# burchim/AVEC

Hardware: AMD Instinct MI355X
Metric: AV utterances/sec fwd+bwd (audio T=400, video 100x88x88) (higher is better)
Workload: dtype bf16

## Files before the change

avec_amd/csrc/api.hip:

```cpp
#include "common.h"
#include "avec_hip.h"
#include "vec.h"
#include "host_tables.h"
#include <stdarg.h>
#include <stdio.h>

static thread_local char g_err[512] = "";

void avec_set_error(const char* fmt, ...) {
  va_list ap; va_start(ap, fmt); vsnprintf(g_err, sizeof(g_err), fmt, ap); va_end(ap);
}
extern "C" const char* avec_last_error() { return g_err; }

static thread_local char g_kname[128] = "";
void avec_note_kernel(const char* fmt, ...) {
  va_list ap; va_start(ap, fmt); vsnprintf(g_kname, sizeof(g_kname), fmt, ap); va_end(ap);
}
extern "C" const char* avec_last_kernel() { return g_kname; }
extern "C" int avec_version() { return AVEC_ABI_VERSION; }
extern "C" int avec_struct_size(int which) {
  switch (which) {
    case 0: return (int)sizeof(avec_rows_t); case 1: return (int)sizeof(avec_epilogue_t); case 2: return (int)sizeof(avec_attn_t); case 3: return (int)sizeof(avec_tn_item_t);
    case 4: return (int)sizeof(avec_tn_batched_t); case 5: return (int)sizeof(avec_ln_item_t); case 6: return (int)sizeof(avec_fp8_item_t); case 7: return (int)sizeof(avec_wgrad3x3_item_t);
    case 8: return (int)sizeof(avec_ngram_t);
    default: return -1;
  }
}

static WsRegistry g_ws;
static LdsOptin g_lds;

extern "C" int avec_set_reduce_workspace(void* base, long long bytes) {
  int dev = 0; hipError_t e = hipGetDevice(&dev);
  AVEC_CHECK_ARG(e == hipSuccess && dev >= 0 && dev < WsRegistry::MAX_DEV, "set_reduce_workspace: no current device");
  AVEC_CHECK_ARG((base == nullptr && bytes == 0) || (base != nullptr && bytes >= (1 << 16) && ((size_t)base & 255) == 0),
                 "set_reduce_workspace: need a 256-byte aligned buffer of at least 64 KB (or NULL, 0 to unregister)");
  g_ws.set_default(dev, base, (size_t)bytes);
  return 0;
}
extern "C" int avec_set_reduce_workspace_stream(void* base, long long bytes, hipStream_t stream) {
  int dev = 0; hipError_t e = hipGetDevice(&dev);
  AVEC_CHECK_ARG(e == hipSuccess && dev >= 0 && dev < WsRegistry::MAX_DEV && base != nullptr && bytes >= (1 << 16) && ((size_t)base & 255) == 0, "set_reduce_workspace_stream: bad arguments");
  AVEC_CHECK_ARG(g_ws.set_stream(dev, stream, base, (size_t)bytes), "set_reduce_workspace_stream: at most %d stream-bound workspaces", WsRegistry::MAX_STREAMS);
  return 0;
}
ColWs avec_reduce_ws(size_t partial_floats, hipStream_t st) {
  int dev = 0; if (hipGetDevice(&dev) != hipSuccess) return ColWs{nullptr};
  return ColWs{(float*)g_ws.find(dev, st, partial_floats * sizeof(float))};
}

int avec_lds_optin_quiet(const void* kernel, size_t bytes) {
  if (bytes <= LdsOptin::FREE_BYTES) return 0;
  int dev = 0; if (hipGetDevice(&dev) != hipSuccess || dev < 0) return (int)hipErrorNoDevice;
  return g_lds.request(dev, kernel, bytes, [](const void* k, size_t n) {
    const hipError_t e = hipFuncSetAttribute(k, hipFuncAttributeMaxDynamicSharedMemorySize, (int)n);
    if (e != hipSuccess) (void)hipGetLastError();
    return (int)e;
  });
}
int avec_lds_optin(const void* kernel, size_t bytes) {
  const int r = avec_lds_optin_quiet(kernel, bytes);
  if (r == LdsOptin::TOO_LARGE) avec_set_error("%zu bytes of LDS requested (> 160 KiB)", bytes);
  else if (r) avec_set_error("cannot reserve %zu bytes of LDS: %s", bytes, hipGetErrorString((hipError_t)r));
  return r;
}
```

avec_amd/csrc/convmod.hip:

```cpp
#include "vec.h"
#include "avec_hip.h"

static constexpr int KMAX = 16;

template <typename T>
__device__ __forceinline__ void glu4(const T* u, long long row, int C, int col, float g[4]) {
  float a[4], b[4]; ld4<T>(u + row * 2 * C + col, a); ld4<T>(u + row * 2 * C + C + col, b);
  for (int e = 0; e < 4; ++e) g[e] = a[e] * sigmoidf_(b[e]);
}

static constexpr int DW_TT = 32;
template <typename T>
__device__ __forceinline__ void stage_glu(float* gs, const T* u, long long b, int Tn, int C, int col, int t_base, int nrows) {
  const int tx = threadIdx.x & 31, ty = threadIdx.x >> 5;
  for (int r0 = ty; r0 < nrows; r0 += 48) {
    float a[6][4], bq[6][4];
#pragma unroll
    for (int q = 0; q < 6; ++q) {
      const int r = r0 + 8 * q, t = t_base + r;
      const bool ok = r < nrows && col < C && t >= 0 && t < Tn;
      const long long row = ok ? b * Tn + t : b * Tn;
      const int cc = col < C ? col : 0;
      ld4<T>(u + row * 2 * C + cc, a[q]); ld4<T>(u + row * 2 * C + C + cc, bq[q]);
      if (!ok) { a[q][0] = a[q][1] = a[q][2] = a[q][3] = 0.f; }
// ... 144 lines not shown
      float g4[4], s1[4], s2[4];
      ld4<float>(bnb.ss + cc, bSc); ld4<float>(bnb.ss + C + cc, bSh); ld4<float>(bnb.ss + 2 * C + cc, bMu); ld4<float>(bnb.ss + 3 * C + cc, bRs);
      ld4<float>(bnb.gamma + cc, g4); ld4<float>(bnb.dstats + cc, s1); ld4<float>(bnb.dstats + C + cc, s2);
#pragma unroll
      for (int e = 0; e < 4; ++e) { bA[e] = g4[e] * bRs[e]; bM1[e] = s1[e] * bnb.inv_n; bM2[e] = s2[e] * bnb.inv_n; }
      if (blockIdx.y == 0 && ty == 0 && col < C && bnb.dgamma) {
#pragma unroll
        for (int e = 0; e < 4; ++e) { atomicAdd(bnb.dgamma + col + e, s2[e]); atomicAdd(bnb.dbeta + col + e, s1[e]); }
      }
    }
    for (int r0 = ty; r0 < nrows; r0 += 48) {
      float d[6][4];
#pragma unroll
      for (int q = 0; q < 6; ++q) {
        const int r = r0 + 8 * q, f = f0 + r; const bool ok = r < nrows && col < C && f >= 0 && f < Tn;
        ld4<T>(dc + ((long long)b * Tn + (ok ? f : 0)) * C + cc, d[q]);
        if (bnb.c) {
          float cv[4]; ld4<T>((const T*)bnb.c + ((long long)b * Tn + (ok ? f : 0)) * C + cc, cv);
#pragma unroll
          for (int e = 0; e < 4; ++e) { const float dd = d[q][e] * dswishf_(cv[e] * bSc[e] + bSh[e]); d[q][e] = bA[e] * (dd - bM1[e] - (cv[e] - bMu[e]) * bRs[e] * bM2[e]); }
        }
        if (!ok) d[q][0] = d[q][1] = d[q][2] = d[q][3] = 0.f;
      }
#pragma unroll
      for (int q = 0; q < 6; ++q) { const int r = r0 + 8 * q; if (r < nrows) *(float4*)(ds + r * 128 + tx * 4) = make_float4(d[q][0], d[q][1], d[q][2], d[q][3]); }
    }
  }
  __syncthreads();
  float part[KMAX + 1][4];
#pragma unroll
  for (int k = 0; k <= KMAX; ++k) for (int e = 0; e < 4; ++e) part[k][e] = 0.f;
  if (col < C) {
    float ww[KMAX][4];
#pragma unroll
    for (int k = 0; k < KMAX; ++k) { if (k < K) ld4<float>(w + (long long)k * C + col, ww[k]); else ww[k][0] = ww[k][1] = ww[k][2] = ww[k][3] = 0.f; }
    const int own = K - 1 - padl;
#pragma unroll
    for (int q = 0; q < DW_TT / 8; ++q) {
      const int r = ty + 8 * q;
      if (r >= nto) break;
      const long long row = (long long)b * Tn + t0 + r;
      float a[4], bq[4]; ld4<T>(u + row * 2 * C + col, a); ld4<T>(u + row * 2 * C + C + col, bq);
      const float4 dq = *(const float4*)(ds + (own + r) * 128 + tx * 4);
      part[KMAX][0] += dq.x; part[KMAX][1] += dq.y; part[KMAX][2] += dq.z; part[KMAX][3] += dq.w;
      float dg[4] = {0.f, 0.f, 0.f, 0.f};
#pragma unroll
      for (int k = 0; k < KMAX; ++k) {
        if (k < K) {
          const float4 g = *(const float4*)(gs + (r + k) * 128 + tx * 4);
          part[k][0] += dq.x * g.x; part[k][1] += dq.y * g.y; part[k][2] += dq.z * g.z; part[k][3] += dq.w * g.w;
          const float4 dd = *(const float4*)(ds + (r + K - 1 - k) * 128 + tx * 4);
          dg[0] += ww[k][0] * dd.x; dg[1] += ww[k][1] * dd.y; dg[2] += ww[k][2] * dd.z; dg[3] += ww[k][3] * dd.w;
        }
      }
      float o1[4], o2[4];
#pragma unroll
      for (int e = 0; e < 4; ++e) { const float sg = sigmoidf_(bq[e]); o1[e] = dg[e] * sg; o2[e] = dg[e] * a[e] * sg * (1.f - sg); }
      st4<T>(du + row * 2 * C + col, o1); st4<T>(du + row * 2 * C + C + col, o2);
    }
  }
  __syncthreads();
  const int lane = threadIdx.x & 63, wv = threadIdx.x >> 6;
#pragma unroll
  for (int k = 0; k <= KMAX; ++k)
#pragma unroll
    for (int e = 0; e < 4; ++e) part[k][e] += __shfl_xor(part[k][e], 32, 64);
  if (lane < 32) {
#pragma unroll
    for (int k = 0; k <= KMAX; ++k) *(float4*)(gs + ((wv * (KMAX + 1) + k) * 32 + tx) * 4) = make_float4(part[k][0], part[k][1], part[k][2], part[k][3]);
  }
  __syncthreads();
  float* mine = ws.partial ? ws_slot(ws, blockIdx.x, blockIdx.y, gridDim.y, (KMAX + 1) * 128) : nullptr;
  for (int i = threadIdx.x; i < (KMAX + 1) * 128; i += 256) {
    const int k = i >> 7, c = i & 127;
    const float v = gs[(0 * (KMAX + 1) + k) * 128 + c] + gs[(1 * (KMAX + 1) + k) * 128 + c] + gs[(2 * (KMAX + 1) + k) * 128 + c] + gs[(3 * (KMAX + 1) + k) * 128 + c];
    if (mine) mine[i] = v;
    else {
      const int cc = blockIdx.x * 128 + c;
      float* d = k == KMAX ? dbias : (k < K ? dw + (long long)k * C : nullptr);
      if (d && cc < C) atomicAdd(d + cc, v);
    }
  }
}

extern "C" int avec_glu_dwconv_fwd(int dtype, const void* u, const float* w, const float* bias, void* out, float* stats,
                                   int B, int T_, int C, int K, int stride, int pad_left, hipStream_t st) {
  AVEC_CHECK_ARG(u && w && out && B > 0 && T_ > 0 && C > 0 && C % 4 == 0 && K > 0 && K <= KMAX && stride > 0 && pad_left >= 0 && pad_left < K, "glu_dwconv_fwd: bad arguments (C=%d K=%d pad_left=%d)", C, K, pad_left);
  const int To = (T_ - 1) / stride + 1;
  const int nchunks = (To + DW_TT - 1) / DW_TT;
  dim3 grid((unsigned)((C / 4 + 31) / 32), (unsigned)(B * nchunks)); const ColPlan plan = ColPlan::grid<2>(grid, C, st, stats != nullptr);
  const size_t lds = (size_t)((DW_TT - 1) * stride + K) * 128 * sizeof(float);
  AVEC_CHECK_ARG(lds <= 64 * 1024, "glu_dwconv_fwd: stride %d too large", stride);
  DISPATCH_T(dtype, hipLaunchKernelGGL(glu_dwconv_fwd_kernel<T>, grid, dim3(256), lds, st, (const T*)u, w, bias, (T*)out, stats, B, T_, C, K, stride, To, pad_left, nchunks, plan.ws));
  AVEC_LAUNCH_CHECK();
  return plan.finish({stats, stats + C}, C, st);
}
__global__ __launch_bounds__(256) void bn_finalize_ws_kernel(const float* __restrict__ partial, int nslots, float count, const float* gamma, const float* beta, float* rmean, float* rvar,
                                                             long long* nbt, float momentum, float eps, float* ss, int C) {
  __shared__ float red[2][16][17];
  const int cl = threadIdx.x & 15, rl = threadIdx.x >> 4;
  const int c = blockIdx.x * 16 + cl;
  const bool lead = rl == 0 && c < C;
  float gm = 0.f, bt = 0.f, rm = 0.f, rv = 0.f;
  if (lead) { gm = gamma[c]; bt = beta[c]; if (rmean) { rm = rmean[c]; rv = rvar[c]; } }
  float s1 = 0.f, s2 = 0.f;
  if (c < C) {
    const float* p = partial + (size_t)(c >> 7) * nslots * 256 + (c & 127);
    for (int r = rl; r < nslots; r += 16) { s1 += p[(size_t)r * 256]; s2 += p[(size_t)r * 256 + 128]; }
  }
  red[0][rl][cl] = s1; red[1][rl][cl] = s2;
  __syncthreads();
  if (!lead) return;
  s1 = 0.f; s2 = 0.f;
#pragma unroll
  for (int k = 0; k < 16; ++k) { s1 += red[0][k][cl]; s2 += red[1][k][cl]; }
  const float n = count;
  const float mean = s1 / n, var = fmaxf(s2 / n - mean * mean, 0.f);
  if (rmean && isfinite(mean) && isfinite(var)) {
    rmean[c] = (1.f - momentum) * rm + momentum * mean;
    rvar[c] = (1.f - momentum) * rv + momentum * var * (n / fmaxf(n - 1.f, 1.f));
    if (c == 0 && nbt) *nbt += 1;
  }
  const float rs = rsqrtf(var + eps);
  ss[c] = gm * rs; ss[C + c] = bt - mean * gm * rs; ss[2 * C + c] = mean; ss[3 * C + c] = rs;
}

extern "C" int avec_glu_dwconv_fwd_bn(int dtype, const void* u, const float* w, const float* bias, void* out, float* stats, int B, int T_, int C, int K, int stride, int pad_left,
                                      const float* gamma, const float* beta, float* running_mean, float* running_var, long long* num_batches_tracked, float momentum, float eps,
                                      float* ss, hipStream_t st) {
  AVEC_CHECK_ARG(u && w && out && stats && gamma && beta && ss && B > 0 && T_ > 0 && C > 0 && C % 4 == 0 && K > 0 && K <= KMAX && stride > 0 && pad_left >= 0 && pad_left < K,
                 "glu_dwconv_fwd_bn: bad arguments (C=%d K=%d pad_left=%d)", C, K, pad_left);
  const int To = (T_ - 1) / stride + 1;
  const int nchunks = (To + DW_TT - 1) / DW_TT;
  dim3 grid((unsigned)((C / 4 + 31) / 32), (unsigned)(B * nchunks)); const ColPlan plan = ColPlan::grid<2>(grid, C, st);
  const size_t lds = (size_t)((DW_TT - 1) * stride + K) * 128 * sizeof(float);
  AVEC_CHECK_ARG(lds <= 64 * 1024, "glu_dwconv_fwd_bn: stride %d too large", stride);
  DISPATCH_T(dtype, hipLaunchKernelGGL(glu_dwconv_fwd_kernel<T>, grid, dim3(256), lds, st, (const T*)u, w, bias, (T*)out, stats, B, T_, C, K, stride, To, pad_left, nchunks, plan.ws));
  AVEC_LAUNCH_CHECK();
  const float count = (float)((long long)B * To);
  if (plan.ws.partial) {
    hipLaunchKernelGGL(bn_finalize_ws_kernel, dim3((C + 15) / 16), dim3(256), 0, st, (const float*)plan.ws.partial, (int)plan.nslots, count, gamma, beta, running_mean, running_var,
                       num_batches_tracked, momentum, eps, ss, C);
    AVEC_LAUNCH_CHECK();
    return 0;
  }
  return avec_bn_finalize(stats, 1, nullptr, count, gamma, beta, running_mean, running_var, num_batches_tracked, momentum, eps, ss, C, 1, st);
}
static int dw_finish(const ColPlan& plan, float* dw, float* dbias, int C, int K, hipStream_t st) {
  float* dst[KMAX + 1];
  for (int k = 0; k < KMAX; ++k) dst[k] = (k < K) ? dw + (long long)k * C : nullptr;
  dst[KMAX] = dbias;
  return plan.finish(dst, C, st);
}
extern "C" int avec_dwconv_glu_bwd_bn(int dtype, const void* da, const void* c, const float* ss, const float* gamma, const float* dstats, float count, const void* u, const float* w,
                                      void* du, float* dw, float* dbias, float* dgamma, float* dbeta, int B, int T_, int C, int K, int pad_left, hipStream_t st) {
  AVEC_CHECK_ARG(da && c && ss && gamma && dstats && count > 0.f && u && w && du && dw && B > 0 && T_ > 0 && C > 0 && C % 4 == 0 && K > 0 && K <= KMAX && pad_left >= 0 && pad_left < K,
                 "dwconv_glu_bwd_bn: bad arguments");
  AVEC_CHECK_ARG((dgamma == nullptr) == (dbeta == nullptr), "dwconv_glu_bwd_bn: dgamma and dbeta come together (both or neither)");
  const int nchunks = (T_ + DW_TT - 1) / DW_TT;
  dim3 grid((unsigned)((C / 4 + 31) / 32), (unsigned)(B * nchunks)); const ColPlan plan = ColPlan::grid<KMAX + 1>(grid, C, st);
  size_t l2 = (size_t)2 * (DW_TT - 1 + K) * 128 * sizeof(float);
  if (l2 < (size_t)4 * (KMAX + 1) * 128 * sizeof(float)) l2 = (size_t)4 * (KMAX + 1) * 128 * sizeof(float);
  AVEC_CHECK_ARG(l2 <= 64 * 1024, "dwconv_glu_bwd_bn: kernel size %d too large", K);
  DwBnb bnb{c, ss, gamma, dstats, 1.f / count, dgamma, dbeta};
  DISPATCH_T(dtype, hipLaunchKernelGGL(dwconv_glu_bwd_fused_kernel<T>, grid, dim3(256), l2, st, (const T*)da, (const T*)u, w, (T*)du, dw, dbias, B, T_, C, K, pad_left, nchunks, plan.ws, bnb));
  AVEC_LAUNCH_CHECK();
  return dw_finish(plan, dw, dbias, C, K, st);
}
extern "C" int avec_dwconv_glu_bwd(int dtype, const void* dc, const void* u, const float* w, void* du, float* dw, float* dbias,
                                   int B, int T_, int C, int K, int stride, int pad_left, hipStream_t st) {
  AVEC_CHECK_ARG(dc && u && w && du && dw && B > 0 && T_ > 0 && C > 0 && C % 4 == 0 && K > 0 && K <= KMAX && stride > 0 && pad_left >= 0 && pad_left < K, "dwconv_glu_bwd: bad arguments");
  const int To = (T_ - 1) / stride + 1;
  long long n4 = (long long)B * T_ * (C / 4); long long nb = (n4 + 255) / 256; if (nb > 4096) nb = 4096;
  const int nchunks = (To + DW_TT - 1) / DW_TT;
  dim3 grid((unsigned)((C / 4 + 31) / 32), (unsigned)(B * nchunks)); const ColPlan plan = ColPlan::grid<KMAX + 1>(grid, C, st);
  size_t lds = (size_t)((DW_TT - 1) * stride + K) * 128 * sizeof(float);
  if (lds < (size_t)4 * (KMAX + 1) * 128 * sizeof(float)) lds = (size_t)4 * (KMAX + 1) * 128 * sizeof(float);
  AVEC_CHECK_ARG(lds <= 64 * 1024, "dwconv_glu_bwd: stride %d too large", stride);
  if (stride == 1) {
    size_t l2 = (size_t)2 * (DW_TT - 1 + K) * 128 * sizeof(float); if (l2 < lds) l2 = lds;
    DISPATCH_T(dtype, hipLaunchKernelGGL(dwconv_glu_bwd_fused_kernel<T>, grid, dim3(256), l2, st, (const T*)dc, (const T*)u, w, (T*)du, dw, dbias, B, T_, C, K, pad_left, nchunks, plan.ws));
  } else
  DISPATCH_T(dtype, hipLaunchKernelGGL(dwconv_glu_bwd_input_kernel<T>, dim3((unsigned)nb), dim3(256), 0, st, (const T*)dc, (const T*)u, w, (T*)du, B, T_, C, K, stride, To, pad_left);
             hipLaunchKernelGGL(dwconv_bwd_weight_kernel<T>, grid, dim3(256), lds, st, (const T*)dc, (const T*)u, dw, dbias, B, T_, C, K, stride, To, pad_left, nchunks, plan.ws));
  AVEC_LAUNCH_CHECK();
  return dw_finish(plan, dw, dbias, C, K, st);
}

template <typename T>
__device__ __forceinline__ void glu_dwconv_stream_body(const T* __restrict__ u, const float* __restrict__ w, const float* __restrict__ bias, const float* __restrict__ ss,
                                                       T* __restrict__ out, T* state, long long p0, int n, int Tq, int C, int K, int stride, int To) {
  extern __shared__ __attribute__((aligned(16))) float gs[];
  const int tx = threadIdx.x & 31, ty = threadIdx.x >> 5; const int col = (blockIdx.x * 32 + tx) * 4; const int b = blockIdx.y;
  const int Hn = K - 1;
  const bool live = col < C; const int cc = live ? col : 0;
  float ww[KMAX][4], bb[4] = {0.f, 0.f, 0.f, 0.f}, sc[4], sh[4];
#pragma unroll
  for (int k = 0; k < KMAX; ++k) { if (k < K) ld4<float>(w + (long long)k * C + cc, ww[k]); else ww[k][0] = ww[k][1] = ww[k][2] = ww[k][3] = 0.f; }
  if (bias) ld4<float>(bias + cc, bb);
  ld4<float>(ss + cc, sc); ld4<float>(ss + C + cc, sh);
  T* const sb = state + (long long)b * Hn * 2 * C;
  const T* const ub = u + (long long)b * Tq * 2 * C;
  for (int r = ty; r < Hn + Tq; r += 8) {
    const bool ctx = r < Hn; const bool ok = live && (!ctx || p0 - Hn + r >= 0);
    const T* row = ctx ? sb + (long long)r * 2 * C : ub + (long long)(r - Hn) * 2 * C;
    float a[4], g[4]; ld4<T>(row + cc, a); ld4<T>(row + C + cc, g);
    *(float4*)(gs + r * 128 + tx * 4) = ok ? make_float4(a[0] * sigmoidf_(g[0]), a[1] * sigmoidf_(g[1]), a[2] * sigmoidf_(g[2]), a[3] * sigmoidf_(g[3])) : make_float4(0.f, 0.f, 0.f, 0.f);
  }
  float na[2][4], nb[2][4];
#pragma unroll
  for (int q = 0; q < 2; ++q) {
    const int r = ty + 8 * q;
    if (r < Hn && n > 0) {
      const int src = r + n; const T* row = src < Hn ? sb + (long long)src * 2 * C : ub + (long long)(src - Hn) * 2 * C;
      ld4<T>(row + cc, na[q]); ld4<T>(row + C + cc, nb[q]);
    }
  }
  __syncthreads();
  if (!live) return;
#pragma unroll
  for (int q = 0; q < 2; ++q) {
    const int r = ty + 8 * q;
    if (r < Hn && n > 0) { st4<T>(sb + (long long)r * 2 * C + col, na[q]); st4<T>(sb + (long long)r * 2 * C + C + col, nb[q]); }
  }
  for (int o = ty; o < To; o += 8) {
    float acc[4] = {bb[0], bb[1], bb[2], bb[3]};
#pragma unroll
    for (int k = 0; k < KMAX; ++k) {
      if (k < K) {
        const float4 g = *(const float4*)(gs + (o * stride + k) * 128 + tx * 4);
        acc[0] += ww[k][0] * g.x; acc[1] += ww[k][1] * g.y; acc[2] += ww[k][2] * g.z; acc[3] += ww[k][3] * g.w;
      }
    }
#pragma unroll
    for (int e = 0; e < 4; ++e) acc[e] = swishf_(acc[e] * sc[e] + sh[e]);
    st4<T>(out + ((long long)b * To + o) * C + col, acc);
  }
}
template <typename T>
__global__ __launch_bounds__(256) void glu_dwconv_stream_kernel(const T* __restrict__ u, const float* __restrict__ w, const float* __restrict__ bias, const float* __restrict__ ss,
                                                                T* __restrict__ out, T* state, const long long* __restrict__ pos, const unsigned char* __restrict__ reset,
                                                                const long long* __restrict__ clen, int div, int Tq, int C, int K, int stride, int To) {
  const int b = blockIdx.y;
  long long p0 = (reset && reset[b]) ? 0 : pos[b] / div; if (p0 < 0) p0 = 0;
  int n = Tq;
  if (clen) { long long c = (clen[b] + div - 1) / div; n = c < 0 ? 0 : (c > Tq ? Tq : (int)c); }
  glu_dwconv_stream_body<T>(u, w, bias, ss, out, state, p0, n, Tq, C, K, stride, To);
}
template <typename T>
__global__ __launch_bounds__(256) void glu_dwconv_stream_la_kernel(const T* __restrict__ u, const float* __restrict__ w, const float* __restrict__ bias, const float* __restrict__ ss,
                                                                   T* __restrict__ out, T* state, const long long* __restrict__ pos, const unsigned char* __restrict__ reset,
                                                                   const long long* __restrict__ ncommit, int div, int Wq, int C, int K, int stride, int To) {
  const int b = blockIdx.y;
  long long p0 = (reset && reset[b]) ? 0 : pos[b] / div; if (p0 < 0) p0 = 0;
  const long long c = ncommit[b] / div;
  glu_dwconv_stream_body<T>(u, w, bias, ss, out, state, p0, c < 0 ? 0 : (c > Wq ? Wq : (int)c), Wq, C, K, stride, To);
}

extern "C" long long avec_glu_dwconv_stream_state_bytes(int dtype, int B, int C, int K) {
  if (B <= 0 || C <= 0 || K <= 0) return 0;
  return (long long)B * (K - 1) * 2 * C * (dtype == AVEC_BF16 ? 2 : 4);
}
extern "C" int avec_glu_dwconv_stream(int dtype, const void* u, const float* w, const float* bias, const float* ss, void* out, void* state, long long state_bytes,
                                      const long long* pos, const unsigned char* reset, const long long* chunk_len, int div, int B, int Tq, int C, int K, int stride, hipStream_t st) {
  AVEC_CHECK_ARG(u && w && ss && out && pos, "glu_dwconv_stream: null pointer (u, w, ss, out and pos are required)");
  AVEC_CHECK_ARG(B > 0 && Tq > 0 && div > 0 && stride > 0 && Tq % stride == 0, "glu_dwconv_stream: bad dims B=%d Tq=%d div=%d stride=%d (Tq must be a multiple of the stride)", B, Tq, div, stride);
  AVEC_CHECK_ARG(C > 0 && C % 4 == 0, "glu_dwconv_stream: C=%d must be a positive multiple of 4 (4-channel vector accesses)", C);
  AVEC_CHECK_ARG(K > 0 && K <= KMAX, "glu_dwconv_stream: kernel size K=%d outside 1..%d", K, KMAX);
  AVEC_CHECK_ARG(K == 1 || state, "glu_dwconv_stream: null state (K=%d needs %d context rows per slot)", K, K - 1);
  AVEC_CHECK_ARG(state_bytes >= avec_glu_dwconv_stream_state_bytes(dtype, B, C, K), "glu_dwconv_stream: state of %lld bytes, %lld needed (avec_glu_dwconv_stream_state_bytes)",
                 state_bytes, avec_glu_dwconv_stream_state_bytes(dtype, B, C, K));
  AVEC_CHECK_ARG(avec_aligned16(u) && avec_aligned16(w) && avec_aligned16(bias) && avec_aligned16(ss) && avec_aligned16(out) && avec_aligned16(state),
                 "glu_dwconv_stream: u, w, bias, ss, out and state must be 16-byte aligned");
  AVEC_CHECK_ARG((((uintptr_t)pos) & 7) == 0 && (((uintptr_t)chunk_len) & 7) == 0, "glu_dwconv_stream: pos and chunk_len must be 8-byte aligned (int64)");
  const size_t lds = (size_t)(K - 1 + Tq) * 128 * sizeof(float);
  AVEC_CHECK_ARG(lds <= 48 * 1024, "glu_dwconv_stream: chunk of %d frames too long (K - 1 + Tq <= 96)", Tq);
  dim3 grid((unsigned)((C / 4 + 31) / 32), (unsigned)B);
  DISPATCH_T(dtype, hipLaunchKernelGGL(glu_dwconv_stream_kernel<T>, grid, dim3(256), lds, st, (const T*)u, w, bias, ss, (T*)out, (T*)state, pos, reset, chunk_len, div, Tq, C, K, stride, Tq / stride));
  AVEC_LAUNCH_CHECK();
  return 0;
}
extern "C" int avec_glu_dwconv_stream_la(int dtype, const void* u, const float* w, const float* bias, const float* ss, void* out, void* state, long long state_bytes,
                                         const long long* pos, const unsigned char* reset, const long long* ncommit, int div, int B, int Wq, int C, int K, int stride, hipStream_t st) {
  AVEC_CHECK_ARG(u && w && ss && out && pos && ncommit, "glu_dwconv_stream_la: null pointer (u, w, ss, out, pos and ncommit are required)");
  AVEC_CHECK_ARG(B > 0 && Wq > 0 && div > 0 && stride > 0 && Wq % stride == 0, "glu_dwconv_stream_la: bad dims B=%d Wq=%d div=%d stride=%d (Wq must be a multiple of the stride)", B, Wq, div, stride);
  AVEC_CHECK_ARG(C > 0 && C % 4 == 0, "glu_dwconv_stream_la: C=%d must be a positive multiple of 4 (4-channel vector accesses)", C);
  AVEC_CHECK_ARG(K > 0 && K <= KMAX, "glu_dwconv_stream_la: kernel size K=%d outside 1..%d", K, KMAX);
  AVEC_CHECK_ARG(K == 1 || state, "glu_dwconv_stream_la: null state (K=%d needs %d context rows per slot)", K, K - 1);
  AVEC_CHECK_ARG(state_bytes >= avec_glu_dwconv_stream_state_bytes(dtype, B, C, K), "glu_dwconv_stream_la: state of %lld bytes, %lld needed (avec_glu_dwconv_stream_state_bytes)",
                 state_bytes, avec_glu_dwconv_stream_state_bytes(dtype, B, C, K));
  AVEC_CHECK_ARG(avec_aligned16(u) && avec_aligned16(w) && avec_aligned16(bias) && avec_aligned16(ss) && avec_aligned16(out) && avec_aligned16(state),
                 "glu_dwconv_stream_la: u, w, bias, ss, out and state must be 16-byte aligned");
  AVEC_CHECK_ARG((((uintptr_t)pos) & 7) == 0 && (((uintptr_t)ncommit) & 7) == 0, "glu_dwconv_stream_la: pos and ncommit must be 8-byte aligned (int64)");
  const size_t lds = (size_t)(K - 1 + Wq) * 128 * sizeof(float);
  AVEC_CHECK_ARG(lds <= 48 * 1024, "glu_dwconv_stream_la: window of %d frames too long (K - 1 + Wq <= 96)", Wq);
  dim3 grid((unsigned)((C / 4 + 31) / 32), (unsigned)B);
  DISPATCH_T(dtype, hipLaunchKernelGGL(glu_dwconv_stream_la_kernel<T>, grid, dim3(256), lds, st, (const T*)u, w, bias, ss, (T*)out, (T*)state, pos, reset, ncommit, div, Wq, C, K, stride, Wq / stride));
  AVEC_LAUNCH_CHECK();
  return 0;
}
__global__ void stream_advance_kernel(long long* pos, unsigned char* reset, const long long* clen, long long full, int B) {
  const int b = blockIdx.x * blockDim.x + threadIdx.x;
  if (b >= B) return;
  long long c = clen ? clen[b] : full; c = c < 0 ? 0 : (c > full ? full : c);
  pos[b] = ((reset && reset[b]) ? 0 : pos[b]) + c;
  if (reset) reset[b] = 0;
}
extern "C" int avec_stream_advance(long long* pos, unsigned char* reset, const long long* chunk_len, long long full, int B, hipStream_t st) {
  AVEC_CHECK_ARG(pos && B > 0 && full > 0 && (((uintptr_t)pos) & 7) == 0 && (((uintptr_t)chunk_len) & 7) == 0, "stream_advance: bad arguments (B=%d full=%lld)", B, full);
  hipLaunchKernelGGL(stream_advance_kernel, dim3((B + 63) / 64), dim3(64), 0, st, pos, reset, chunk_len, full, B);
  AVEC_LAUNCH_CHECK();
  return 0;
}

__global__ __launch_bounds__(256) void stream_window_kernel(const float* __restrict__ x_new, const float* __restrict__ tail, float* __restrict__ X, const long long* __restrict__ pend,
                                                            const long long* __restrict__ n_new, const unsigned char* __restrict__ last, const unsigned char* __restrict__ reset,
                                                            const unsigned char* __restrict__ ended, long long* __restrict__ nvalid, long long* __restrict__ ncommit,
                                                            long long* __restrict__ emit, int Tc, int LAe, int D, int S) {
  const int r = blockIdx.x, b = blockIdx.y;
  const bool rs = reset && reset[b];
  long long pe = rs ? 0 : pend[b]; pe = pe < 0 ? 0 : (pe > LAe ? LAe : pe);
  long long nn = n_new ? n_new[b] : Tc; nn = nn < 0 ? 0 : (nn > Tc ? Tc : nn);
  if (!rs && ended[b]) { pe = 0; nn = 0; }
  const long long n = pe + nn;
  const float* src = r < pe ? tail + ((long long)b * LAe + r) * D : (r < n ? x_new + ((long long)b * Tc + (r - pe)) * D : nullptr);
  float* dst = X + ((long long)b * (Tc + LAe) + r) * D;
  for (int c = threadIdx.x; c < D; c += 256) dst[c] = src ? src[c] : 0.f;
  if (r == 0 && threadIdx.x == 0) {
    const bool ends = last && last[b];
    long long c = n - LAe; c = c < 0 ? 0 : c - c % S;
    nvalid[b] = n; ncommit[b] = ends ? 0 : c; emit[b] = ends ? n : c;
  }
}
extern "C" int avec_stream_window(const float* x_new, const float* tail, float* X, const long long* pend, const long long* n_new, const unsigned char* last, const unsigned char* reset,
                                  const unsigned char* ended, long long* nvalid, long long* ncommit, long long* emit, int B, int Tc, int LAe, int D, int S, hipStream_t st) {
  AVEC_CHECK_ARG(x_new && X && pend && ended && nvalid && ncommit && emit && (tail || LAe == 0),
                 "stream_window: null pointer (x_new, tail, X, pend, ended, nvalid, ncommit and emit are required)");
  AVEC_CHECK_ARG(B > 0 && Tc > 0 && LAe >= 0 && D > 0 && S > 0 && Tc % S == 0 && LAe % S == 0, "stream_window: bad dims B=%d Tc=%d LAe=%d D=%d S=%d (Tc and LAe must be multiples of S)", B, Tc, LAe, D, S);
  AVEC_CHECK_ARG(!(((uintptr_t)x_new | (uintptr_t)tail | (uintptr_t)X) & 3) && !(((uintptr_t)pend | (uintptr_t)n_new | (uintptr_t)nvalid | (uintptr_t)ncommit | (uintptr_t)emit) & 7),
// ... 38 lines not shown
```

avec_amd/csrc/norm.hip:

```cpp
#include "common.h"
#include "avec_hip.h"

#include "vec.h"
#include <type_traits>

__global__ __launch_bounds__(256) void col_finalize_kernel(ColFin f) {
  __shared__ float red[16][17];
  const int cw = threadIdx.x & 15, sl = threadIdx.x >> 4;
  const int ncols = f.NV * f.W;
  const int o = blockIdx.x * 16 + cw;
  const unsigned cb = blockIdx.y;
  const int s0 = blockIdx.z * 128;
  float s = 0.f;
  if (o < ncols) {
    const float* p = f.partial + ((size_t)cb * f.nslots) * ncols + o;
#pragma unroll
    for (int k = 0; k < 8; ++k) {
      const int si = s0 + sl + 16 * k; const int sc = si < f.nslots ? si : f.nslots - 1;
      const float v = p[(size_t)sc * ncols];
      s += si < f.nslots ? v : 0.f;
    }
  }
  red[sl][cw] = s;
  __syncthreads();
  if (sl == 0 && o < ncols) {
    float t = 0.f;
#pragma unroll
    for (int k = 0; k < 16; ++k) t += red[k][cw];
    const int n = o / f.W, w = o - n * f.W; const int col = (int)cb * f.W + w;
    float* d = nullptr;
#pragma unroll
    for (int i = 0; i < FIN_MAXNV; ++i) if (i == n) d = f.dst[i];
    if (d && col < f.C) atomicAdd(d + (long long)col * f.dstride, t);
  }
}
int col_finalize(const ColWs& ws, unsigned colblocks, unsigned nslots, int NV, int W, float* const* dst, int C, hipStream_t st, int dstride) {
  AVEC_CHECK_ARG(NV >= 1 && NV <= FIN_MAXNV, "col_finalize: %d reduced quantities (at most %d)", NV, FIN_MAXNV);
  ColFin f; f.partial = ws.partial; f.NV = NV; f.W = W; f.C = C; f.nslots = (int)nslots; f.dstride = dstride;
  for (int i = 0; i < FIN_MAXNV; ++i) f.dst[i] = i < NV ? dst[i] : nullptr;
  dim3 grid((unsigned)((NV * W + 15) / 16), colblocks, (nslots + 127) / 128);
  hipLaunchKernelGGL(col_finalize_kernel, grid, dim3(256), 0, st, f);
  AVEC_LAUNCH_CHECK(); return 0;
}

template <typename TO>
__global__ __launch_bounds__(256) void ln_fwd_kernel(const float* __restrict__ x, const float* __restrict__ g, const float* __restrict__ b,
                                                     TO* __restrict__ y, float* __restrict__ mean, float* __restrict__ rstd, long long M, int D, float eps) {
  const int lane = threadIdx.x & 63; const long long row = (long long)blockIdx.x * 4 + (threadIdx.x >> 6);
  if (row >= M) return;
  const float* xr = x + row * D;
  float s = 0.f;
  for (int c = lane * 4; c < D; c += 256) { float v[4]; ld4<float>(xr + c, v); s += v[0] + v[1] + v[2] + v[3]; }
  const float mu = wave_sum(s) / D;
  float q = 0.f;
  for (int c = lane * 4; c < D; c += 256) { float v[4]; ld4<float>(xr + c, v); for (int e = 0; e < 4; ++e) { float d = v[e] - mu; q += d * d; } }
  const float rs = rsqrtf(wave_sum(q) / D + eps);
  if (lane == 0) { mean[row] = mu; rstd[row] = rs; }
  for (int c = lane * 4; c < D; c += 256) {
    float v[4], gg[4], bb[4], o[4]; ld4<float>(xr + c, v); ld4<float>(g + c, gg); ld4<float>(b + c, bb);
    for (int e = 0; e < 4; ++e) o[e] = (v[e] - mu) * rs * gg[e] + bb[e];
    st4<TO>(y + row * D + c, o);
  }
}

template <typename TG, int NG>
__global__ __launch_bounds__(256) void ln_bwd_kernel(const TG* __restrict__ dy, const float* __restrict__ x, const float* __restrict__ mean,
                                                     const float* __restrict__ rstd, const float* __restrict__ g, float* dx, const float* dres,
                                                     float* __restrict__ dg, float* __restrict__ db, long long M, int D, ColWs ws) {
  const int lane = threadIdx.x & 63; const int wave_id = blockIdx.x * 4 + (threadIdx.x >> 6); const int nwaves = gridDim.x * 4;
  float pg[NG][4], pb[NG][4], gg[NG][4];
#pragma unroll
  for (int i = 0; i < NG; ++i) {
    const int c = lane * 4 + i * 256;
#pragma unroll
    for (int e = 0; e < 4; ++e) { pg[i][e] = 0.f; pb[i][e] = 0.f; gg[i][e] = 0.f; }
    if (c < D) ld4<float>(g + c, gg[i]);
  }
  struct RowData { float d[NG][4], v[NG][4], o[NG][4], mu, rs; };
  auto fetch = [&](long long row, RowData& r) {
    r.mu = mean[row]; r.rs = rstd[row];
#pragma unroll
    for (int i = 0; i < NG; ++i) {
      const int c = lane * 4 + i * 256;
      if (c < D) {
        ld4<TG>(dy + row * D + c, r.d[i]); ld4<float>(x + row * D + c, r.v[i]);
        if (dres) ld4<float>(dres + row * D + c, r.o[i]); else { r.o[i][0] = r.o[i][1] = r.o[i][2] = r.o[i][3] = 0.f; }
      } else {
#pragma unroll
        for (int e = 0; e < 4; ++e) { r.d[i][e] = 0.f; r.v[i][e] = r.mu; r.o[i][e] = 0.f; }
      }
    }
  };
  RowData cur, nxt;
  long long row = wave_id;
  if (row < M) fetch(row, cur);
  for (; row < M; row += nwaves) {
    const bool more = row + nwaves < M;
    if (more) fetch(row + nwaves, nxt);
    float s1 = 0.f, s2 = 0.f;
#pragma unroll
    for (int i = 0; i < NG; ++i)
#pragma unroll
      for (int e = 0; e < 4; ++e) {
        const float xh = (cur.v[i][e] - cur.mu) * cur.rs, t = cur.d[i][e] * gg[i][e];
        cur.v[i][e] = xh; s1 += t; s2 += t * xh; pg[i][e] += cur.d[i][e] * xh; pb[i][e] += cur.d[i][e];
      }
    s1 = wave_sum(s1) / D; s2 = wave_sum(s2) / D;
#pragma unroll
    for (int i = 0; i < NG; ++i) {
      const int c = lane * 4 + i * 256; if (c >= D) break;
#pragma unroll
      for (int e = 0; e < 4; ++e) cur.o[i][e] += cur.rs * (cur.d[i][e] * gg[i][e] - s1 - cur.v[i][e] * s2);
      st4<float>(dx + row * D + c, cur.o[i]);
    }
    if (more) cur = nxt;
  }
  extern __shared__ float lnred[];
  for (int c = threadIdx.x; c < 2 * D; c += 256) lnred[c] = 0.f;
  __syncthreads();
#pragma unroll
  for (int i = 0; i < NG; ++i) {
    int c = lane * 4 + i * 256; if (c >= D) break;
    for (int e = 0; e < 4; ++e) { atomicAdd(lnred + c + e, pg[i][e]); atomicAdd(lnred + D + c + e, pb[i][e]); }
  }
  __syncthreads();
  if (!ws.partial) { for (int c = threadIdx.x; c < D; c += 256) { atomicAdd(dg + c, lnred[c]); atomicAdd(db + c, lnred[D + c]); } return; }
  float* mine = ws_slot(ws, 0, blockIdx.x, gridDim.x, 2 * D);
  for (int c = threadIdx.x; c < 2 * D; c += 256) mine[c] = lnred[c];
}

extern "C" int avec_layernorm_fwd(int dtype, const float* x, const float* gamma, const float* beta, void* y, int y_f32,
                                  float* mean, float* rstd, long long M, int D, float eps, hipStream_t st) {
  AVEC_CHECK_ARG(x && gamma && beta && y && mean && rstd, "layernorm_fwd: null pointer");
  AVEC_CHECK_ARG(M > 0 && D > 0 && D % 4 == 0, "layernorm_fwd: D=%d must be a positive multiple of 4", D);
  dim3 grid((unsigned)((M + 3) / 4));
  if (y_f32 || dtype == AVEC_F32) hipLaunchKernelGGL(ln_fwd_kernel<float>, grid, dim3(256), 0, st, x, gamma, beta, (float*)y, mean, rstd, M, D, eps);
  else hipLaunchKernelGGL(ln_fwd_kernel<bf16>, grid, dim3(256), 0, st, x, gamma, beta, (bf16*)y, mean, rstd, M, D, eps);
  AVEC_LAUNCH_CHECK(); return 0;
}

struct LnPrep { void* out; float alpha, p; const unsigned long long* rng; unsigned stream; int f32; };
template <typename TG, int NG>
__global__ __launch_bounds__(256) void ln_bwd_rows_kernel(const TG* __restrict__ dy, const float* __restrict__ x, const float* __restrict__ mean,
                                                          const float* __restrict__ rstd, const float* __restrict__ g, float* __restrict__ dx,
                                                          const float* __restrict__ dres, long long M, int D, LnPrep pr) {
  const int lane = threadIdx.x & 63; const long long row = (long long)blockIdx.x * 4 + (threadIdx.x >> 6);
  if (row >= M) return;
  const float mu = mean[row], rs = rstd[row];
  DropKey dk; dk.k0 = 0u; dk.thr = 0u; dk.scale = 1.f;
  if (pr.out) dk = drop_key(pr.rng, pr.stream, pr.p);
  float d[NG][4], v[NG][4], o[NG][4], gg[NG][4];
#pragma unroll
  for (int i = 0; i < NG; ++i) {
    const int c = lane * 4 + i * 256;
    if (c < D) {
      ld4<TG>(dy + row * D + c, d[i]); ld4<float>(x + row * D + c, v[i]); ld4<float>(g + c, gg[i]);
      if (dres) ld4<float>(dres + row * D + c, o[i]); else { o[i][0] = o[i][1] = o[i][2] = o[i][3] = 0.f; }
    } else {
#pragma unroll
      for (int e = 0; e < 4; ++e) { d[i][e] = 0.f; v[i][e] = mu; o[i][e] = 0.f; gg[i][e] = 0.f; }
    }
  }
  float s1 = 0.f, s2 = 0.f;
#pragma unroll
  for (int i = 0; i < NG; ++i)
#pragma unroll
    for (int e = 0; e < 4; ++e) { const float xh = (v[i][e] - mu) * rs, t = d[i][e] * gg[i][e]; v[i][e] = xh; s1 += t; s2 += t * xh; }
  s1 = wave_sum(s1) / D; s2 = wave_sum(s2) / D;
#pragma unroll
  for (int i = 0; i < NG; ++i) {
    const int c = lane * 4 + i * 256; if (c >= D) break;
#pragma unroll
    for (int e = 0; e < 4; ++e) o[i][e] += rs * (d[i][e] * gg[i][e] - s1 - v[i][e] * s2);
    st4<float>(dx + row * D + c, o[i]);
    if (pr.out) {
      float q[4];
      float ds[4]; drop4(dk, (unsigned long long)row * D + c, ds);
#pragma unroll
      for (int e = 0; e < 4; ++e) q[e] = o[i][e] * (pr.alpha * ds[e]);
      if (pr.f32) st4<float>((float*)pr.out + row * D + c, q); else st4<bf16>((bf16*)pr.out + row * D + c, q);
    }
  }
}

template <typename TO>
__global__ __launch_bounds__(256) void ln_fwd2_kernel(const float* __restrict__ x, const float* __restrict__ g1, const float* __restrict__ b1, float eps1,
                                                      float* __restrict__ y1, float* __restrict__ mean1, float* __restrict__ rstd1,
                                                      const float* __restrict__ g2, const float* __restrict__ b2, float eps2,
                                                      TO* __restrict__ h2, float* __restrict__ mean2, float* __restrict__ rstd2, long long M, int D) {
  const int lane = threadIdx.x & 63; const long long row = (long long)blockIdx.x * 4 + (threadIdx.x >> 6);
  if (row >= M) return;
  float v[2][4];
#pragma unroll
  for (int i = 0; i < 2; ++i) { const int c = lane * 4 + i * 256; if (c < D) ld4<float>(x + row * D + c, v[i]); else v[i][0] = v[i][1] = v[i][2] = v[i][3] = 0.f; }
  auto norm = [&](const float* g, const float* b, float eps, float* mean, float* rstd) {
    float sm = 0.f;
#pragma unroll
    for (int i = 0; i < 2; ++i) sm += v[i][0] + v[i][1] + v[i][2] + v[i][3];
    const float mu = wave_sum(sm) / D;
    float q = 0.f;
#pragma unroll
    for (int i = 0; i < 2; ++i) { const int c = lane * 4 + i * 256; if (c < D) for (int e = 0; e < 4; ++e) { const float d = v[i][e] - mu; q += d * d; } }
    const float rs = rsqrtf(wave_sum(q) / D + eps);
    if (lane == 0) { mean[row] = mu; rstd[row] = rs; }
#pragma unroll
    for (int i = 0; i < 2; ++i) {
      const int c = lane * 4 + i * 256; if (c >= D) break;
      float gg[4], bb[4]; ld4<float>(g + c, gg); ld4<float>(b + c, bb);
      for (int e = 0; e < 4; ++e) v[i][e] = (v[i][e] - mu) * rs * gg[e] + bb[e];
    }
  };
  norm(g1, b1, eps1, mean1, rstd1);
#pragma unroll
  for (int i = 0; i < 2; ++i) { const int c = lane * 4 + i * 256; if (c < D) st4<float>(y1 + row * D + c, v[i]); }
  norm(g2, b2, eps2, mean2, rstd2);
#pragma unroll
  for (int i = 0; i < 2; ++i) { const int c = lane * 4 + i * 256; if (c < D) st4<TO>(h2 + row * D + c, v[i]); }
}
extern "C" int avec_layernorm_fwd2(int dtype, const float* x, const float* gamma1, const float* beta1, float eps1, float* y1, float* mean1, float* rstd1,
                                   const float* gamma2, const float* beta2, float eps2, void* h2, float* mean2, float* rstd2, long long M, int D, hipStream_t st) {
  AVEC_CHECK_ARG(x && gamma1 && beta1 && y1 && mean1 && rstd1 && gamma2 && beta2 && h2 && mean2 && rstd2, "layernorm_fwd2: null pointer");
  AVEC_CHECK_ARG(M > 0 && D > 0 && D % 4 == 0 && D <= 512, "layernorm_fwd2: D=%d must be a multiple of 4 in [4, 512]", D);
  dim3 grid((unsigned)((M + 3) / 4));
  if (dtype == AVEC_F32) hipLaunchKernelGGL(ln_fwd2_kernel<float>, grid, dim3(256), 0, st, x, gamma1, beta1, eps1, y1, mean1, rstd1, gamma2, beta2, eps2, (float*)h2, mean2, rstd2, M, D);
  else hipLaunchKernelGGL(ln_fwd2_kernel<bf16>, grid, dim3(256), 0, st, x, gamma1, beta1, eps1, y1, mean1, rstd1, gamma2, beta2, eps2, (bf16*)h2, mean2, rstd2, M, D);
  AVEC_LAUNCH_CHECK(); return 0;
}
template <typename TG>
__global__ __launch_bounds__(256) void ln_bwd_rows2_kernel(const TG* __restrict__ dy2, const float* __restrict__ x2, const float* __restrict__ mean2, const float* __restrict__ rstd2,
                                                           const float* __restrict__ g2, const float* __restrict__ dres2, float* __restrict__ dx2,
                                                           const float* __restrict__ x1, const float* __restrict__ mean1, const float* __restrict__ rstd1,
                                                           const float* __restrict__ g1, float* __restrict__ dx1, long long M, int D, LnPrep pr) {
  const int lane = threadIdx.x & 63; const long long row = (long long)blockIdx.x * 4 + (threadIdx.x >> 6);
  if (row >= M) return;
  float d[2][4], v[2][4], o[2][4], gg[2][4], w1[2][4], gg1[2][4];
  const float mu2 = mean2[row], rs2 = rstd2[row], mu1 = mean1[row], rs1 = rstd1[row];
  DropKey dk; dk.k0 = 0u; dk.thr = 0u; dk.scale = 1.f;
  if (pr.out) dk = drop_key(pr.rng, pr.stream, pr.p);
#pragma unroll
  for (int i = 0; i < 2; ++i) {
    const int c = lane * 4 + i * 256;
    if (c < D) {
      ld4<TG>(dy2 + row * D + c, d[i]); ld4<float>(x2 + row * D + c, v[i]); ld4<float>(g2 + c, gg[i]); ld4<float>(x1 + row * D + c, w1[i]); ld4<float>(g1 + c, gg1[i]);
      if (dres2) ld4<float>(dres2 + row * D + c, o[i]); else { o[i][0] = o[i][1] = o[i][2] = o[i][3] = 0.f; }
    } else {
#pragma unroll
      for (int e = 0; e < 4; ++e) { d[i][e] = 0.f; v[i][e] = mu2; o[i][e] = 0.f; gg[i][e] = 0.f; w1[i][e] = mu1; gg1[i][e] = 0.f; }
    }
  }
  float s1 = 0.f, s2 = 0.f;
#pragma unroll
  for (int i = 0; i < 2; ++i)
#pragma unroll
    for (int e = 0; e < 4; ++e) { const float xh = (v[i][e] - mu2) * rs2, t = d[i][e] * gg[i][e]; v[i][e] = xh; s1 += t; s2 += t * xh; }
  s1 = wave_sum(s1) / D; s2 = wave_sum(s2) / D;
#pragma unroll
  for (int i = 0; i < 2; ++i) {
    const int c = lane * 4 + i * 256;
#pragma unroll
    for (int e = 0; e < 4; ++e) o[i][e] += rs2 * (d[i][e] * gg[i][e] - s1 - v[i][e] * s2);
    if (c < D) st4<float>(dx2 + row * D + c, o[i]); else { o[i][0] = o[i][1] = o[i][2] = o[i][3] = 0.f; }
  }
  float t1 = 0.f, t2 = 0.f;
#pragma unroll
  for (int i = 0; i < 2; ++i)
#pragma unroll
    for (int e = 0; e < 4; ++e) { const float xh = (w1[i][e] - mu1) * rs1, t = o[i][e] * gg1[i][e]; w1[i][e] = xh; t1 += t; t2 += t * xh; }
  t1 = wave_sum(t1) / D; t2 = wave_sum(t2) / D;
#pragma unroll
  for (int i = 0; i < 2; ++i) {
    const int c = lane * 4 + i * 256; if (c >= D) break;
    float r[4];
#pragma unroll
    for (int e = 0; e < 4; ++e) r[e] = rs1 * (o[i][e] * gg1[i][e] - t1 - w1[i][e] * t2);
    st4<float>(dx1 + row * D + c, r);
    if (pr.out) {
      float q[4], ds[4]; drop4(dk, (unsigned long long)row * D + c, ds);
#pragma unroll
      for (int e = 0; e < 4; ++e) q[e] = r[e] * (pr.alpha * ds[e]);
      if (pr.f32) st4<float>((float*)pr.out + row * D + c, q); else st4<bf16>((bf16*)pr.out + row * D + c, q);
    }
  }
}
extern "C" int avec_layernorm_bwd2(int dtype, const void* dy2, const float* x2, const float* mean2, const float* rstd2, const float* gamma2, const float* dres2, float* dx2,
                                   const float* x1, const float* mean1, const float* rstd1, const float* gamma1, float* dx1,
                                   void* prep, float prep_alpha, float prep_drop_p, const unsigned long long* rng, unsigned rng_stream, long long M, int D, hipStream_t st) {
  AVEC_CHECK_ARG(dy2 && x2 && mean2 && rstd2 && gamma2 && dx2 && x1 && mean1 && rstd1 && gamma1 && dx1, "layernorm_bwd2: null pointer");
  AVEC_CHECK_ARG(M > 0 && D > 0 && D % 4 == 0 && D <= 512 && (!prep || prep_drop_p <= 0.f || rng), "layernorm_bwd2: D=%d must be a multiple of 4 in [4, 512]; dropout needs rng", D);
  LnPrep pr; pr.out = prep; pr.alpha = prep_alpha; pr.p = prep ? prep_drop_p : 0.f; pr.rng = rng; pr.stream = rng_stream; pr.f32 = dtype == AVEC_F32;
  dim3 grid((unsigned)((M + 3) / 4));
  if (dtype == AVEC_F32) hipLaunchKernelGGL(ln_bwd_rows2_kernel<float>, grid, dim3(256), 0, st, (const float*)dy2, x2, mean2, rstd2, gamma2, dres2, dx2, x1, mean1, rstd1, gamma1, dx1, M, D, pr);
  else hipLaunchKernelGGL(ln_bwd_rows2_kernel<bf16>, grid, dim3(256), 0, st, (const bf16*)dy2, x2, mean2, rstd2, gamma2, dres2, dx2, x1, mean1, rstd1, gamma1, dx1, M, D, pr);
  AVEC_LAUNCH_CHECK(); return 0;
}

struct LnItem { const void* dy; const float* x; const float* mean; const float* rstd; float* dg; float* db; int M, D, dy_f32, first; };
struct LnGroup { LnItem it[AVEC_LN_GROUP_MAX]; int n; };
static constexpr int LNG_ROWS = 128;
__global__ __launch_bounds__(256) void ln_param_grads_grouped_kernel(LnGroup grp) {
  __shared__ float red[2][256][4];
  const int w = blockIdx.x;
  int lo = 0, hi = grp.n - 1;
  while (lo < hi) { const int mid = (lo + hi + 1) >> 1; if (grp.it[mid].first <= w) lo = mid; else hi = mid - 1; }
  const LnItem& t = grp.it[lo];
  const int D = t.D, L = D >> 2, R = 256 / L;
  const int r = threadIdx.x / L, l = threadIdx.x - r * L;
  const int m0 = (w - t.first) * LNG_ROWS; int m1 = m0 + LNG_ROWS; if (m1 > t.M) m1 = t.M;
  float pg[4] = {0.f, 0.f, 0.f, 0.f}, pb[4] = {0.f, 0.f, 0.f, 0.f};
  if (r < R) {
    constexpr int U = 8;
    for (int m = m0 + r; m < m1; m += R * U) {
      float d[U][4], v[U][4], mu[U], rs[U];
#pragma unroll
      for (int u = 0; u < U; ++u) {
        const int mm = m + u * R; const bool ok = mm < m1; const long long mi = ok ? mm : m;
        if (t.dy_f32) ld4<float>((const float*)t.dy + mi * D + l * 4, d[u]); else ld4<bf16>((const bf16*)t.dy + mi * D + l * 4, d[u]);
        ld4<float>(t.x + mi * D + l * 4, v[u]); mu[u] = t.mean[mi]; rs[u] = ok ? t.rstd[mi] : 0.f;
        if (!ok) d[u][0] = d[u][1] = d[u][2] = d[u][3] = 0.f;
      }
#pragma unroll
      for (int u = 0; u < U; ++u)
#pragma unroll
        for (int e = 0; e < 4; ++e) { pg[e] += d[u][e] * (v[u][e] - mu[u]) * rs[u]; pb[e] += d[u][e]; }
    }
  }
#pragma unroll
  for (int e = 0; e < 4; ++e) { red[0][threadIdx.x][e] = pg[e]; red[1][threadIdx.x][e] = pb[e]; }
  __syncthreads();
  for (int o = threadIdx.x; o < 2 * D; o += 256) {
    const int which = o >= D, c = o - which * D; float s = 0.f;
    for (int rr = 0; rr < R; ++rr) s += red[which][rr * L + (c >> 2)][c & 3];
    atomicAdd((which ? t.db : t.dg) + c, s);
  }
}
extern "C" int avec_layernorm_param_grads_grouped(int dtype, const avec_ln_item_t* items, int n, hipStream_t st) {
  AVEC_CHECK_ARG(items && n > 0 && n <= AVEC_LN_GROUP_MAX, "layernorm_param_grads_grouped: need 1..%d items (got %d)", AVEC_LN_GROUP_MAX, n);
  LnGroup grp; grp.n = n; int first = 0;
  for (int k = 0; k < n; ++k) {
    const avec_ln_item_t& s = items[k];
    AVEC_CHECK_ARG(s.dy && s.x && s.mean && s.rstd && s.dgamma && s.dbeta && s.M > 0 && s.M < (1ll << 31) && s.D >= 4 && s.D % 4 == 0 && s.D <= 1024,
                   "layernorm_param_grads_grouped: item %d: null pointer or D=%d not a multiple of 4 in [4, 1024]", k, s.D);
    LnItem& t = grp.it[k];
    t.dy = s.dy; t.x = s.x; t.mean = s.mean; t.rstd = s.rstd; t.dg = s.dgamma; t.db = s.dbeta; t.M = (int)s.M; t.D = s.D;
    t.dy_f32 = (s.dy_f32 || dtype == AVEC_F32) ? 1 : 0; t.first = first;
    first += (int)((s.M + LNG_ROWS - 1) / LNG_ROWS);
  }
  hipLaunchKernelGGL(ln_param_grads_grouped_kernel, dim3((unsigned)first), dim3(256), 0, st, grp);
  AVEC_LAUNCH_CHECK(); return 0;
}

static int layernorm_bwd_impl(int dtype, const void* dy, int dy_f32, const float* x, const float* mean, const float* rstd, const float* gamma,
                              float* dx, const float* dres, float* dgamma, float* dbeta, long long M, int D, const LnPrep& pr, hipStream_t st) {
  AVEC_CHECK_ARG(dy && x && mean && rstd && gamma && dx && (!dgamma == !dbeta), "layernorm_bwd: null pointer");
  AVEC_CHECK_ARG(M > 0 && D > 0 && D % 4 == 0 && D <= 1536, "layernorm_bwd: D=%d must be a multiple of 4 and <= 1536", D);
  AVEC_CHECK_ARG(!pr.out || (!dgamma && (pr.p <= 0.f || pr.rng)), "layernorm_bwd_prep: the second output comes with the dx-only kernel (dgamma == NULL); dropout needs rng");
  if (!dgamma) {
    const dim3 grid((unsigned)((M + 3) / 4)); const bool f32in = dy_f32 || dtype == AVEC_F32;
#define AVEC_LN_ROWS(TG, NG) hipLaunchKernelGGL((ln_bwd_rows_kernel<TG, NG>), grid, dim3(256), 0, st, (const TG*)dy, x, mean, rstd, gamma, dx, dres, M, D, pr)
    if (D <= 512) { if (f32in) AVEC_LN_ROWS(float, 2); else AVEC_LN_ROWS(bf16, 2); }
    else { if (f32in) AVEC_LN_ROWS(float, 6); else AVEC_LN_ROWS(bf16, 6); }
#undef AVEC_LN_ROWS
    AVEC_LAUNCH_CHECK(); return 0;
  }
  long long nb = (M + 15) / 16; if (nb > 256) nb = 256; if (nb < 1) nb = 1;
  const ColPlan plan = ColPlan::flat<2>((unsigned)nb, D, st).cap_without_ws(128);
  const size_t lds = (size_t)2 * D * sizeof(float);
#define AVEC_LN_BWD(TG, NG) hipLaunchKernelGGL((ln_bwd_kernel<TG, NG>), dim3(plan.nslots), dim3(256), lds, st, (const TG*)dy, x, mean, rstd, gamma, dx, dres, dgamma, dbeta, M, D, plan.ws)
  const bool f32in = dy_f32 || dtype == AVEC_F32;
  if (D <= 512) { if (f32in) AVEC_LN_BWD(float, 2); else AVEC_LN_BWD(bf16, 2); }
  else { if (f32in) AVEC_LN_BWD(float, 6); else AVEC_LN_BWD(bf16, 6); }
#undef AVEC_LN_BWD
  AVEC_LAUNCH_CHECK();
  return plan.finish({dgamma, dbeta}, D, st);
}
extern "C" int avec_layernorm_bwd(int dtype, const void* dy, int dy_f32, const float* x, const float* mean, const float* rstd, const float* gamma,
                                  float* dx, const float* dres, float* dgamma, float* dbeta, long long M, int D, hipStream_t st) {
  LnPrep pr; pr.out = nullptr; pr.alpha = 1.f; pr.p = 0.f; pr.rng = nullptr; pr.stream = 0; pr.f32 = 0;
  return layernorm_bwd_impl(dtype, dy, dy_f32, x, mean, rstd, gamma, dx, dres, dgamma, dbeta, M, D, pr, st);
}
extern "C" int avec_layernorm_bwd_prep(int dtype, const void* dy, int dy_f32, const float* x, const float* mean, const float* rstd, const float* gamma,
                                       float* dx, const float* dres, void* prep, float prep_alpha, float prep_drop_p, const unsigned long long* rng, unsigned rng_stream,
                                       long long M, int D, hipStream_t st) {
  AVEC_CHECK_ARG(prep, "layernorm_bwd_prep: null prep buffer");
  LnPrep pr; pr.out = prep; pr.alpha = prep_alpha; pr.p = prep_drop_p; pr.rng = rng; pr.stream = rng_stream; pr.f32 = dtype == AVEC_F32;
  return layernorm_bwd_impl(dtype, dy, dy_f32, x, mean, rstd, gamma, dx, dres, nullptr, nullptr, M, D, pr, st);
}

template <typename T>
__global__ __launch_bounds__(256) void grad_prep_kernel(const float* __restrict__ dout, long long ldd, T* __restrict__ dacc, float alpha, float p,
                                                        const unsigned long long* rng, unsigned stream, float* dbias, long long M, int N, ColWs ws) {
  const int tx = threadIdx.x & 31, ty = threadIdx.x >> 5;
  const int col = (blockIdx.x * 32 + tx) * 4;
  float part[1][4] = {{0.f, 0.f, 0.f, 0.f}};
  const DropKey dk = drop_key(rng, stream, p);
  if (col < N) {
    for (long long row = (long long)blockIdx.y * 8 + ty; row < M; row += (long long)gridDim.y * 8) {
      float v[4]; ld4<float>(dout + row * ldd + col, v);
      float ds[4]; drop4(dk, (unsigned long long)row * N + col, ds);
      for (int e = 0; e < 4; ++e) { v[e] *= alpha * ds[e]; part[0][e] += v[e]; }
      st4<T>(dacc + row * N + col, v);
    }
  }
  float* const dst[1] = {dbias};
  if (dbias) colreduce_atomic<1>(part, dst, col, N, ws);
}

template <typename T>
__global__ __launch_bounds__(256) void grad_prep_flat_kernel(const float* __restrict__ dout, long long ldd, T* __restrict__ dacc, float alpha, float p,
                                                             const unsigned long long* rng, unsigned stream, long long M, int N) {
  const int N4 = N >> 2; const long long n4 = M * N4;
  const DropKey dk = drop_key(rng, stream, p);
  for (long long i = (long long)blockIdx.x * 256 + threadIdx.x; i < n4; i += (long long)gridDim.x * 256) {
    const long long row = n4 < (1ll << 31) ? (long long)((unsigned)i / (unsigned)N4) : i / N4; const int col = (int)(i - row * N4) * 4;
    float v[4]; ld4<float>(dout + row * ldd + col, v);
    float ds[4]; drop4(dk, (unsigned long long)row * N + col, ds);
    for (int e = 0; e < 4; ++e) v[e] *= alpha * ds[e];
    st4<T>(dacc + row * N + col, v);
  }
}
extern "C" int avec_grad_prep(int dtype, const float* dout, long long ld, void* dacc, float alpha, float drop_p, const unsigned long long* rng,
                              unsigned rng_stream, float* dbias, long long M, int N, hipStream_t st) {
  AVEC_CHECK_ARG(dout && dacc && M > 0 && N > 0 && N % 4 == 0 && ld % 4 == 0, "grad_prep: bad arguments (N=%d ld=%lld)", N, ld);
  AVEC_CHECK_ARG(!(drop_p > 0.f) || rng, "grad_prep: dropout without rng");
  if (!dbias) {
    long long nb = (M * (N / 4) + 255) / 256; if (nb > 8192) nb = 8192;
    DISPATCH_T(dtype, hipLaunchKernelGGL(grad_prep_flat_kernel<T>, dim3((unsigned)nb), dim3(256), 0, st, dout, ld, (T*)dacc, alpha, drop_p, rng, rng_stream, M, N));
    AVEC_LAUNCH_CHECK(); return 0;
  }
  dim3 grid = col_grid(M, N); const ColPlan plan = ColPlan::grid<1>(grid, N, st);
  DISPATCH_T(dtype, hipLaunchKernelGGL(grad_prep_kernel<T>, grid, dim3(256), 0, st, dout, ld, (T*)dacc, alpha, drop_p, rng, rng_stream, dbias, M, N, plan.ws));
  AVEC_LAUNCH_CHECK();
  return plan.finish({dbias}, N, st);
}

template <typename T>
__global__ __launch_bounds__(256) void colsum_kernel(const T* __restrict__ x, long long ld, float* out, long long M, int N, ColWs ws) {
  const int tx = threadIdx.x & 31, ty = threadIdx.x >> 5; const int col = (blockIdx.x * 32 + tx) * 4;
  float part[1][4] = {{0.f, 0.f, 0.f, 0.f}};
  if (col < N) for (long long row = (long long)blockIdx.y * 8 + ty; row < M; row += (long long)gridDim.y * 8) {
    float v[4]; ld4<T>(x + row * ld + col, v); for (int e = 0; e < 4; ++e) part[0][e] += v[e];
  }
  float* const dst[1] = {out};
  colreduce_atomic<1>(part, dst, col, N, ws);
}
extern "C" int avec_colsum(int dtype, const void* x, long long ld, float* out, long long M, int N, hipStream_t st) { return colsum_launch(dtype, x, ld, out, M, N, true, st); }
int colsum_launch(int dtype, const void* x, long long ld, float* out, long long M, int N, bool use_ws, hipStream_t st) {
  AVEC_CHECK_ARG(x && out && M > 0 && N > 0 && N % 4 == 0 && ld % 4 == 0, "colsum: bad arguments");
  dim3 grid = col_grid(M, N); if (!use_ws && grid.y > 16) grid.y = 16; const ColPlan plan = ColPlan::grid<1>(grid, N, st, use_ws);
  DISPATCH_T(dtype, hipLaunchKernelGGL(colsum_kernel<T>, grid, dim3(256), 0, st, (const T*)x, ld, out, M, N, plan.ws));
  AVEC_LAUNCH_CHECK();
  return plan.finish({out}, N, st);
}

template <typename T>
__global__ __launch_bounds__(256) void bn_stats_kernel(const T* __restrict__ y, float* stats, long long M, int C, ColWs ws) {
  const int tx = threadIdx.x & 31, ty = threadIdx.x >> 5; const int col = (blockIdx.x * 32 + tx) * 4;
  float part[2][4] = {{0.f, 0.f, 0.f, 0.f}, {0.f, 0.f, 0.f, 0.f}};
  if (col < C) for (long long row = (long long)blockIdx.y * 8 + ty; row < M; row += (long long)gridDim.y * 8) {
    float v[4]; ld4<T>(y + row * C + col, v); for (int e = 0; e < 4; ++e) { part[0][e] += v[e]; part[1][e] += v[e] * v[e]; }
  }
  float* const dst[2] = {stats, stats + C};
  colreduce_atomic<2>(part, dst, col, C, ws);
}
extern "C" int avec_bn_stats(int dtype, const void* y, float* stats, long long M, int C, hipStream_t st) {
  AVEC_CHECK_ARG(y && stats && M > 0 && C > 0 && C % 4 == 0, "bn_stats: bad arguments");
  dim3 grid = col_grid(M, C); const ColPlan plan = ColPlan::grid<2>(grid, C, st);
  DISPATCH_T(dtype, hipLaunchKernelGGL(bn_stats_kernel<T>, grid, dim3(256), 0, st, (const T*)y, stats, M, C, plan.ws));
  AVEC_LAUNCH_CHECK();
  return plan.finish({stats, stats + C}, C, st);
}

__global__ __launch_bounds__(256) void bn_finalize_kernel(const float* stats, int nrep, const float* count_ptr, float count, const float* gamma, const float* beta, float* rmean, float* rvar,
                                                          long long* nbt, float momentum, float eps, float* ss, int C, int training) {
  __shared__ float red[2][16][17];
  const int cl = threadIdx.x & 15, rl = threadIdx.x >> 4;
  const int c = blockIdx.x * 16 + cl;
  const bool lead = rl == 0 && c < C;
  float gm = 0.f, bt = 0.f, rm = 0.f, rv = 0.f, n = count;
  if (lead) { gm = gamma[c]; bt = beta[c]; if (rmean) { rm = rmean[c]; rv = rvar[c]; } if (training && count_ptr) n = *count_ptr; }
  float s1 = 0.f, s2 = 0.f;
  if (training && c < C) for (int r = rl; r < nrep; r += 16) { s1 += stats[(long long)r * 2 * C + c]; s2 += stats[(long long)r * 2 * C + C + c]; }
  red[0][rl][cl] = s1; red[1][rl][cl] = s2;
  __syncthreads();
  if (!lead) return;
  float mean, var;
  if (training) {
    s1 = 0.f; s2 = 0.f;
#pragma unroll
    for (int k = 0; k < 16; ++k) { s1 += red[0][k][cl]; s2 += red[1][k][cl]; }
    mean = s1 / n; var = fmaxf(s2 / n - mean * mean, 0.f);
    if (rmean && isfinite(mean) && isfinite(var)) {
      rmean[c] = (1.f - momentum) * rm + momentum * mean;
      rvar[c] = (1.f - momentum) * rv + momentum * var * (n / fmaxf(n - 1.f, 1.f));
      if (c == 0 && nbt) *nbt += 1;
    }
  } else { mean = rm; var = rv; }
  const float rs = rsqrtf(var + eps);
  ss[c] = gm * rs; ss[C + c] = bt - mean * gm * rs; ss[2 * C + c] = mean; ss[3 * C + c] = rs;
}
__global__ __launch_bounds__(256) void bn_collapse_kernel(const float* __restrict__ stats, int nrep, float count, float* __restrict__ out, int C2) {
  const int c = blockIdx.x * 256 + threadIdx.x;
  if (c < C2) { float s = 0.f; for (int r = 0; r < nrep; ++r) s += stats[(long long)r * C2 + c]; out[c] = s; }
  if (c == 0) out[C2] = count;
}
__global__ __launch_bounds__(256) void bn_affine_grads_kernel(const float* __restrict__ dstats, float* dgamma, float* dbeta, int C) {
  const int c = blockIdx.x * 256 + threadIdx.x;
  if (c < C) { dgamma[c] += dstats[C + c]; dbeta[c] += dstats[c]; }
}
extern "C" int avec_bn_collapse(const float* stats, int n_replicas, float count, float* out, int C, hipStream_t st) {
  AVEC_CHECK_ARG(stats && out && n_replicas > 0 && C > 0, "bn_collapse: bad arguments");
  hipLaunchKernelGGL(bn_collapse_kernel, dim3((2 * C + 255) / 256), dim3(256), 0, st, stats, n_replicas, count, out, 2 * C);
  AVEC_LAUNCH_CHECK(); return 0;
}
extern "C" int avec_bn_affine_grads(const float* dstats, float* dgamma, float* dbeta, int C, hipStream_t st) {
  AVEC_CHECK_ARG(dstats && dgamma && dbeta && C > 0, "bn_affine_grads: bad arguments");
  hipLaunchKernelGGL(bn_affine_grads_kernel, dim3((C + 255) / 256), dim3(256), 0, st, dstats, dgamma, dbeta, C);
  AVEC_LAUNCH_CHECK(); return 0;
}
extern "C" int avec_bn_finalize(const float* stats, int n_replicas, const float* count_ptr, float count, const float* gamma, const float* beta, float* running_mean,
                                float* running_var, long long* num_batches_tracked, float momentum, float eps, float* ss, int C, int training, hipStream_t st) {
  AVEC_CHECK_ARG(gamma && beta && ss && C > 0 && (training ? (stats != nullptr) : (running_mean && running_var)), "bn_finalize: bad arguments");
  hipLaunchKernelGGL(bn_finalize_kernel, dim3((C + 15) / 16), dim3(256), 0, st, stats, n_replicas > 0 ? n_replicas : 1, count_ptr, count, gamma, beta, running_mean, running_var,
                     num_batches_tracked, momentum, eps, ss, C, training);
  AVEC_LAUNCH_CHECK(); return 0;
}

__global__ void stamp_kernel(unsigned long long* out, int i) { if (threadIdx.x == 0) out[i] = wall_clock64(); }
extern "C" int avec_stamp(unsigned long long* out, int slot, hipStream_t st) {
  AVEC_CHECK_ARG(out && slot >= 0, "stamp: bad arguments");
  hipLaunchKernelGGL(stamp_kernel, dim3(1), dim3(64), 0, st, out, slot);
  AVEC_LAUNCH_CHECK(); return 0;
}

__global__ __launch_bounds__(256) void bn_bwd_finalize_kernel(const float* __restrict__ stats, int nrep, const float* __restrict__ ss, float* __restrict__ dstats, int C) {
  const int c = blockIdx.x * 256 + threadIdx.x;
  if (c >= C) return;
  float s1 = 0.f, sy = 0.f;
  for (int r = 0; r < nrep; ++r) { s1 += stats[(long long)r * 2 * C + c]; sy += stats[(long long)r * 2 * C + C + c]; }
  dstats[c] = s1; dstats[C + c] = ss[3 * C + c] * (sy - ss[2 * C + c] * s1);
// ... 666 lines not shown
```

avec_amd/lib.py:

```python
import ctypes
import os
import re

_HERE = os.path.dirname(os.path.abspath(__file__))
HEADER = os.path.join(os.path.dirname(_HERE), "include", "avec_hip.h")
LIB_PATH = os.environ.get("AVEC_LIB_PATH") or os.path.join(_HERE, "libavec_hip.so")

F32, BF16 = 0, 1
ROWS_PLAIN, ROWS_CONV_FWD, ROWS_CONV_BWD, ROWS_STEM3D = 0, 1, 2, 3
ACT_NONE, ACT_SWISH, ACT_RELU, ACT_GELU = 0, 1, 2, 3


class Rows(ctypes.Structure):
    _fields_ = [("ld", ctypes.c_longlong), ("rows_out", ctypes.c_int), ("rows_in", ctypes.c_int), ("step", ctypes.c_int),
                ("H", ctypes.c_int), ("W", ctypes.c_int), ("C", ctypes.c_int), ("KH", ctypes.c_int), ("KW", ctypes.c_int),
                ("stride", ctypes.c_int), ("pad", ctypes.c_int), ("OH", ctypes.c_int), ("OW", ctypes.c_int), ("T3", ctypes.c_int)]


class Epilogue(ctypes.Structure):
    _fields_ = [("out", ctypes.c_void_p), ("ldo", ctypes.c_longlong), ("out_f32", ctypes.c_int),
                ("out_pre", ctypes.c_void_p), ("ldpre", ctypes.c_longlong),
                ("bias", ctypes.c_void_p), ("act", ctypes.c_int),
                ("drop_p", ctypes.c_float), ("rng", ctypes.c_void_p), ("rng_stream", ctypes.c_uint),
                ("res", ctypes.c_void_p), ("ldres", ctypes.c_longlong), ("alpha", ctypes.c_float), ("res_act", ctypes.c_int),
                ("dact_z", ctypes.c_void_p), ("ldz", ctypes.c_longlong), ("dact", ctypes.c_int),
                ("colsum", ctypes.c_void_p), ("stats", ctypes.c_void_p),
                ("bnb_y", ctypes.c_void_p), ("ldby", ctypes.c_longlong), ("bnb_ss", ctypes.c_void_p), ("bnb_mask", ctypes.c_int),
                ("res_cls0", ctypes.c_int), ("res_mask", ctypes.c_void_p)]


class Attn(ctypes.Structure):
    _fields_ = [("q", ctypes.c_void_p), ("k", ctypes.c_void_p), ("v", ctypes.c_void_p), ("ld", ctypes.c_longlong),
                ("e", ctypes.c_void_p), ("lde", ctypes.c_longlong),
                ("lens", ctypes.c_void_p), ("len_div", ctypes.c_int), ("q_full", ctypes.c_int),
                ("mask", ctypes.c_void_p), ("mask_bstride", ctypes.c_longlong),
                ("o", ctypes.c_void_p), ("ldo", ctypes.c_longlong), ("lse", ctypes.c_void_p),
                ("dout", ctypes.c_void_p),
                ("dq", ctypes.c_void_p), ("dk", ctypes.c_void_p), ("dv", ctypes.c_void_p), ("lddq", ctypes.c_longlong), ("ldd", ctypes.c_longlong),
                ("de", ctypes.c_void_p), ("ldde", ctypes.c_longlong), ("pbuf", ctypes.c_void_p), ("dsbuf", ctypes.c_void_p), ("ldt", ctypes.c_longlong), ("dsrel", ctypes.c_void_p), ("ldr", ctypes.c_longlong),
                ("B", ctypes.c_int), ("H", ctypes.c_int), ("T", ctypes.c_int), ("d", ctypes.c_int), ("scale", ctypes.c_float), ("Tk", ctypes.c_int)]


class TnItem(ctypes.Structure):
    _fields_ = [("P", ctypes.c_void_p), ("Q", ctypes.c_void_p), ("O", ctypes.c_void_p), ("p_colsum", ctypes.c_void_p),
                ("ldp", ctypes.c_longlong), ("ldq", ctypes.c_longlong), ("ldo", ctypes.c_longlong), ("M", ctypes.c_longlong),
                ("I", ctypes.c_int), ("J", ctypes.c_int), ("q_rows_out", ctypes.c_int), ("q_rows_in", ctypes.c_int), ("q_step", ctypes.c_int),
                ("reserved", ctypes.c_int)]


class TnBatched(ctypes.Structure):
    _fields_ = [("P", ctypes.c_void_p), ("ldp", ctypes.c_longlong), ("Q", ctypes.c_void_p), ("ldq", ctypes.c_longlong),
                ("O", ctypes.c_void_p), ("O_act", ctypes.c_void_p), ("ldo", ctypes.c_longlong),
                ("M", ctypes.c_longlong), ("I", ctypes.c_int), ("J", ctypes.c_int), ("nb_outer", ctypes.c_int), ("nb_inner", ctypes.c_int),
                ("strides6", ctypes.POINTER(ctypes.c_longlong))]


class LnItem(ctypes.Structure):
    _fields_ = [("dy", ctypes.c_void_p), ("x", ctypes.c_void_p), ("mean", ctypes.c_void_p), ("rstd", ctypes.c_void_p), ("dgamma", ctypes.c_void_p),
                ("dbeta", ctypes.c_void_p), ("M", ctypes.c_longlong), ("D", ctypes.c_int), ("dy_f32", ctypes.c_int)]


class Fp8Item(ctypes.Structure):
    _fields_ = [("src", ctypes.c_void_p), ("dst", ctypes.c_void_p), ("n", ctypes.c_longlong), ("slot", ctypes.c_int), ("K", ctypes.c_int), ("Kp", ctypes.c_int),
                ("reserved", ctypes.c_int)]


class WgradItem(ctypes.Structure):
    _fields_ = [("x", ctypes.c_void_p), ("dy", ctypes.c_void_p), ("dw", ctypes.c_void_p), ("images", ctypes.c_longlong), ("C", ctypes.c_int), ("H", ctypes.c_int),
                ("W", ctypes.c_int), ("reserved", ctypes.c_int)]


class NGram(ctypes.Structure):
    _fields_ = [("order", ctypes.c_int), ("V", ctypes.c_int), ("unigram", ctypes.c_void_p), ("ctx_cap", ctypes.c_longlong), ("ctx_key", ctypes.c_void_p),
                ("ctx_bo", ctypes.c_void_p), ("ctx_off", ctypes.c_void_p), ("ctx_cnt", ctypes.c_void_p), ("cont_tok", ctypes.c_void_p), ("cont_lp", ctypes.c_void_p)]


TN_GROUP_MAX, LN_GROUP_MAX, WGRAD_GROUP_MAX = 32, 40, 16
ABI_STRUCTS = (Rows, Epilogue, Attn, TnItem, TnBatched, LnItem, Fp8Item, WgradItem, NGram)


def _ctype(decl):
    decl = decl.strip()
    if "*" in decl or decl.startswith("hipStream_t"):
        return ctypes.c_void_p
    base = re.sub(r"\b[A-Za-z_][A-Za-z_0-9]*$", "", decl).strip() or decl
    base = base.replace("const", "").strip()
    return {"int": ctypes.c_int, "long long": ctypes.c_longlong, "float": ctypes.c_float, "unsigned": ctypes.c_uint,
            "void": None}[base]


def declared_functions(header=HEADER):
    txt = open(header).read()
    txt = re.sub(r"/\*.*?\*/", " ", txt, flags=re.S)
    out = {}
    for m in re.finditer(r"(?:^|\n)\s*(const char\*|long long|int)\s+(avec_[a-z0-9_]+)\s*\(([^;{]*?)\)\s*;", txt):
        ret, name, args = m.group(1), m.group(2), m.group(3)
        args = " ".join(args.split())
        argtypes = [] if args in ("", "void") else [_ctype(a) for a in args.split(",")]
        restype = {"int": ctypes.c_int, "long long": ctypes.c_longlong, "const char*": ctypes.c_char_p}[ret]
        out[name] = (restype, argtypes)
    return out


class _Lib:
    def __init__(self):
        self._dll = None

    def load(self):
        if self._dll is None:
            if not os.path.exists(LIB_PATH):
                raise RuntimeError("libavec_hip.so not found at %s -- build it with `python -m avec_amd.build` "
                                   "(there is no non-HIP fallback)" % LIB_PATH)
            dll = ctypes.CDLL(LIB_PATH)
            for name, (restype, argtypes) in declared_functions().items():
                fn = getattr(dll, name)
                fn.restype = restype
                fn.argtypes = argtypes
            want = int(re.search(r"#define AVEC_ABI_VERSION (\d+)", open(HEADER).read()).group(1))
            if dll.avec_version() != want:
                raise RuntimeError("libavec_hip.so ABI version %d, include/avec_hip.h declares %d: rebuild (python -m avec_amd.build)" % (dll.avec_version(), want))
            for which, st in enumerate(ABI_STRUCTS):
                if dll.avec_struct_size(which) != ctypes.sizeof(st):
                    raise RuntimeError("libavec_hip.so: sizeof(%s) is %d in the library, %d in avec_amd/lib.py" % (st.__name__, dll.avec_struct_size(which), ctypes.sizeof(st)))
            self._dll = dll
        return self._dll

    def __getattr__(self, name):
        fn = getattr(self.load(), "avec_" + name)

        def call(*args):
            rc = fn(*args)
            if rc != 0:
                raise RuntimeError("avec_%s failed (%d): %s" % (name, rc, self._dll.avec_last_error().decode()))
        call.__name__ = name
        self.__dict__[name] = call
        return call

    def raw(self, name):
        return getattr(self.load(), name)


lib = _Lib()
```

avec_amd/ops.py:

```python
import collections
import ctypes
import os

import torch

from . import fp8
from . import runtime as rt
from .lib import (ACT_GELU, ACT_NONE, ACT_RELU, ACT_SWISH, BF16, LN_GROUP_MAX, ROWS_CONV_BWD, ROWS_CONV_FWD, ROWS_PLAIN, ROWS_STEM3D, TN_GROUP_MAX, WGRAD_GROUP_MAX, Attn, Epilogue, LnItem, Rows, TnBatched, TnItem,
                  WgradItem, lib)

_byref = ctypes.byref


class KernelTimer:
    NAMES = {(0, ROWS_CONV_FWD): "gemm_nt<conv_fwd>", (0, ROWS_CONV_BWD): "gemm_nt<conv_bwd_data>", (0, ROWS_STEM3D): "gemm_nt<stem3d>",
             (0, ROWS_PLAIN): "gemm_nt<plain>", (1, ROWS_CONV_FWD): "gemm_tn<conv_wgrad>", (1, ROWS_STEM3D): "gemm_tn<stem3d_wgrad>",
             (1, ROWS_PLAIN): "gemm_tn<plain>", (2, 0): "conv3x3_slab<fwd>", (2, 1): "conv3x3_slab<bwd_data>", (2, 2): "conv3x3_slab<wgrad>"}

    def __init__(self):
        self.enabled = False
        self.records = []

    def reset(self, enabled):
        self.enabled, self.records = enabled, []

    def start(self):
        if not self.enabled:
            return None
        e = torch.cuda.Event(enable_timing=True)
        e.record()
        return e

    def stop(self, e0, key, flops, abytes=0.0):
        if e0 is None:
            return
        e1 = torch.cuda.Event(enable_timing=True)
        e1.record()
        name = lib.raw("avec_last_kernel")()
        self.records.append((key, flops, e0, e1, name.decode() if name else "", float(abytes)))

    def bracket_overhead_us(self, n=200):
        evs = []
        for _ in range(n):
            a, b = torch.cuda.Event(enable_timing=True), torch.cuda.Event(enable_timing=True)
            a.record(); b.record()
            evs.append((a, b))
        torch.cuda.synchronize()
        d = sorted(a.elapsed_time(b) * 1e3 for a, b in evs)
        return d[len(d) // 2]

    def summary(self, peak_tflops, steps=1):
        if not self.records:
            return None
        torch.cuda.synchronize()
        ovh = self.bracket_overhead_us() * 1e-6
        agg, rows = {}, {}
        for key, flops, e0, e1, name, ab in self.records:
            dt = max(e0.elapsed_time(e1) * 1e-3 - ovh, 1e-7)
            a = agg.setdefault(key, [0.0, 0.0, 0])
            a[0] += dt; a[1] += flops; a[2] += 1
            r = rows.setdefault(name or self.NAMES.get(key, str(key)), [0.0, 0.0, 0, 0.0])
            r[0] += dt; r[1] += flops; r[2] += 1; r[3] += ab

        def row(name, v):
            return {"kernel": name, "launches_per_step": round(v[2] / steps, 1), "avg_us": round(1e6 * v[0] / v[2], 2), "ms_per_step": round(1e3 * v[0] / steps, 3),
                    "alg_gflop_per_launch": round(v[1] / v[2] / 1e9, 3), "alg_bytes_per_launch": round(v[3] / v[2]), "tflops": round(v[1] / v[0] / 1e12, 1),
                    "frac": round(v[1] / v[0] / 1e12 / peak_tflops, 4)}
        ordered = sorted(rows.items(), key=lambda kv: -kv[1][0])
        top_name, top = ordered[0]
        t_all = sum(v[0] for v in rows.values()); f_all = sum(v[1] for v in rows.values())
        achieved = top[1] / top[0] / 1e12
        return {"bound": "mfma", "kernel": top_name, "achieved": round(achieved, 2), "peak": peak_tflops, "unit": "TFLOP/s",
                "frac": round(achieved / peak_tflops, 5), "traffic": None, "launches": round(top[2] / steps, 1), "avg_launch_ms": round(1e3 * top[0] / top[2], 5),
                "alg_gflop_per_launch": round(top[1] / top[2] / 1e9, 3), "alg_bytes_per_launch": round(top[3] / top[2]),
                "event_bracket_overhead_us": round(ovh * 1e6, 2),
                "rows": [row(n, v) for n, v in ordered[:8]],
                "gemm_family_total": {"ms_per_step": round(1e3 * t_all / steps, 3), "tflops": round(f_all / t_all / 1e12, 1), "frac": round(f_all / t_all / 1e12 / peak_tflops, 4)},
                "families": {self.NAMES.get(k, str(k)): {"ms_total": round(1e3 * v[0] / steps, 3), "tflops": round(v[1] / v[0] / 1e12, 2), "launches": round(v[2] / steps, 1)}
                             for k, v in sorted(agg.items(), key=lambda kv: -kv[1][0])}}


KERNEL_TIMER = KernelTimer()


def _p(t):
    return None if t is None else t.data_ptr()


def _rng(device, drop_p=1.0):
    return rt.rng_state(device).data_ptr() if drop_p > 0 else None


STAMPS = {"on": os.environ.get("AVEC_STAMPS", "0") == "1", "buf": None, "names": []}


def stamp(name):
    if not STAMPS["on"]:
        return
    if STAMPS["buf"] is None:
        STAMPS["buf"] = torch.zeros(256, dtype=torch.int64, device="cuda")
    if name not in STAMPS["names"]:
        STAMPS["names"].append(name)
    lib.stamp(STAMPS["buf"].data_ptr(), STAMPS["names"].index(name), rt.stream())


class StampFn(torch.autograd.Function):

    @staticmethod
    def forward(ctx, x, name):
        ctx.name = name
        stamp(name + ":f")
        return x.view_as(x)

    @staticmethod
    def backward(ctx, g):
        stamp(ctx.name + ":b")
        return g, None


def mark(x, name):
    return StampFn.apply(x, name) if (STAMPS["on"] and torch.is_tensor(x) and x.requires_grad) else (stamp(name + ":f") or x)


def grad_of(p):
    if p.grad is None:
        p.grad = torch.zeros_like(p)
    return p.grad


def empty(shape, dtype, ref):
    if dtype == torch.bfloat16 and len(shape) == 2 and shape[1] % 8:
        n = shape[0] * shape[1]
        return torch.empty(n + 8, dtype=dtype, device=ref.device)[:n].view(shape)
    return torch.empty(shape, dtype=dtype, device=ref.device)


def _chunk_readable(t, ld, width, rows):
    if width % 8 == 0 and ld % 8 == 0 and t.data_ptr() % 16 == 0:
        return True
    if ld >= (width + 7) // 8 * 8:
        return True
    st = t.untyped_storage()
    end = (t.storage_offset() + (rows - 1) * ld + (width + 7) // 8 * 8) * t.element_size()
    return end <= st.nbytes()


def rows_plain(ld, rows_out=1, rows_in=1, step=0):
    r = Rows()
    r.ld, r.rows_out, r.rows_in, r.step = ld, rows_out, rows_in, step
    return r


def rows_conv(H, W, C, KH, KW, stride, pad, OH, OW):
    r = Rows()
    r.H, r.W, r.C, r.KH, r.KW, r.stride, r.pad, r.OH, r.OW = H, W, C, KH, KW, stride, pad, OH, OW
    return r


def gemm_nt_fp8(A, ent, out, M, N, K, *, bias=None, act=ACT_NONE, out_pre=None, drop_p=0.0, sid=0, res=None, alpha=1.0, out_f32=False, ldo=None):
    Kp = ent.Kp
    q = torch.empty((M, Kp), dtype=torch.uint8, device=A.device)
    lib.fp8_quantize(rt.dt(), A.data_ptr(), K, q.data_ptr(), Kp, M, K, ent.a_amax, 1, rt.stream())
    ep = Epilogue()
    ep.out, ep.ldo, ep.out_f32 = out.data_ptr(), (N if ldo is None else ldo), int(out_f32)
    if out_pre is not None:
        ep.out_pre, ep.ldpre = out_pre.data_ptr(), N
    ep.bias, ep.act, ep.alpha = _p(bias), act, alpha
    if drop_p > 0.0:
        ep.drop_p, ep.rng, ep.rng_stream = drop_p, _rng(out.device, drop_p), sid
    if res is not None:
        ep.res, ep.ldres, ep.res_act = res.data_ptr(), N, 0
    ev = KERNEL_TIMER.start()
    lib.gemm_nt_fp8(q.data_ptr(), Kp, ent.wq, Kp, M, N, Kp, ent.a_amax, ent.w_amax, _byref(ep), rt.stream())
    KERNEL_TIMER.stop(ev, (0, 0), 2.0 * M * N * K)
    return out


def gemm_nt(A, W, out, M, N, K, *, rows=None, mode=ROWS_PLAIN, a_f32=False, ldw=None, bias=None, act=ACT_NONE, out_pre=None,
            drop_p=0.0, sid=0, res=None, res_act=False, alpha=1.0, dact_z=None, dact=0, colsum=None, stats=None, out_f32=False,
            ldo=None, ldres=None, dtype=None, flops=None, bnb=None, res_cls0=False, abytes=None, res_mask=None):
    ep = Epilogue()
    ep.out, ep.ldo, ep.out_f32 = out.data_ptr(), (N if ldo is None else ldo), int(out_f32)
    if out_pre is not None:
        ep.out_pre, ep.ldpre = out_pre.data_ptr(), N
    ep.bias = _p(bias)
    ep.act = act
    if drop_p > 0.0:
        ep.drop_p, ep.rng, ep.rng_stream = drop_p, _rng(out.device, drop_p), sid
    if res is not None:
        ep.res, ep.ldres, ep.res_act, ep.res_cls0 = res.data_ptr(), (N if ldres is None else ldres), int(res_act), int(res_cls0)
        if res_mask is not None:
            ep.res_mask = res_mask.data_ptr()
    ep.alpha = alpha
    if dact_z is not None:
        ep.dact_z, ep.ldz, ep.dact = dact_z.data_ptr(), N, dact
    ep.colsum, ep.stats = _p(colsum), _p(stats)
    if bnb is not None:
        ep.bnb_y, ep.ldby, ep.stats = bnb.y.data_ptr(), N, bnb.stats.data_ptr()
        if bnb.mask_z is not None:
            ep.dact_z, ep.ldz, ep.dact, ep.bnb_mask = bnb.mask_z.data_ptr(), N, 2, 0
        else:
            ep.bnb_ss, ep.bnb_mask = bnb.ss.data_ptr(), 1
    if rows is None:
        rows = rows_plain(K)
    ev = KERNEL_TIMER.start()
    lib.gemm_nt(rt.dt() if dtype is None else dtype, A.data_ptr(), _byref(rows), mode, int(a_f32), W.data_ptr(),
                K if ldw is None else ldw, M, N, K, _byref(ep), rt.stream())
    esz = A.element_size()
    KERNEL_TIMER.stop(ev, (0, mode), 2.0 * M * N * K if flops is None else flops,
                      ((M * K + N * K) * esz + M * N * (4 if out_f32 else esz)) if abytes is None else abytes)
    return out


DEFER_WGRAD = os.environ.get("AVEC_DEFER_WGRAD", "1") != "0"


_QueueKind = collections.namedtuple("_QueueKind", "item group_max launcher dtype timer_key abytes flush_when_full")


def _wgrad3x3_bytes(it):
    return 2.0 * 2 * it.images * it.H * it.W * it.C + 4.0 * 9 * it.C * it.C


_QUEUE_KINDS = {
    "tn": _QueueKind(TnItem, TN_GROUP_MAX, "gemm_tn_grouped", lambda: BF16, (1, ROWS_PLAIN), lambda it: 2.0 * it.M * (it.I + it.J) + 4.0 * it.I * it.J, True),
    "ln": _QueueKind(LnItem, LN_GROUP_MAX, "layernorm_param_grads_grouped", rt.dt, None, None, True),
    "cw": _QueueKind(WgradItem, WGRAD_GROUP_MAX, "wgrad3x3_c128_grouped", None, (2, 2), _wgrad3x3_bytes, False),
    "cw64": _QueueKind(WgradItem, WGRAD_GROUP_MAX, "wgrad3x3_c64_grouped", None, (2, 2), _wgrad3x3_bytes, False),
}


class _PendingGrads:
    __slots__ = ("stream", "items", "flops", "keep")

    def __init__(self, stream):
        self.stream = stream
        self.clear()

    def clear(self):
        self.items, self.flops, self.keep = {k: [] for k in _QUEUE_KINDS}, dict.fromkeys(_QUEUE_KINDS, 0.0), []

    def push(self, kind, item, keep, flops=0.0):
        self.items[kind].append(item)
        self.keep += keep
        self.flops[kind] += flops
        if _QUEUE_KINDS[kind].flush_when_full and len(self.items[kind]) >= _QUEUE_KINDS[kind].group_max:
            self.flush((kind,))

    def flush(self, kinds=None):
        cur = torch.cuda.current_stream()
        if cur.cuda_stream != self.stream.cuda_stream:
            for t in self.keep:
                t.record_stream(cur)
        for kind in (_QUEUE_KINDS if kinds is None else kinds):
            k, items = _QUEUE_KINDS[kind], self.items[kind]
            if not items:
                continue
            ev = KERNEL_TIMER.start() if k.timer_key is not None else None
            for i in range(0, len(items), k.group_max):
                chunk = items[i:i + k.group_max]
                getattr(lib, k.launcher)(*(() if k.dtype is None else (k.dtype(),)), (k.item * len(chunk))(*chunk), len(chunk), rt.stream())
            if ev is not None:
                KERNEL_TIMER.stop(ev, k.timer_key, self.flops[kind], sum(k.abytes(it) for it in items))
            self.items[kind], self.flops[kind] = [], 0.0
        if not any(self.items.values()):
            self.keep = []


class _BackwardPass:
    __slots__ = ("task", "queues", "prep", "ln2", "pos", "bn_ready")

    def __init__(self, task):
        self.task = task
        self.queues = {}
        self.prep = {}
        self.ln2 = {}
        self.pos = {}
        self.bn_ready = {}

    def pending(self):
        st = torch.cuda.current_stream()
        q = self.queues.get(st.cuda_stream)
        if q is None:
            q = self.queues[st.cuda_stream] = _PendingGrads(st)
        return q


_PASS = None


def _pass():
    global _PASS
    task = torch._C._current_graph_task_id()
    if task == -1:
        return None
    if _PASS is None or _PASS.task != task:
        _PASS = _BackwardPass(task)
        torch.autograd.Variable._execution_engine.queue_callback(_flush_at_end)
    return _PASS


def _in_backward():
    return DEFER_WGRAD and torch._C._current_graph_task_id() != -1


def reset_backward_state():
    global _PASS
    _PASS = None


def flush_param_grads(all_streams=False):
    if _PASS is None:
        return
    if all_streams:
        for q in list(_PASS.queues.values()):
            q.flush()
        return
    q = _PASS.queues.get(torch.cuda.current_stream().cuda_stream)
    if q is not None:
        q.flush()


def _flush_at_end():
    global _PASS
    flush_param_grads(all_streams=True)
    _PASS = None


def gemm_tn(P, Q, O, M, I, J, *, ldp=None, q_rows=None, q_mode=ROWS_PLAIN, q_f32=False, ldo=None, dtype=None, p_colsum=None, side=False):
    if q_rows is None:
        q_rows = rows_plain(J)
    if side and q_mode == ROWS_PLAIN and q_f32 and dtype is None and rt.compute_dtype() == "bf16" and _in_backward() and Q.dim() == 2 and Q.dtype == torch.float32:
        Qb = empty((Q.shape[0], J), rt.act_dtype(), Q)
        lib.cast_rows(rt.dt(), Q.data_ptr(), q_rows.ld, Qb.data_ptr(), J, Q.shape[0], J, rt.stream())
        Q, q_f32, q_rows = Qb, False, rows_plain(J, q_rows.rows_out, q_rows.rows_in, q_rows.step)
    if side and q_mode == ROWS_PLAIN and not q_f32 and dtype is None and rt.compute_dtype() == "bf16" and _in_backward():
        it = TnItem()
        it.P, it.Q, it.O, it.p_colsum = P.data_ptr(), Q.data_ptr(), O.data_ptr(), _p(p_colsum)
        it.ldp, it.ldq, it.ldo, it.M, it.I, it.J = (I if ldp is None else ldp), q_rows.ld, (J if ldo is None else ldo), M, I, J
        it.q_rows_out, it.q_rows_in, it.q_step = q_rows.rows_out, q_rows.rows_in, q_rows.step
        if lib.raw("avec_gemm_tn_grouped_ok")(BF16, _byref(it)) and _chunk_readable(P, it.ldp, I, M) and _chunk_readable(Q, it.ldq, J, M):
            _pass().pending().push("tn", it, [P, Q], 2.0 * M * I * J)
            return
    ev = KERNEL_TIMER.start()
    st = rt.stream()
    if side and not KERNEL_TIMER.enabled:
        sd = rt.wgrad_fork(P, Q)
        st = st if sd is None else sd.cuda_stream
    lib.gemm_tn_bias(rt.dt() if dtype is None else dtype, P.data_ptr(), I if ldp is None else ldp, Q.data_ptr(), _byref(q_rows), q_mode,
                     int(q_f32), O.data_ptr(), J if ldo is None else ldo, _p(p_colsum), M, I, J, st)
    KERNEL_TIMER.stop(ev, (1, q_mode), 2.0 * M * I * J, (M * I + M * J) * 2.0 + I * J * 4.0)


def layernorm_fwd(x, w, b, M, D, out_f32, eps):
    y = empty((M, D), torch.float32 if out_f32 else rt.act_dtype(), x)
    mean = empty((M,), torch.float32, x)
    rstd = empty((M,), torch.float32, x)
    lib.layernorm_fwd(rt.dt(), x.data_ptr(), w.data_ptr(), b.data_ptr(), y.data_ptr(), int(out_f32), mean.data_ptr(), rstd.data_ptr(), M, D, eps,
                      rt.stream())
    return y, mean, rstd


def _tag_prep(out, alpha, drop_p, sid):
    out._avec_prep = (float(alpha), float(drop_p), int(sid))
    return out


def _prep_request(x):
    return getattr(x, "_avec_prep", None)


def _take_prep(dy, M, N, alpha, drop_p, sid):
    p = _pass()
    r = None if p is None else p.prep.pop(dy.data_ptr(), None)
    if r is not None and r[1:] == (M, N, float(alpha), float(drop_p), int(sid)) and r[0].dtype == rt.act_dtype():
        return r[0]
    return None


def layernorm_bwd(dy, dy_f32, x, mean, rstd, w, b, M, D, dres=None, prep=None):
    dx = empty((M, D), torch.float32, x)
    gw, gb = grad_of(w), grad_of(b)
    if D <= 1024 and D % 4 == 0 and _in_backward():
        if prep is not None:
            pt = empty((M, D), rt.act_dtype(), x)
            alpha, drop_p, sid = prep
            lib.layernorm_bwd_prep(rt.dt(), dy.data_ptr(), int(dy_f32), x.data_ptr(), mean.data_ptr(), rstd.data_ptr(), w.data_ptr(), dx.data_ptr(), _p(dres),
                                   pt.data_ptr(), alpha, drop_p, _rng(x.device, drop_p), sid, M, D, rt.stream())
            _pass().prep[dx.data_ptr()] = (pt, M, D, alpha, drop_p, sid)
        else:
            lib.layernorm_bwd(rt.dt(), dy.data_ptr(), int(dy_f32), x.data_ptr(), mean.data_ptr(), rstd.data_ptr(), w.data_ptr(), dx.data_ptr(), _p(dres),
                              None, None, M, D, rt.stream())
        defer_ln_param_grads(dy, dy_f32, x, mean, rstd, w, b, M, D)
        return dx
    lib.layernorm_bwd(rt.dt(), dy.data_ptr(), int(dy_f32), x.data_ptr(), mean.data_ptr(), rstd.data_ptr(), w.data_ptr(), dx.data_ptr(), _p(dres),
                      gw.data_ptr(), gb.data_ptr(), M, D, rt.stream())
    return dx


def layernorm_bwd_pair(dy2, x2, mean2, rstd2, w2, b2, dres2, x1, mean1, rstd1, w1, req1, ctx1, M, D):
    dx2, dx1 = empty((M, D), torch.float32, x2), empty((M, D), torch.float32, x2)
    pt, alpha, drop_p, sid = None, 1.0, 0.0, 0
    if req1 is not None:
        pt = empty((M, D), rt.act_dtype(), x2)
        alpha, drop_p, sid = req1
        _pass().prep[dx1.data_ptr()] = (pt, M, D, alpha, drop_p, sid)
    lib.layernorm_bwd2(rt.dt(), dy2.data_ptr(), x2.data_ptr(), mean2.data_ptr(), rstd2.data_ptr(), w2.data_ptr(), dres2.data_ptr(), dx2.data_ptr(),
                       x1.data_ptr(), mean1.data_ptr(), rstd1.data_ptr(), w1.data_ptr(), dx1.data_ptr(), _p(pt), alpha, drop_p, _rng(x2.device, drop_p), sid, M, D,
                       rt.stream())
    _pass().ln2[dx2.data_ptr()] = (dx1, ctx1, dx2, dx2._version)
    defer_ln_param_grads(dy2, False, x2, mean2, rstd2, w2, b2, M, D)
    return dx2


def grad_prep(dout, M, N, alpha=1.0, drop_p=0.0, sid=0, dbias=None):
    dacc = empty((M, N), rt.act_dtype(), dout)
    lib.grad_prep(rt.dt(), dout.data_ptr(), N, dacc.data_ptr(), alpha, drop_p, _rng(dout.device, drop_p), sid, _p(dbias), M, N, rt.stream())
    return dacc


def colsum(x, ld, out, M, N):
    lib.colsum(rt.dt(), x.data_ptr(), ld, out.data_ptr(), M, N, rt.stream())


def _f32c(t):
    return t if (t.dtype == torch.float32 and t.is_contiguous()) else t.float().contiguous()




def linear_fwd(x2d, weight, bias, M, *, in_f32, out_f32, act=ACT_NONE, out_pre=None, drop_p=0.0, sid=0, res=None, alpha=1.0,
               rows=None, K=None):
    sh = rt.shadow(weight)
    N, Kw = sh.A, sh.Tm * sh.C
    out = empty((M, N), torch.float32 if out_f32 else rt.act_dtype(), x2d)
    ent = fp8.entry(weight, Kw) if (rows is None and not in_f32 and sh.group is None) else None
    if ent is not None and ent.N == N:
        return gemm_nt_fp8(x2d, ent, out, M, N, Kw, bias=bias, act=act, out_pre=out_pre, drop_p=drop_p, sid=sid, res=res, alpha=alpha, out_f32=out_f32)
    gemm_nt(x2d, sh.fwd, out, M, N, Kw, rows=rows, a_f32=in_f32, bias=bias, act=act, out_pre=out_pre, drop_p=drop_p, sid=sid,
            res=res, alpha=alpha, out_f32=out_f32)
    return out


def linear_bwd_weight(dacc, x2d, weight, M, *, q_f32=False, q_rows=None, ldp=None, bias=None):
    sh = rt.shadow(weight)
    gemm_tn(dacc, x2d, grad_of(weight), M, sh.A, sh.Tm * sh.C, q_f32=q_f32, q_rows=q_rows, ldp=ldp, p_colsum=None if bias is None else grad_of(bias), side=True)


def linear_bwd_input(dacc, weight, M, *, out_f32, res=None, res_act=False, dact_z=None, dact=0, drop_p=0.0, sid=0, colsum_to=None, lda=None, out=None):
    sh = rt.shadow(weight)
    N, K = sh.Tm * sh.C, sh.A
    if out is None:
        out = empty((M, N), torch.float32 if out_f32 else rt.act_dtype(), dacc)
    gemm_nt(dacc, sh.bwd, out, M, N, K, rows=rows_plain(K if lda is None else lda), ldw=sh.ldb, res=res, res_act=res_act, dact_z=dact_z, dact=dact,
            drop_p=drop_p, sid=sid, colsum=colsum_to, out_f32=out_f32)
    return out


class LinearFn(torch.autograd.Function):

    @staticmethod
    def forward(ctx, x, weight, bias, in_f32, out_f32):
        rt.require_gpu(x)
        shp = x.shape
        x2 = x.reshape(-1, shp[-1])
        x2 = x2 if x2.is_contiguous() else x2.contiguous()
        M = x2.shape[0]
        y = linear_fwd(x2, weight, bias, M, in_f32=in_f32, out_f32=out_f32)
        ctx.saved = (x2, weight, bias, in_f32, out_f32, M, shp)
        return y.view(*shp[:-1], y.shape[-1])

    @staticmethod
    def backward(ctx, dy):
        x2, weight, bias, in_f32, out_f32, M, shp = ctx.saved
        N = weight.shape[0]
        dy = dy.reshape(M, N)
        dy = dy if dy.is_contiguous() else dy.contiguous()
        dacc = grad_prep(dy, M, N) if out_f32 else dy
        linear_bwd_weight(dacc, x2, weight, M, q_f32=in_f32, bias=bias)
        dx = None
        if ctx.needs_input_grad[0]:
            dx = linear_bwd_input(dacc, weight, M, out_f32=in_f32).view(shp)
        return dx, None, None, None, None


def linear(x, weight, bias, out_f32=True):
    if rt.compute_dtype() == "f32":
        return LinearFn.apply(x.float(), weight, bias, False, True)
    if x.dtype == torch.float32:
        return LinearFn.apply(x, weight, bias, True, out_f32)
    return LinearFn.apply(x.to(rt.act_dtype()), weight, bias, False, out_f32)


LN_PAIR = True


class LayerNormFn(torch.autograd.Function):

    @staticmethod
    def forward(ctx, x, w, b, eps, nxt=None):
        rt.require_gpu(x)
        shp = x.shape
        pair = None
        x2 = _f32c(x.reshape(-1, shp[-1]))
        M, D = x2.shape
        if nxt is not None and LN_PAIR and D <= 512 and D % 4 == 0:
            w2, b2, eps2 = nxt
            y, mean, rstd = empty((M, D), torch.float32, x2), empty((M,), torch.float32, x2), empty((M,), torch.float32, x2)
            h2, mean2, rstd2 = empty((M, D), rt.act_dtype(), x2), empty((M,), torch.float32, x2), empty((M,), torch.float32, x2)
            lib.layernorm_fwd2(rt.dt(), x2.data_ptr(), w.data_ptr(), b.data_ptr(), eps, y.data_ptr(), mean.data_ptr(), rstd.data_ptr(),
                               w2.data_ptr(), b2.data_ptr(), eps2, h2.data_ptr(), mean2.data_ptr(), rstd2.data_ptr(), M, D, rt.stream())
            pair = (h2, mean2, rstd2, w2.data_ptr(), float(eps2), M, D, ctx)
        else:
            y, mean, rstd = layernorm_fwd(x2, w, b, M, D, True, eps)
        ctx.saved = (x2, mean, rstd, w, b, M, D, shp, _prep_request(x))
        out = y.view(shp)
        if pair is not None:
            out._avec_ln2 = pair
        return out

    @staticmethod
    def backward(ctx, dy):
        x2, mean, rstd, w, b, M, D, shp, req = ctx.saved
        p = _pass()
        if p is not None:
            r = p.ln2.pop(dy.data_ptr(), None)
            if r is not None and r[1] is ctx and dy.dtype == torch.float32 and dy.is_contiguous() and (dy is r[2] or dy._base is r[2]) and r[2]._version == r[3]:
                defer_ln_param_grads(dy.reshape(M, D), True, x2, mean, rstd, w, b, M, D)
                return r[0].view(shp), None, None, None, None
        dx = layernorm_bwd(_f32c(dy.reshape(M, D)), True, x2, mean, rstd, w, b, M, D, prep=req)
        return dx.view(shp), None, None, None, None


class ActivationFn(torch.autograd.Function):

    @staticmethod
    def forward(ctx, x, act, dim):
        rt.require_gpu(x)
        assert act in (1, 2, 3)
        assert act != 3 or dim in (-1, x.dim() - 1), "GLU over the last axis"
        x2 = _f32c(x)
        C = x2.shape[-1] // 2 if act == 3 else x2.shape[-1]
        assert act != 3 or x2.shape[-1] == 2 * C, "GLU needs an even last axis"
        rows = x2.numel() // x2.shape[-1]
        y = torch.empty(x2.shape[:-1] + (C,), dtype=torch.float32, device=x2.device)
        lib.act_f32(act, x2.data_ptr(), None, y.data_ptr(), rows, C, 0, rt.stream())
        ctx.saved = (x2, act, rows, C)
        return y.to(x.dtype) if x.dtype != torch.float32 else y

    @staticmethod
    def backward(ctx, dy):
        x2, act, rows, C = ctx.saved
        dyc = _f32c(dy)
        dx = torch.empty_like(x2)
        lib.act_f32(act, x2.data_ptr(), dyc.data_ptr(), dx.data_ptr(), rows, C, 1, rt.stream())
        return dx, None, None


class DropoutFn(torch.autograd.Function):
    @staticmethod
    def forward(ctx, x, p, sid):
        x = _f32c(x)
        y = torch.empty_like(x)
        lib.dropout_f32(x.data_ptr(), y.data_ptr(), p, _rng(x.device), sid, x.numel(), rt.stream())
        ctx.saved = (p, sid)
        return y

    @staticmethod
    def backward(ctx, dy):
        p, sid = ctx.saved
        dy = _f32c(dy)
        dx = torch.empty_like(dy)
        lib.dropout_f32(dy.data_ptr(), dx.data_ptr(), p, _rng(dy.device), sid, dy.numel(), rt.stream())
        return dx, None, None


def defer_ln_param_grads(dy, dy_f32, x, mean, rstd, w, b, M, D):
    it = LnItem()
    it.dy, it.x, it.mean, it.rstd, it.dgamma, it.dbeta = dy.data_ptr(), x.data_ptr(), mean.data_ptr(), rstd.data_ptr(), grad_of(w).data_ptr(), grad_of(b).data_ptr()
    it.M, it.D, it.dy_f32 = M, D, int(dy_f32)
    if _in_backward() and D % 4 == 0 and D <= 1024:
        _pass().pending().push("ln", it, [dy, x, mean, rstd])
    else:
        lib.layernorm_param_grads_grouped(rt.dt(), (LnItem * 1)(it), 1, rt.stream())


class FeedForwardFn(torch.autograd.Function):
    @staticmethod
    def forward(ctx, x, ln_w, ln_b, w1, b1, w2, b2, eps, alpha, drop_p, sid1, sid2):
        rt.require_gpu(x)
        shp = x.shape
        x2 = _f32c(x.reshape(-1, shp[-1]))
        M, D = x2.shape
        F = w1.shape[0]
        adt = rt.act_dtype()
        ln_prev = None
        pre = getattr(x, "_avec_ln2", None)
        if pre is not None and pre[3] == ln_w.data_ptr() and pre[4] == float(eps) and pre[5:7] == (M, D) and x2.data_ptr() == x.data_ptr() and pre[0].dtype == adt:
            h0, mean, rstd = pre[0], pre[1], pre[2]
            ln_prev = pre[7]
        else:
            h0, mean, rstd = layernorm_fwd(x2, ln_w, ln_b, M, D, False, eps)
        z = empty((M, F), adt, x2)
        h1 = linear_fwd(h0, w1, b1, M, in_f32=False, out_f32=False, act=ACT_SWISH, out_pre=z, drop_p=drop_p, sid=sid1)
        y = linear_fwd(h1, w2, b2, M, in_f32=False, out_f32=True, drop_p=drop_p, sid=sid2, res=x2, alpha=alpha)
        ctx.saved = (x2, mean, rstd, h0, z, h1, ln_w, ln_b, w1, b1, w2, b2, alpha, drop_p, sid1, sid2, M, D, F, shp)
        ctx.prep_req = _prep_request(x)
        ctx.ln_prev = ln_prev
        return _tag_prep(y.view(shp), alpha, drop_p, sid2)

    @staticmethod
    def backward(ctx, dy):
        x2, mean, rstd, h0, z, h1, ln_w, ln_b, w1, b1, w2, b2, alpha, drop_p, sid1, sid2, M, D, F, shp = ctx.saved
        dy = _f32c(dy.reshape(M, D))
        dacc = _take_prep(dy, M, D, alpha, drop_p, sid2)
        if dacc is None:
            dacc = grad_prep(dy, M, D, alpha=alpha, drop_p=drop_p, sid=sid2)
        linear_bwd_weight(dacc, h1, w2, M, bias=b2)
        dz = linear_bwd_input(dacc, w2, M, out_f32=False, dact_z=z, dact=ACT_SWISH, drop_p=drop_p, sid=sid1)
        linear_bwd_weight(dz, h0, w1, M, bias=b1)
        dh0 = linear_bwd_input(dz, w1, M, out_f32=False)
        pv = ctx.ln_prev
        if pv is not None and _in_backward() and D <= 512 and D % 4 == 0 and dh0.dtype == rt.act_dtype():
            x1, mean1, rstd1, w1n, b1n, M1, D1, shp1, req1 = pv.saved
            if (M1, D1) == (M, D):
                return (layernorm_bwd_pair(dh0, x2, mean, rstd, ln_w, ln_b, dy, x1, mean1, rstd1, w1n, req1, pv, M, D).view(shp),) + (None,) * 11
        dx = layernorm_bwd(dh0, False, x2, mean, rstd, ln_w, ln_b, M, D, dres=dy, prep=ctx.prep_req)
        return (dx.view(shp),) + (None,) * 11


_PE_CACHE = {}


def rel_pos_table(T, D, device):
    key = (T, D, str(device), rt.compute_dtype())
    if key not in _PE_CACHE:
        pos = torch.arange(T - 1, -T, -1, dtype=torch.float32).unsqueeze(1)
        inv = 10000 ** (2 * torch.arange(0, D // 2, dtype=torch.float32).unsqueeze(0) / D)
        ang = pos / inv
        pe = torch.zeros(2 * T - 1, D)
        pe[:, 0::2] = ang.sin()
        pe[:, 1::2] = ang.cos()
        _PE_CACHE[key] = pe.to(device=device, dtype=rt.act_dtype()).contiguous()
    return _PE_CACHE[key]


def _attn_args(qkv, e, lens, len_div, mask, o, lse, B, H, T, d, D, q_full=0, *, kv=None, Tk=0, scale=None):
    a = Attn()
    a.q_full = q_full
    if kv is None:
        esz = qkv.element_size()
        a.q, a.k, a.v, a.ld = qkv.data_ptr(), qkv.data_ptr() + D * esz, qkv.data_ptr() + 2 * D * esz, 3 * D
    else:
        a.q, a.k, a.v, a.ld = qkv.data_ptr(), kv[0].data_ptr(), kv[1].data_ptr(), kv[2]
    a.e, a.lde = e.data_ptr(), (e.stride(0) if e.dim() == 2 else D)
    a.lens, a.len_div = _p(lens), len_div
    if mask is not None:
        a.mask, a.mask_bstride = mask.data_ptr(), (T * (Tk or T) if mask.shape[0] > 1 else 0)
    a.o, a.ldo, a.lse = o.data_ptr(), D, lse.data_ptr()
    a.B, a.H, a.T, a.d, a.scale, a.Tk = B, H, T, d, (1.0 / d ** 0.5 if scale is None else scale), Tk
    return a


def _pad8(n):
    return (n + 7) // 8 * 8


def _attn_backward(a, do, dq, dsrel, de=None, products=False, one_launch=False):
    B, H, T, d = a.B, a.H, a.T, a.d
    D, esz = H * d, do.element_size()
    a.dout = do.data_ptr()
    a.dq, a.lddq = dq.data_ptr(), dq.stride(0)
    if products:
        a.dk, a.dv, a.ldd = a.dq + D * esz, a.dq + 2 * D * esz, a.lddq
        a.de, a.ldde = de.data_ptr(), de.stride(0)
    Tld = _pad8(a.Tk or T)
    scratch = empty((2, B * H, T, Tld), do.dtype, do)
    a.pbuf, a.dsbuf, a.ldt = scratch.data_ptr(), scratch.data_ptr() + scratch[0].numel() * esz, Tld
    a.dsrel, a.ldr = dsrel.data_ptr(), dsrel.shape[2]
    lib.relpos_attention_bwd(rt.dt(), _byref(a), rt.stream())
    if not products:
# ... 185 lines not shown
            dea = empty((2 * Tp - 1, D), adt, dy)
            lib.cast_rows(rt.dt(), de.data_ptr(), D, dea.data_ptr(), D, 2 * Tp - 1, D, rt.stream())
            linear_bwd_weight(dea, pe, wp, 2 * Tp - 1, bias=bp)
        if patch > 1:
            dh = empty((M, D), adt, dy)
            lib.patch_pool_bwd(rt.dt(), dhp.data_ptr(), dh.data_ptr(), B, T, D, patch, rt.stream())
        else:
            dh = dhp
        if ln_w is not None:
            dx = layernorm_bwd(dh, False, x2, mean, rstd, ln_w, ln_b, M, D, dres=dy if residual else None, prep=ctx.prep_req)
        else:
            dx = dy.clone() if residual else torch.zeros_like(dy)
            lib.to_f32_rows(rt.dt(), dh.data_ptr(), D, dx.data_ptr(), D, M, D, 1, rt.stream())
        return (dx.view(B, T, D),) + (None,) * 20


class RelPosCoreFn(torch.autograd.Function):

    @staticmethod
    def forward(ctx, qkv, e, lens, len_div, mask, B, H, T, d, scale):
        rt.require_gpu(qkv)
        D, adt = H * d, rt.act_dtype()
        assert qkv.dtype == adt and e.dtype == adt and qkv.is_contiguous() and e.is_contiguous() and qkv.shape == (B * T, 3 * D) and e.shape == (2 * T - 1, D)
        assert d % 2 == 0, "the batched-GEMM backward needs an even head width (pad the operands)"
        if mask is not None:
            mask = mask.reshape(mask.shape[0], T, T).float().contiguous()
        o = empty((B * T, D), adt, qkv)
        lse = empty((B * H, T, 2), torch.float32, qkv)
        a = _attn_args(qkv, e, lens, len_div, mask, o, lse, B, H, T, d, D, scale=scale)
        lib.relpos_attention_fwd(rt.dt(), _byref(a), rt.stream())
        ctx.saved = (qkv, e, o, lse, lens, len_div, mask, B, H, T, d, scale)
        return o

    @staticmethod
    def backward(ctx, do):
        qkv, e, o, lse, lens, len_div, mask, B, H, T, d, scale = ctx.saved
        D, adt = H * d, rt.act_dtype()
        do = do.to(adt).contiguous()
        dqkv = empty((B * T, 3 * D), adt, do)
        de = torch.zeros((2 * T - 1, D), dtype=torch.float32, device=do.device)
        a = _attn_args(qkv, e, lens, len_div, mask, o, lse, B, H, T, d, D, scale=scale)
        dsrel = torch.zeros((H, B * T, _pad8(2 * T - 1)), dtype=adt, device=do.device)
        _attn_backward(a, do, dqkv, dsrel, de, products=True)
        return dqkv, de.to(adt), None, None, None, None, None, None, None, None


def relpos_core_infer(q, k, v, e, lens, mask, B, H, T, Tk, d, scale, want_probs=False):
    rt.require_gpu(q)
    D, adt = H * d, rt.act_dtype()
    for t in (q, k, v, e):
        assert t.dtype == adt and t.is_contiguous()
    assert q.shape == (B * T, D) and k.shape == (B * Tk, D) and v.shape == (B * Tk, D) and e.shape == (Tk + T - 1, D)
    if mask is not None:
        mask = mask.reshape(mask.shape[0], T, Tk).float().contiguous()
    o = empty((B * T, D), adt, q)
    lse = empty((B * H, T, 2), torch.float32, q)
    a = _attn_args(q, e, lens, 1, mask, o, lse, B, H, T, d, D, kv=(k, v, D), Tk=Tk, scale=scale)
    lib.relpos_attention_fwd(rt.dt(), _byref(a), rt.stream())
    if not want_probs:
        return o, None
    dq = empty((B * T, D), adt, q)
    zero = torch.zeros((B * T, D), dtype=adt, device=q.device)
    dsrel = torch.zeros((H, B * T, _pad8(Tk + T - 1)), dtype=adt, device=q.device)
    scratch = _attn_backward(a, zero, dq, dsrel)
    return o, scratch[0].view(B, H, T, -1)[..., :Tk].float()


def _pool_mask(mask, T, P):
    pad = (P - T % P) % P
    m = torch.nn.functional.pad(mask.reshape(mask.shape[0], 1, T, T).float(), (0, pad, 0, pad), value=0.0)
    Tp = (T + pad) // P
    return m.reshape(m.shape[0], Tp, P, Tp, P).amin(dim=(2, 4))


class BNState:

    NREP = 64

    def __init__(self, C, ref):
        self.stats = rt.zeros_scratch(self.NREP * 2 * C, ref.device)
        self.red = None
        self.ss = torch.empty(4 * C, dtype=torch.float32, device=ref.device)
        self.C = C


RELU_BITMASK = True
def bn_finalize(bn, st, count, training):
    C = st.C
    cptr = None
    sptr, nrep = st.stats.data_ptr(), st.NREP
    if training and rt.sync_batchnorm():
        st.red = rt.sync_bn_stats(st.stats, st.NREP, C, count, key=(id(bn), "f"))
        sptr, nrep, cptr = st.red.data_ptr(), 1, st.red.data_ptr() + 2 * C * 4
    lib.bn_finalize(sptr, nrep, cptr, float(count), bn.weight.data_ptr(), bn.bias.data_ptr(), *_bn_running(bn, training), bn.eps, st.ss.data_ptr(), C, int(training),
                    rt.stream())
    return cptr


def _bn_running(bn, training):
    track = bn.track_running_stats and bn.running_mean is not None
    return (bn.running_mean.data_ptr() if track else None, bn.running_var.data_ptr() if track else None,
            bn.num_batches_tracked.data_ptr() if (track and training) else None, bn.momentum if bn.momentum is not None else 0.1)


def bn_backward(bn, st, cptr, count, dout, y, out, act, M, want_dres=False, pre=None, mask=None):
    C = st.C
    adt = rt.act_dtype()
    dstats = rt.zeros_scratch(2 * C, dout.device)
    if pre is not None:
        lib.bn_bwd_finalize(pre.stats.data_ptr(), BNState.NREP, st.ss.data_ptr(), dstats.data_ptr(), C, rt.stream())
        act, out, want_dres, mask = ACT_NONE, None, False, None
    elif mask is not None:
        lib.bn_bwd_reduce_mask(rt.dt(), dout.data_ptr(), y.data_ptr(), mask.data_ptr(), st.ss.data_ptr(), dstats.data_ptr(), M, C, rt.stream())
    else:
        lib.bn_bwd_reduce(rt.dt(), dout.data_ptr(), y.data_ptr(), _p(out), st.ss.data_ptr(), act, dstats.data_ptr(), M, C, rt.stream())
    dstats, gw, gb = _bn_sync_grads(bn, dstats, C)
    dy = empty((M, C), adt, dout)
    dres = empty((M, C), adt, dout) if want_dres else None
    if mask is not None:
        lib.bn_bwd_apply_mask(rt.dt(), dout.data_ptr(), y.data_ptr(), mask.data_ptr(), st.ss.data_ptr(), bn.weight.data_ptr(), dstats.data_ptr(), cptr, float(count),
                              dy.data_ptr(), _p(dres), _p(gw), _p(gb), M, C, rt.stream())
    else:
        lib.bn_bwd_apply(rt.dt(), dout.data_ptr(), y.data_ptr(), _p(out), st.ss.data_ptr(), bn.weight.data_ptr(), dstats.data_ptr(), cptr, float(count), act,
                         dy.data_ptr(), _p(dres), _p(gw), _p(gb), M, C, rt.stream())
    return dy, (dout if pre is not None else dres)


def _add_local_affine_grads(dstats, gw, gb, C, key):
    if not rt.sync_batchnorm():
        return dstats, False
    from . import peer
    px = peer.active()
    if px is not None and dstats.is_cuda and dstats.is_contiguous() :
        return px.all_reduce_sum_fused(dstats, 1, 2 * C, None, key, dgamma=gw, dbeta=gb, C=C), True
    lib.bn_affine_grads(dstats.data_ptr(), gw.data_ptr(), gb.data_ptr(), C, rt.stream())
    return rt.all_reduce_small(dstats, key), True


def _bn_sync_grads(bn, dstats, C):
    gw, gb = grad_of(bn.weight), grad_of(bn.bias)
    dstats, synced = _add_local_affine_grads(dstats, gw, gb, C, (id(bn), "b"))
    return (dstats, None, None) if synced else (dstats, gw, gb)


def dw_pad_left(conv):
    K = conv.kernel_size[0]
    kind = getattr(conv, "padding_type", "same")
    if kind == "causal":
        return K - 1
    assert kind == "same", "the fused convolution module supports 'same' and 'causal' padding, got %r" % (kind,)
    return K // 2

CONVMOD_BN_FUSE = True


class ConvModuleFn(torch.autograd.Function):
    @staticmethod
    def forward(ctx, x, _anchor, mod, res_conv, drop_p, sid, training):
        rt.require_gpu(x)
        B, T, D = x.shape
        ln, pw1, dw, bn, pw2 = mod.layers[0], mod.layers[1], mod.layers[3], mod.layers[4], mod.layers[6]
        Dp, K, stride = dw.weight.shape[0], dw.weight.shape[2], dw.stride[0]
        To = (T - 1) // stride + 1
        M, Mo, adt = B * T, B * To, rt.act_dtype()
        x2 = _f32c(x.reshape(M, D))
        h, mean, rstd = layernorm_fwd(x2, ln.weight, ln.bias, M, D, False, ln.eps)
        u = linear_fwd(h, pw1.weight, pw1.bias, M, in_f32=False, out_f32=False)
        c = empty((Mo, Dp), adt, x2)
        st = BNState(Dp, x2)
        use_batch = training and not getattr(bn, "frozen", False)
        if use_batch and not rt.sync_batchnorm() and CONVMOD_BN_FUSE:
            lib.glu_dwconv_fwd_bn(rt.dt(), u.data_ptr(), dw.weight.data_ptr(), _p(dw.bias), c.data_ptr(), st.stats.data_ptr(), B, T, Dp, K, stride, dw_pad_left(dw),
                                  bn.weight.data_ptr(), bn.bias.data_ptr(), *_bn_running(bn, use_batch), bn.eps, st.ss.data_ptr(), rt.stream())
            cptr = None
        else:
            lib.glu_dwconv_fwd(rt.dt(), u.data_ptr(), dw.weight.data_ptr(), _p(dw.bias), c.data_ptr(), st.stats.data_ptr() if use_batch else None,
                               B, T, Dp, K, stride, dw_pad_left(dw), rt.stream())
            cptr = bn_finalize(bn, st, Mo, use_batch)
        a = empty((Mo, Dp), adt, x2)
        lib.bn_apply_fwd(rt.dt(), c.data_ptr(), st.ss.data_ptr(), None, ACT_SWISH, a.data_ptr(), Mo, Dp, rt.stream())
        if res_conv is not None:
            rs = res_conv.stride[0]
            R = linear_fwd(x2, res_conv.weight, res_conv.bias, Mo, in_f32=(adt != torch.float32), out_f32=True,
                           rows=rows_plain(D, To, T, rs) if rs > 1 else None)
        else:
            R = x2
        y = linear_fwd(a, pw2.weight, pw2.bias, Mo, in_f32=False, out_f32=True, drop_p=drop_p, sid=sid, res=R, alpha=1.0)
        ctx.saved = (x2, mean, rstd, h, u, c, a, st, cptr, use_batch, mod, res_conv, drop_p, sid, B, T, To, D, Dp, K, stride)
        ctx.prep_req = _prep_request(x)
        return _tag_prep(y.view(B, To, Dp), 1.0, drop_p, sid)

    @staticmethod
    def backward(ctx, dy):
        x2, mean, rstd, h, u, c, a, st, cptr, use_batch, mod, res_conv, drop_p, sid, B, T, To, D, Dp, K, stride = ctx.saved
        ln, pw1, dw, bn, pw2 = mod.layers[0], mod.layers[1], mod.layers[3], mod.layers[4], mod.layers[6]
        M, Mo, adt = B * T, B * To, rt.act_dtype()
        dy = _f32c(dy.reshape(Mo, Dp))
        dacc = _take_prep(dy, Mo, Dp, 1.0, drop_p, sid)
        if dacc is None:
            dacc = grad_prep(dy, Mo, Dp, drop_p=drop_p, sid=sid)
        linear_bwd_weight(dacc, a, pw2.weight, Mo, bias=pw2.bias)
        da = linear_bwd_input(dacc, pw2.weight, Mo, out_f32=False)
        du = empty((M, 2 * Dp), adt, dy)
        if use_batch and CONVMOD_BN_FUSE and stride == 1 and not rt.sync_batchnorm():
            dstats = rt.zeros_scratch(2 * Dp, da.device)
            lib.bn_bwd_reduce(rt.dt(), da.data_ptr(), c.data_ptr(), None, st.ss.data_ptr(), ACT_SWISH, dstats.data_ptr(), Mo, Dp, rt.stream())
            lib.dwconv_glu_bwd_bn(rt.dt(), da.data_ptr(), c.data_ptr(), st.ss.data_ptr(), bn.weight.data_ptr(), dstats.data_ptr(), float(Mo), u.data_ptr(), dw.weight.data_ptr(),
                                  du.data_ptr(), grad_of(dw.weight).data_ptr(), None if dw.bias is None else grad_of(dw.bias).data_ptr(),
                                  grad_of(bn.weight).data_ptr(), grad_of(bn.bias).data_ptr(), B, T, Dp, K, dw_pad_left(dw), rt.stream())
        else:
            if use_batch:
                dc, _ = bn_backward(bn, st, cptr, Mo, da, c, None, ACT_SWISH, Mo)
            else:
                dc = _bn_eval_backward(bn, st, da, c, ACT_SWISH, Mo)
            lib.dwconv_glu_bwd(rt.dt(), dc.data_ptr(), u.data_ptr(), dw.weight.data_ptr(), du.data_ptr(), grad_of(dw.weight).data_ptr(),
                               None if dw.bias is None else grad_of(dw.bias).data_ptr(), B, T, Dp, K, stride, dw_pad_left(dw), rt.stream())
        linear_bwd_weight(du, h, pw1.weight, M, bias=pw1.bias)
        dh = linear_bwd_input(du, pw1.weight, M, out_f32=False)
        if res_conv is None:
            dx = layernorm_bwd(dh, False, x2, mean, rstd, ln.weight, ln.bias, M, D, dres=dy, prep=ctx.prep_req)
        else:
            rs = res_conv.stride[0]
            dx = layernorm_bwd(dh, False, x2, mean, rstd, ln.weight, ln.bias, M, D)
            dracc = grad_prep(dy, Mo, Dp)
            linear_bwd_weight(dracc, x2, res_conv.weight, Mo, q_f32=(adt != torch.float32), q_rows=rows_plain(D, To, T, rs) if rs > 1 else None, bias=res_conv.bias)
            dxr = linear_bwd_input(dracc, res_conv.weight, Mo, out_f32=True)
            lib.strided_rows_add(dx.data_ptr(), dxr.data_ptr(), B, T, To, D, rs, rt.stream())
        return dx.view(B, T, D), None, None, None, None, None, None


def _bn_eval_backward(bn, st, dout, y, act, M, out=None):
    C = st.C
    dstats = torch.zeros(2 * C, dtype=torch.float32, device=dout.device)
    dstats2 = torch.zeros(2 * C, dtype=torch.float32, device=dout.device)
    lib.bn_bwd_reduce(rt.dt(), dout.data_ptr(), y.data_ptr(), _p(out), st.ss.data_ptr(), act, dstats2.data_ptr(), M, C, rt.stream())
    dy = empty((M, C), rt.act_dtype(), dout)
    lib.bn_bwd_apply(rt.dt(), dout.data_ptr(), y.data_ptr(), _p(out), st.ss.data_ptr(), bn.weight.data_ptr(), dstats.data_ptr(), None, 1.0, act,
                     dy.data_ptr(), None, None, None, M, C, rt.stream())
    grad_of(bn.weight).add_(dstats2[C:])
    grad_of(bn.bias).add_(dstats2[:C])
    return dy


class InterCTCFn(torch.autograd.Function):
    @staticmethod
    def forward(ctx, x, w1, b1, w2, b2):
        rt.require_gpu(x)
        B, T, D = x.shape
        M, V = B * T, w1.shape[0]
        x2 = _f32c(x.reshape(M, D))
        conv = rt.act_dtype() != torch.float32
        logits = linear_fwd(x2, w1, b1, M, in_f32=conv, out_f32=True)
        probs = empty((M, V), rt.act_dtype(), x2)
        lib.softmax_fwd(rt.dt(), logits.data_ptr(), probs.data_ptr(), M, V, rt.stream())
        y = linear_fwd(probs, w2, b2, M, in_f32=False, out_f32=True, res=x2, alpha=1.0)
        ctx.saved = (x2, logits, probs, w1, b1, w2, b2, B, T, D, V, conv)
        return y.view(B, T, D), logits.view(B, T, V)

    @staticmethod
    def backward(ctx, dy, dlogits_ext):
        x2, logits, probs, w1, b1, w2, b2, B, T, D, V, conv = ctx.saved
        M = B * T
        dy = _f32c(dy.reshape(M, D))
        dacc = grad_prep(dy, M, D)
        linear_bwd_weight(dacc, probs, w2, M, bias=b2)
        dprobs = linear_bwd_input(dacc, w2, M, out_f32=False)
        dl = empty((M, V), torch.float32, dy)
        dext = None if dlogits_ext is None else _f32c(dlogits_ext.reshape(M, V))
        lib.softmax_bwd(rt.dt(), dprobs.data_ptr(), logits.data_ptr(), dl.data_ptr(), _p(dext), M, V, rt.stream())
        dla = grad_prep(dl, M, V)
        linear_bwd_weight(dla, x2, w1, M, q_f32=conv, bias=b1)
        dx = linear_bwd_input(dla, w1, M, out_f32=True, res=dy)
        return dx.view(B, T, D), None, None, None, None


class FusionFn(torch.autograd.Function):
    @staticmethod
    def forward(ctx, a, v, w1, b1, w2, b2):
        rt.require_gpu(a)
        B, T, Da = a.shape
        Dv = v.shape[-1]
        M, F, adt = B * T, w1.shape[0], rt.act_dtype()
        a2, v2 = _f32c(a.reshape(M, Da)), _f32c(v.reshape(M, Dv))
        xc = empty((M, Da + Dv), adt, a2)
        lib.cast_rows(rt.dt(), a2.data_ptr(), Da, xc.data_ptr(), Da + Dv, M, Da, rt.stream())
        lib.cast_rows(rt.dt(), v2.data_ptr(), Dv, xc.data_ptr() + Da * xc.element_size(), Da + Dv, M, Dv, rt.stream())
        z = empty((M, F), adt, a2)
        h = linear_fwd(xc, w1, b1, M, in_f32=False, out_f32=False, act=ACT_SWISH, out_pre=z)
        y = linear_fwd(h, w2, b2, M, in_f32=False, out_f32=True)
        ctx.saved = (xc, z, h, w1, b1, w2, b2, B, T, Da, Dv, F)
        return y.view(B, T, -1)

    @staticmethod
    def backward(ctx, dy):
        xc, z, h, w1, b1, w2, b2, B, T, Da, Dv, F = ctx.saved
        M, N = B * T, w2.shape[0]
        dy = _f32c(dy.reshape(M, N))
        dacc = grad_prep(dy, M, N)
        linear_bwd_weight(dacc, h, w2, M, bias=b2)
        dz = linear_bwd_input(dacc, w2, M, out_f32=False, dact_z=z, dact=ACT_SWISH)
        linear_bwd_weight(dz, xc, w1, M, bias=b1)
        sh = rt.shadow(w1)
        da = empty((M, Da), torch.float32, dy)
        dv = empty((M, Dv), torch.float32, dy)
        gemm_nt(dz, sh.bwd, da, M, Da, F, out_f32=True)
        gemm_nt(dz, sh.bwd[Da * F:], dv, M, Dv, F, out_f32=True)
        return da.view(B, T, Da), dv.view(B, T, Dv), None, None, None, None


class CTCLossFn(torch.autograd.Function):
    @staticmethod
    def forward(ctx, logits, logit_len, targets, target_len, blank, zero_infinity):
        rt.require_gpu(logits)
        B, T, V = logits.shape
        lg = _f32c(logits)
        tg = targets.to(device=lg.device, dtype=torch.int64).contiguous()
        if tg.dim() == 1:
            tg = tg.view(B, -1)
        Lmax = tg.shape[1]
        il = logit_len.to(device=lg.device, dtype=torch.int64).contiguous()
        tl = target_len.to(device=lg.device, dtype=torch.int64).contiguous()
        nll = empty((B,), torch.float32, lg)
        mean = torch.zeros((), dtype=torch.float32, device=lg.device)
        need_grad = ctx.needs_input_grad[0]
        grad = empty((B, T, V), torch.float32, lg) if need_grad else None
        ws = empty((lib.raw("avec_ctc_workspace_floats")(B, T, max(Lmax, 1)),), torch.float32, lg)
        lib.ctc_loss(lg.data_ptr(), il.data_ptr(), tg.data_ptr(), tl.data_ptr(), nll.data_ptr(), mean.data_ptr(), _p(grad), ws.data_ptr(),
                     B, T, V, Lmax, blank, int(zero_infinity), rt.stream())
        ctx.saved = (grad, B)
        ctx.nll = nll
        return mean

    @staticmethod
    def backward(ctx, dloss):
        grad, B = ctx.saved
        out = torch.empty_like(grad)
        dl = dloss.float().contiguous()
        lib.scale_by_scalar(grad.data_ptr(), dl.data_ptr(), 1.0 / B, out.data_ptr(), grad.numel(), rt.stream())
        return out, None, None, None, None, None


class CTCLossMultiFn(torch.autograd.Function):

    @staticmethod
    def forward(ctx, blank, zero_infinity, targets, target_len, weights, *flat):
        n = len(flat) // 2
        logits, lens = [_f32c(t) for t in flat[0::2]], flat[1::2]
        rt.require_gpu(logits[0])
        B, _, V = logits[0].shape
        dev = logits[0].device
        tg = targets.to(device=dev, dtype=torch.int64).contiguous()
        if tg.dim() == 1:
            tg = tg.view(B, -1)
        Lmax = tg.shape[1]
        tl = target_len.to(device=dev, dtype=torch.int64).contiguous()
        ils = [l.to(device=dev, dtype=torch.int64).contiguous() for l in lens]
        nll = torch.empty((n, B), dtype=torch.float32, device=dev)
        means = rt.zeros_scratch(n + 1, dev)
        grads = [empty(tuple(lg.shape), torch.float32, lg) if ctx.needs_input_grad[5 + 2 * i] else None for i, lg in enumerate(logits)]
        arr_p = lambda ptrs: (ctypes.c_void_p * n)(*ptrs)
        Ts = (ctypes.c_int * n)(*[lg.shape[1] for lg in logits])
        lib.ctc_loss_multi(n, arr_p([lg.data_ptr() for lg in logits]), arr_p([l.data_ptr() for l in ils]), Ts, arr_p([nll[i].data_ptr() for i in range(n)]),
                           arr_p([means[i:].data_ptr() for i in range(n)]), arr_p([g.data_ptr() if g is not None else None for g in grads]),
                           tg.data_ptr(), tl.data_ptr(), (ctypes.c_float * n)(*[float(x) for x in weights]), means[n:].data_ptr(), B, V, Lmax, blank, int(zero_infinity), rt.stream())
        total = means[n]
        ctx.set_materialize_grads(False)
        ctx.saved = (grads, B, n, [float(x) for x in weights])
        ctx.keep = (logits, ils, tg, tl, nll)
        outs = tuple(means[i] for i in range(n))
# ... 981 lines not shown
```

include/avec_hip.h:

```cpp
#ifndef AVEC_HIP_H
#define AVEC_HIP_H
#include <stdint.h>
#ifdef __HIPCC__
#include <hip/hip_runtime.h>
#else
typedef struct ihipStream_t* hipStream_t;
#endif
#ifdef __cplusplus
extern "C" {
#endif

#define AVEC_F32 0
#define AVEC_BF16 1
#define AVEC_ABI_VERSION 4
#define AVEC_STAT_REPLICAS 64

int avec_version(void);
int avec_struct_size(int which);
const char* avec_last_error(void);
const char* avec_last_kernel(void);
int avec_set_reduce_workspace(void* base, long long bytes);
int avec_set_reduce_workspace_stream(void* base, long long bytes, hipStream_t stream);

enum { AVEC_ROWS_PLAIN = 0, AVEC_ROWS_CONV_FWD = 1, AVEC_ROWS_CONV_BWD = 2 };
typedef struct avec_rows {
  long long ld;
  int rows_out, rows_in, step;
  int H, W, C, KH, KW, stride, pad, OH, OW;
  int T3;
} avec_rows_t;

typedef struct avec_epilogue {
  void* out; long long ldo; int out_f32;
  void* out_pre; long long ldpre;
  const float* bias;
  int act;
  float drop_p; const unsigned long long* rng; unsigned rng_stream;
  const void* res; long long ldres; float alpha; int res_act;
  const void* dact_z; long long ldz; int dact;
  float* colsum;
  float* stats;
  const void* bnb_y; long long ldby; const float* bnb_ss; int bnb_mask;
  int res_cls0;
  const unsigned char* res_mask;
} avec_epilogue_t;

int avec_gemm_nt(int dtype, const void* A, const avec_rows_t* a_rows, int a_mode, int a_f32,
                 const void* W, long long ldw, long long M, int N, int K,
                 const avec_epilogue_t* ep, hipStream_t stream);

typedef struct { const float* src; void* dst; long long n; int slot; int K, Kp; int reserved; } avec_fp8_item_t;
int avec_fp8_quantize(int src_dtype, const void* x, long long ldx, void* q, long long ldq, long long M, int K, float* amax, int compute_amax, hipStream_t stream);
int avec_fp8_weights_refresh(const avec_fp8_item_t* table, int n_items, int blocks_per_item, float* amax, hipStream_t stream);
int avec_gemm_nt_fp8(const void* A, long long lda, const void* W, long long ldw, long long M, int N, int K,
                     const float* amax_a, const float* amax_w, const avec_epilogue_t* ep, hipStream_t stream);


int avec_gemm_tn(int dtype, const void* P, long long ldp, const void* Q, const avec_rows_t* q_rows, int q_mode, int q_f32,
                 float* O, long long ldo, long long M, int I, int J, hipStream_t stream);
int avec_gemm_tn_bias(int dtype, const void* P, long long ldp, const void* Q, const avec_rows_t* q_rows, int q_mode, int q_f32,
                      float* O, long long ldo, float* p_colsum, long long M, int I, int J, hipStream_t stream);
#define AVEC_TN_GROUP_MAX 32
typedef struct avec_tn_item {
  const void* P; const void* Q; float* O; float* p_colsum;
  long long ldp, ldq, ldo, M;
  int I, J;
  int q_rows_out, q_rows_in, q_step;
  int reserved;
} avec_tn_item_t;
int avec_gemm_tn_grouped_ok(int dtype, const avec_tn_item_t* item);
int avec_gemm_tn_grouped(int dtype, const avec_tn_item_t* items, int n, hipStream_t stream);
int avec_gemm_tn_batched(int dtype, const void* P, long long ldp, const void* Q, long long ldq, float* O, long long ldo, long long M, int I, int J,
                         int nb_outer, int nb_inner, const long long* strides6, hipStream_t stream);
int avec_gemm_tn_batched_store(int dtype, const void* P, long long ldp, const void* Q, long long ldq, void* O_act, long long ldo, long long M, int I, int J,
                               int nb_outer, int nb_inner, const long long* strides6, hipStream_t stream);

typedef struct {
  const void* P; long long ldp; const void* Q; long long ldq;
  float* O; void* O_act; long long ldo;
  long long M; int I, J, nb_outer, nb_inner;
  const long long* strides6;
} avec_tn_batched_t;
int avec_gemm_tn_batched_multi(int dtype, const avec_tn_batched_t* items, int n, hipStream_t stream);

#define AVEC_PEER_MAX_WORLD 8
int avec_peer_exchange_sum(const float* in, float* out, int n, void* const* pages, long long page_stride_granules, int rank, int world,
                           unsigned* epoch, int* err_flag, int timeout_ms, hipStream_t stream);
int avec_peer_exchange_sum_fused(const float* in, int n_replicas, int n_in, int has_tail, float tail, float* dgamma, float* dbeta, int C, float* out,
                                 void* const* pages, long long page_stride_granules, int rank, int world, unsigned* epoch, int* err_flag, int timeout_ms,
                                 hipStream_t stream);
int avec_enable_peer_access(int peer_device);
int avec_peer_buffer_alloc(void** ptr, long long bytes, void* ipc_handle_64b);
int avec_peer_buffer_open(const void* ipc_handle_64b, void** ptr);
int avec_peer_buffer_close(void* ptr);
int avec_peer_buffer_free(void* ptr);

int avec_layernorm_fwd(int dtype, const float* x, const float* gamma, const float* beta, void* y, int y_f32,
                       float* mean, float* rstd, long long M, int D, float eps, hipStream_t stream);
int avec_layernorm_bwd(int dtype, const void* dy, int dy_f32, const float* x, const float* mean, const float* rstd, const float* gamma,
                       float* dx, const float* dres, float* dgamma, float* dbeta, long long M, int D, hipStream_t stream);
int avec_layernorm_bwd_prep(int dtype, const void* dy, int dy_f32, const float* x, const float* mean, const float* rstd, const float* gamma,
                            float* dx, const float* dres, void* prep, float prep_alpha, float prep_drop_p, const unsigned long long* rng, unsigned rng_stream,
                            long long M, int D, hipStream_t stream);
int avec_layernorm_fwd2(int dtype, const float* x, const float* gamma1, const float* beta1, float eps1, float* y1, float* mean1, float* rstd1,
                        const float* gamma2, const float* beta2, float eps2, void* h2, float* mean2, float* rstd2, long long M, int D, hipStream_t stream);
int avec_layernorm_bwd2(int dtype, const void* dy2, const float* x2, const float* mean2, const float* rstd2, const float* gamma2, const float* dres2, float* dx2,
                        const float* x1, const float* mean1, const float* rstd1, const float* gamma1, float* dx1,
                        void* prep, float prep_alpha, float prep_drop_p, const unsigned long long* rng, unsigned rng_stream, long long M, int D, hipStream_t stream);
#define AVEC_LN_GROUP_MAX 40
typedef struct avec_ln_item {
  const void* dy; const float* x; const float* mean; const float* rstd; float* dgamma; float* dbeta;
  long long M; int D; int dy_f32;
} avec_ln_item_t;
int avec_layernorm_param_grads_grouped(int dtype, const avec_ln_item_t* items, int n, hipStream_t stream);
int avec_grad_prep(int dtype, const float* dout, long long ld, void* dacc, float alpha, float drop_p, const unsigned long long* rng,
                   unsigned rng_stream, float* dbias, long long M, int N, hipStream_t stream);
int avec_colsum(int dtype, const void* x, long long ld, float* out, long long M, int N, hipStream_t stream);
int avec_strided_rows_add(float* dx, const float* src, int B, int T, int To, int D, int step, hipStream_t stream);
int avec_bn_stats(int dtype, const void* y, float* stats, long long M, int C, hipStream_t stream);
int avec_bn_collapse(const float* stats, int n_replicas, float count, float* out, int C, hipStream_t stream);
int avec_bn_affine_grads(const float* dstats, float* dgamma, float* dbeta, int C, hipStream_t stream);
int avec_bn_finalize(const float* stats, int n_replicas, const float* count_ptr, float count, const float* gamma, const float* beta, float* running_mean,
                     float* running_var, long long* num_batches_tracked, float momentum, float eps, float* ss, int C, int training, hipStream_t stream);
int avec_stamp(unsigned long long* out, int slot, hipStream_t stream);
int avec_bn_bwd_finalize(const float* stats, int n_replicas, const float* ss, float* dstats, int C, hipStream_t stream);
int avec_bn_apply_fwd(int dtype, const void* y, const float* ss, const void* residual, int act, void* out, long long M, int C, hipStream_t stream);
int avec_bn_bwd_reduce(int dtype, const void* dout, const void* y, const void* out, const float* ss, int act, float* dstats, long long M, int C, hipStream_t stream);
int avec_bn_bwd_apply(int dtype, const void* dout, const void* y, const void* out, const float* ss, const float* gamma, const float* dstats,
                      const float* count_ptr, float count, int act, void* dy, void* dres, float* dgamma, float* dbeta, long long M, int C, hipStream_t stream);
int avec_bn_apply_fwd_mask(int dtype, const void* y, const float* ss, const void* residual, const float* residual_ss, void* out, unsigned char* mask, long long M, int C,
                           hipStream_t stream);
int avec_bn_bwd_reduce_mask(int dtype, const void* dout, const void* y, const unsigned char* mask, const float* ss, float* dstats, long long M, int C, hipStream_t stream);
int avec_bn_bwd_apply_mask(int dtype, const void* dout, const void* y, const unsigned char* mask, const float* ss, const float* gamma, const float* dstats,
                           const float* count_ptr, float count, void* dy, void* dres, float* dgamma, float* dbeta, long long M, int C, hipStream_t stream);
int avec_softmax_fwd(int dtype, const float* logits, void* probs, long long M, int V, hipStream_t stream);
int avec_softmax_bwd(int dtype, const void* dprobs, const float* logits, float* dlogits, const float* dadd, long long M, int V, hipStream_t stream);
int avec_cast_rows(int dtype, const float* src, long long ld_src, void* dst, long long ld_dst, long long M, int N, hipStream_t stream);
int avec_to_f32_rows(int dtype, const void* src, long long ld_src, float* dst, long long ld_dst, long long M, int N, int accum, hipStream_t stream);
int avec_act_f32(int act, const float* x, const float* dy, float* out, long long rows, int C, int backward, hipStream_t stream);
int avec_dropout_f32(const float* x, float* y, float p, const unsigned long long* rng, unsigned rng_stream, long long n, hipStream_t stream);
int avec_maxpool_hw_fwd(int dtype, const void* x, void* out, unsigned char* idx, long long frames, int H, int W, int C, int KH, int KW, int SH, int SW,
                        int pad0_h, int pad0_w, int pad1_h, int pad1_w, hipStream_t stream);
int avec_maxpool_hw_bwd(int dtype, const void* dy, const unsigned char* idx, void* dx, long long frames, int H, int W, int C, int KH, int KW, int SH, int SW,
                        int pad0_h, int pad0_w, int pad1_h, int pad1_w, hipStream_t stream);
int avec_upsample_rows(int dtype, const void* src, void* dst, long long B, int T, int D, int P, int backward, hipStream_t stream);
int avec_patch_pool_fwd(int dtype, const void* x, void* y, int B, int T, int D, int P, hipStream_t stream);
int avec_patch_pool_bwd(int dtype, const void* dy, void* dx, int B, int T, int D, int P, hipStream_t stream);
int avec_patch_unpool_add(int dtype, const void* o, const float* res, float* out, float drop_p, const unsigned long long* rng, unsigned rng_stream,
                          int B, int T, int D, int P, hipStream_t stream);
int avec_patch_unpool_bwd(int dtype, const float* dout, void* dob, float drop_p, const unsigned long long* rng, unsigned rng_stream,
                          int B, int T, int D, int P, hipStream_t stream);
int avec_avgpool_fwd(int dtype, const void* x, void* y, long long N, int HW, int C, hipStream_t stream);
int avec_avgpool_bwd(int dtype, const void* dy, void* dx, long long N, int HW, int C, hipStream_t stream);

int avec_glu_dwconv_fwd(int dtype, const void* u, const float* w, const float* bias, void* out, float* stats,
                        int B, int T, int C, int K, int stride, int pad_left, hipStream_t stream);
int avec_glu_dwconv_fwd_bn(int dtype, const void* u, const float* w, const float* bias, void* out, float* stats, int B, int T, int C, int K, int stride, int pad_left,
                           const float* gamma, const float* beta, float* running_mean, float* running_var, long long* num_batches_tracked, float momentum, float eps,
                           float* ss, hipStream_t stream);
int avec_dwconv_glu_bwd(int dtype, const void* dc, const void* u, const float* w, void* du, float* dw, float* dbias,
                        int B, int T, int C, int K, int stride, int pad_left, hipStream_t stream);
int avec_dwconv_glu_bwd_bn(int dtype, const void* da, const void* c, const float* ss, const float* gamma, const float* dstats, float count, const void* u, const float* w,
                           void* du, float* dw, float* dbias, float* dgamma, float* dbeta, int B, int T, int C, int K, int pad_left, hipStream_t stream);

typedef struct avec_attn {
  const void *q, *k, *v; long long ld;
  const void* e; long long lde;
  const long long* lens; int len_div;
  int q_full;
  const float* mask; long long mask_bstride;
  void* o; long long ldo; float* lse;
  const void* dout;
  void *dq, *dk, *dv; long long lddq, ldd;
  float* de; long long ldde;
  void *pbuf, *dsbuf; long long ldt;
  void* dsrel; long long ldr;
  int B, H, T, d; float scale;
  int Tk;
} avec_attn_t;
int avec_relpos_attention_fwd(int dtype, const avec_attn_t* args, hipStream_t stream);
int avec_relpos_attention_bwd(int dtype, const avec_attn_t* args, hipStream_t stream);

long long avec_glu_dwconv_stream_state_bytes(int dtype, int B, int C, int K);
int avec_glu_dwconv_stream(int dtype, const void* u, const float* w, const float* bias, const float* ss, void* out, void* state, long long state_bytes,
                           const long long* pos, const unsigned char* reset, const long long* chunk_len, int div, int B, int Tq, int C, int K, int stride, hipStream_t stream);
long long avec_relpos_attention_stream_state_bytes(int dtype, int B, int H, int d, int L, int Tq);
int avec_relpos_attention_stream(int dtype, const void* q, const void* k, const void* v, long long ld, const void* e, long long lde, void* kcache, void* vcache,
                                 long long cache_bytes, const long long* pos, const unsigned char* reset, const long long* chunk_len, int div, void* o, long long ldo,
                                 int B, int H, int Tq, int d, int L, float scale, hipStream_t stream);
int avec_stream_advance(long long* pos, unsigned char* reset, const long long* chunk_len, long long full, int B, hipStream_t stream);

int avec_stream_window(const float* x_new, const float* tail, float* X, const long long* pend, const long long* n_new, const unsigned char* last, const unsigned char* reset,
                       const unsigned char* ended, long long* nvalid, long long* ncommit, long long* emit, int B, int Tc, int LAe, int D, int S, hipStream_t stream);
int avec_stream_window_advance(const float* X, float* tail, long long* pend, long long* pos, const long long* nvalid, const long long* ncommit, unsigned char* last,
                               unsigned char* reset, unsigned char* ended, int B, int W, int LAe, int D, hipStream_t stream);
int avec_glu_dwconv_stream_la(int dtype, const void* u, const float* w, const float* bias, const float* ss, void* out, void* state, long long state_bytes,
                              const long long* pos, const unsigned char* reset, const long long* ncommit, int div, int B, int Wq, int C, int K, int stride, hipStream_t stream);
int avec_relpos_attention_stream_la(int dtype, const void* q, const void* k, const void* v, long long ld, const void* e, long long lde, void* kcache, void* vcache,
                                    long long cache_bytes, const long long* pos, const unsigned char* reset, const long long* nvalid, const long long* ncommit, int div,
                                    void* o, long long ldo, int B, int H, int Wq, int Tq, int d, int L, int R, float scale, hipStream_t stream);

long long avec_audio_stream_state_bytes(int B);
int avec_mel_frames_stream(const float* wave, long long ldw, const float* window, float* frames, const void* state, long long state_bytes,
                           const long long* n_samples, const unsigned char* reset, const unsigned char* last, long long* out_len, long long* meta,
                           int B, int W, int Tmax, int n_fft, int win, int hop, hipStream_t stream);
int avec_audio_stem_stream(int dtype, const float* mel, const float* w, const float* bias, const float* ss, void* out, const long long* out_len,
                           const long long* meta, int B, int n_mels, int Tmax, int C, hipStream_t stream);
int avec_audio_stream_advance(const float* wave, long long ldw, void* state, long long state_bytes, const long long* n_samples, unsigned char* reset,
                              unsigned char* last, int B, int W, int n_fft, int win, int hop, hipStream_t stream);

long long avec_video_stream_state_bytes(int dtype, int B, int H, int W);
int avec_video_stem_stream(int dtype, const float* chunk, long long ldc, const void* state, long long state_bytes, const long long* n_frames,
                           const unsigned char* reset, const unsigned char* last, const void* w8, const float* bias, const float* ss, void* out,
                           long long* out_len, int B, int Tin, int Tmax, int H, int W, hipStream_t stream);
int avec_video_stream_advance(int dtype, const float* chunk, long long ldc, void* state, long long state_bytes, const long long* n_frames, unsigned char* reset,
                              unsigned char* last, int B, int Tin, int H, int W, hipStream_t stream);

long long avec_av_fuse_stream_state_bytes(int dtype, int B, int Da, int Dv, int cap);
int avec_av_fuse_stream(int dtype, const float* a, const long long* a_len, const float* v, const long long* v_len, void* state, long long state_bytes,
                        unsigned char* reset, void* xc, long long* pair_len, int B, int Ra, int Rv, int Da, int Dv, int cap, int max_emit, hipStream_t stream);

int avec_mel_frames(const float* audio, const float* window, float* frames, int B, long long L, int n_fft, int win, int hop, hipStream_t stream);
int avec_mel_power_log(const float* spec, const float* fb, float* out, int B, int F, int n_bins, int n_mels, hipStream_t stream);
int avec_specaugment(float* mel, const long long* lens, int B, int n_mels, int F, int mF, int Fparam, int mT, float pS,
                     const unsigned long long* rng, unsigned rng_stream, hipStream_t stream);
int avec_debug_rng_uniform(const unsigned long long* rng, unsigned rng_stream, const long long* ids, int n, float* out, hipStream_t stream);
int avec_audio_stem_conv_fwd(int dtype, const float* mel, const float* w, const float* bias, void* y, float* stats, int B, int n_mels, int F, int C, hipStream_t stream);
int avec_audio_stem_act_fwd(int dtype, const void* y, const float* ss, void* a, int B, int n_mels, int F, int C, hipStream_t stream);
int avec_audio_stem_bwd(int dtype, const void* da, const void* y, const float* mel, const float* ss, const float* gamma, float* dstats,
                        const float* count_ptr, float count, int phase, float* dw, float* dbias, float* dgamma, float* dbeta,
                        int B, int n_mels, int F, int C, hipStream_t stream);
int avec_stem_im2col(int dtype, const float* video, void* A, long long clips, int T, int H, int W, int ldk, hipStream_t stream);
int avec_stem3d_supported(long long clips, int T, int H, int W);
int avec_stem3d_fwd(const float* video, const void* w_shadow, int ldw, const float* bias, void* y, float* stats, long long clips, int T, int H, int W, hipStream_t stream);
int avec_stem3d_wgrad(const float* video, const void* dy, float* dw, long long clips, int T, int H, int W, hipStream_t stream);
int avec_stem3p_supported(long long clips, int T, int H, int W);
int avec_stem3p_fwd(const void* video_bf16, const void* w_shadow, const float* bias, const float* gamma, void* zp, unsigned char* idx, float* stats,
                    long long clips, int T, int H, int W, hipStream_t stream);
int avec_stem3p_reduce(void* dpool, const void* zp, const float* ss, float* dstats, long long frames, int PH, int PW, hipStream_t stream);
int avec_stem3p_wgrad_supported(long long clips, int T, int H, int W);
int avec_stem3p_geom(long long clips, int T, int H, int W, int* out);
int avec_stem3p_wgrad(const void* video_bf16, const void* w_shadow, const float* bias, const void* dpool_masked, const unsigned char* idx, const float* ss,
                      const float* gamma, const float* dstats, const float* count_ptr, float count, float* dw, float* dgamma, float* dbeta,
                      long long clips, int T, int H, int W, hipStream_t stream);
int avec_stem3p_dz(const void* video_bf16, const void* w_shadow, const float* bias, const void* dpool_masked, const unsigned char* idx, const float* ss,
                   const float* gamma, const float* dstats, const float* count_ptr, float count, void* dz, float* dgamma, float* dbeta,
                   long long clips, int T, int H, int W, hipStream_t stream);
int avec_stem_pool_fwd(int dtype, const void* y, const float* ss, void* out, unsigned char* idx, void* ymax, long long frames, int H, int W, int C, hipStream_t stream);
int avec_stem_pool_bwd_reduce_pooled(int dtype, const void* dpool, const unsigned char* idx, const void* ymax, const float* ss, float* dstats,
                                     long long frames, int H, int W, int C, hipStream_t stream);
int avec_stem_pool_bwd(int dtype, const void* dpool, const unsigned char* idx, const void* y, const float* ss, const float* gamma, float* dstats,
                       const float* count_ptr, float count, int phase, void* dy, float* dgamma, float* dbeta, long long frames, int H, int W, int C, hipStream_t stream);

int avec_conv3x3_c64_supported(int H, int W, int Cin, int Cout, int KH, int KW, int stride);
int avec_conv3x3_c64(const void* x, const void* w, void* y, const void* res, float* stats, long long images, int H, int W, int flip, hipStream_t stream);
int avec_conv3x3_c64_res_masked(const void* x, const void* w, void* y, const void* res, const unsigned char* res_mask, long long images, int H, int W, int flip, hipStream_t stream);
int avec_wgrad3x3_c64(const void* x, const void* dy, float* dw, long long images, int H, int W, hipStream_t stream);
int avec_wgrad3x3_c128_supported(int H, int W, int Cin, int Cout, int KH, int KW, int stride);
int avec_wgrad3x3_c128(const void* x, const void* dy, float* dw, long long images, int C, int H, int W, hipStream_t stream);
#define AVEC_WGRAD_GROUP_MAX 16
typedef struct { const void* x; const void* dy; float* dw; long long images; int C, H, W, reserved; } avec_wgrad3x3_item_t;
int avec_wgrad3x3_c128_grouped(const avec_wgrad3x3_item_t* items, int n, hipStream_t stream);
int avec_wgrad3x3_c64_grouped(const avec_wgrad3x3_item_t* items, int n, hipStream_t stream);

int avec_video_input(const unsigned char* clips, const long long* clip_off, const int* geom, const int* masks, int max_masks, int channels, const float* lut, float mean, float stdv,
                     int mean_frame, float* out, float* frame_ws, int B, int Tout, int OH, int OW, hipStream_t stream);
int avec_video_tta_batch(const float* x, float* y, int B, long long rows, int W, int n, unsigned flip_mask, hipStream_t stream);

long long avec_ctc_workspace_floats(int B, int T, int Lmax);
int avec_ctc_loss(const float* logits, const long long* in_lens, const long long* targets, const long long* tgt_lens, float* nll, float* mean_out,
                  float* grad, float* workspace, int B, int T, int V, int Lmax, int blank, int zero_infinity, hipStream_t stream);
int avec_ctc_loss_multi_fits(int T, int V, int Lmax);
int avec_ctc_loss_multi(int n_heads, const float* const* logits, const long long* const* in_lens, const int* T, float* const* nll, float* const* mean_out, float* const* grad,
                        const long long* targets, const long long* tgt_lens, const float* weights, float* total, int B, int V, int Lmax, int blank, int zero_infinity, hipStream_t stream);
int avec_scale_by_scalar(const float* g, const float* scalar_dev, float mul, float* out, long long n, hipStream_t stream);
int avec_scale_by_scalar_multi(int n_tensors, const float* const* g, float* const* out, const long long* numel, const float* mul, const float* scalar_dev, hipStream_t stream);
int avec_softmax_ce(const float* logits, const long long* targets, long long ignore_index, float* loss, float* mean_out, float* grad, long long M, int V, hipStream_t stream);
int avec_len_affine(const long long* in, long long* out, int n, long long sub, long long div, long long add, hipStream_t stream);
int avec_argmax_rows(const float* x, long long* out, long long M, int V, hipStream_t stream);

typedef struct avec_ngram {
  int order;
  int V;
  const float* unigram;
  long long ctx_cap;
  const unsigned long long* ctx_key;
  const float* ctx_bo;
  const int* ctx_off;
  const int* ctx_cnt;
  const int* cont_tok;
  const float* cont_lp;
} avec_ngram_t;
long long avec_ctc_beam_workspace_bytes(int B, int T, int W);
int avec_ctc_beam_search(const float* logits, const long long* lengths, int B, int T, int V, int W, float inv_tmp, const avec_ngram_t* lm, float alpha, float beta,
                         float oov_logprob, void* workspace, long long workspace_bytes, int* tokens, int* out_len, float* score, float* ctc_logp, hipStream_t stream);
long long avec_ctc_beam_state_bytes(int B, int W);
int avec_ctc_beam_stream(const float* logits, const long long* chunk_len, const unsigned char* reset, int B, int Tc, int V, int W, int Tcap, float inv_tmp,
                         const avec_ngram_t* lm, float alpha, float beta, float oov_logprob, void* state, long long state_bytes, void* backptr, long long backptr_bytes,
                         int* tokens, int* out_len, float* score, float* ctc_logp, int* stable_len, int emit, hipStream_t stream);
int avec_ngram_rows(const avec_ngram_t* lm, const int* ctx, const int* ctx_len, int n, int max_len, float oov_logprob, float* rows, hipStream_t stream);
long long avec_ctc_align_workspace_bytes(int B, int T, int Lmax);
int avec_ctc_align_fits_lds(int T, int Lmax);
int avec_ctc_align(const float* logits, const long long* in_lens, const long long* targets, const long long* tgt_lens,
                   int B, int T, int V, int Lmax, int blank, int tier ,
                   void* workspace, long long workspace_bytes,
                   int* path, int* spans, float* score, float* token_logp, hipStream_t stream);
int avec_embed_pos(int dtype, const long long* ids, const float* E, const float* P, void* out, int out_f32, long long N, int L, int V, int D, hipStream_t stream);
int avec_causal_attention_supported(int d);
int avec_causal_attention(int dtype, const void* qkv, long long ld, const long long* lens, void* o, long long ldo, int N, int H, int L, int d, float scale, hipStream_t stream);
long long avec_lm_head_nll_workspace_bytes(long long R, int V, int D);
int avec_lm_head_nll(int dtype, const void* h, long long ldh, const void* W, long long ldw, const float* bias, const long long* tgt, float* nll, long long R, int V, int D,
                     void* workspace, long long workspace_bytes, hipStream_t stream);
int avec_lm_segment_sum(const float* nll, const long long* lens, long long S, int L, float* out, hipStream_t stream);
int avec_lm_rescore_select(const float* neural, const long long* lens, const float* beam_score, float alpha, float beta, int B, int K, float* total, long long* best,
                           hipStream_t stream);
int avec_ctc_tta_pick(const int* tokens, const int* out_len, const float* score, const long long* best_slot, int B, int n, int W, int T, long long* best_aug,
// ... 20 lines not shown
```

Baseline: 1880.

## Defer dwconv and layernorm column-reduction finalizes into one grouped launch

Backward depthwise-conv and layernorm kernels now write per-block partial sums into private buffers instead of each launching its own column-finalize. The finalizes are queued and later run as one grouped kernel that looks up its item by binary search and atomically adds into the gradient tensors. This cuts many small kernel launches per backward pass. In exchange it allocates extra partial buffers, adds atomics, and adds bookkeeping for deferred finalization. Layernorm arithmetic is pinned with fp-contract-off helpers to keep rounding consistent across the two paths.

```diff
diff --git a/avec_amd/csrc/api.hip b/avec_amd/csrc/api.hip
--- a/avec_amd/csrc/api.hip
+++ b/avec_amd/csrc/api.hip
@@ -22,7 +22,7 @@
   switch (which) {
     case 0: return (int)sizeof(avec_rows_t); case 1: return (int)sizeof(avec_epilogue_t); case 2: return (int)sizeof(avec_attn_t); case 3: return (int)sizeof(avec_tn_item_t);
     case 4: return (int)sizeof(avec_tn_batched_t); case 5: return (int)sizeof(avec_ln_item_t); case 6: return (int)sizeof(avec_fp8_item_t); case 7: return (int)sizeof(avec_wgrad3x3_item_t);
-    case 8: return (int)sizeof(avec_ngram_t);
+    case 8: return (int)sizeof(avec_ngram_t); case 9: return (int)sizeof(avec_fin_item_t);
     default: return -1;
   }
 }
diff --git a/avec_amd/csrc/convmod.hip b/avec_amd/csrc/convmod.hip
--- a/avec_amd/csrc/convmod.hip
+++ b/avec_amd/csrc/convmod.hip
@@ -320,28 +320,57 @@
   dst[KMAX] = dbias;
   return plan.finish(dst, C, st);
 }
+static inline ColPlan dw_plan(dim3 grid, int C, float* partial, hipStream_t st) {
+  return partial ? ColPlan{ColWs{partial}, grid.x, grid.y, KMAX + 1, 128} : ColPlan::grid<KMAX + 1>(grid, C, st);
+}
+static inline dim3 dw_bwd_grid(int B, int To, int C) { return dim3((unsigned)((C / 4 + 31) / 32), (unsigned)(B * ((To + DW_TT - 1) / DW_TT))); }
+extern "C" long long avec_dwconv_bwd_partial_floats(int B, int T_, int C, int stride) {
+  if (B <= 0 || T_ <= 0 || C <= 0 || stride <= 0) return 0;
+  const dim3 g = dw_bwd_grid(B, (T_ - 1) / stride + 1, C);
+  return (long long)g.x * g.y * (KMAX + 1) * 128;
+}
+extern "C" int avec_dwconv_bwd_fin_item(const float* partial, float* dw, float* dbias, int B, int T_, int C, int K, int stride, avec_fin_item_t* item) {
+  AVEC_CHECK_ARG(partial && dw && item && B > 0 && T_ > 0 && C > 0 && C % 4 == 0 && K > 0 && K <= KMAX && stride > 0, "dwconv_bwd_fin_item: bad arguments");
+  const dim3 g = dw_bwd_grid(B, (T_ - 1) / stride + 1, C);
+  item->partial = partial; item->colblocks = (int)g.x; item->nslots = (int)g.y; item->NV = KMAX + 1; item->W = 128; item->C = C; item->dstride = 1;
+  for (int k = 0; k < AVEC_FIN_MAXNV; ++k) item->dst[k] = k < K ? dw + (long long)k * C : nullptr;
+  item->dst[KMAX] = dbias;
+  return 0;
+}
+static int dwconv_glu_bwd_bn_impl(int dtype, const void* da, const void* c, const float* ss, const float* gamma, const float* dstats, float count, const void* u, const float* w,
+                                  void* du, float* dw, float* dbias, float* partial, float* dgamma, float* dbeta, int B, int T_, int C, int K, int pad_left, hipStream_t st) {
+  const int nchunks = (T_ + DW_TT - 1) / DW_TT;
+  const dim3 grid = dw_bwd_grid(B, T_, C); const ColPlan plan = dw_plan(grid, C, partial, st);
+  size_t l2 = (size_t)2 * (DW_TT - 1 + K) * 128 * sizeof(float);
+  if (l2 < (size_t)4 * (KMAX + 1) * 128 * sizeof(float)) l2 = (size_t)4 * (KMAX + 1) * 128 * sizeof(float);
+  AVEC_CHECK_ARG(l2 <= 64 * 1024, "dwconv_glu_bwd_bn: kernel size %d too large", K);
+  DwBnb bnb{c, ss, gamma, dstats, 1.f / count, dgamma, dbeta};
+  DISPATCH_T(dtype, hipLaunchKernelGGL(dwconv_glu_bwd_fused_kernel<T>, grid, dim3(256), l2, st, (const T*)da, (const T*)u, w, (T*)du, dw, dbias, B, T_, C, K, pad_left, nchunks, plan.ws, bnb));
+  AVEC_LAUNCH_CHECK();
+  return partial ? 0 : dw_finish(plan, dw, dbias, C, K, st);
+}
 extern "C" int avec_dwconv_glu_bwd_bn(int dtype, const void* da, const void* c, const float* ss, const float* gamma, const float* dstats, float count, const void* u, const float* w,
                                       void* du, float* dw, float* dbias, float* dgamma, float* dbeta, int B, int T_, int C, int K, int pad_left, hipStream_t st) {
   AVEC_CHECK_ARG(da && c && ss && gamma && dstats && count > 0.f && u && w && du && dw && B > 0 && T_ > 0 && C > 0 && C % 4 == 0 && K > 0 && K <= KMAX && pad_left >= 0 && pad_left < K,
                  "dwconv_glu_bwd_bn: bad arguments");
   AVEC_CHECK_ARG((dgamma == nullptr) == (dbeta == nullptr), "dwconv_glu_bwd_bn: dgamma and dbeta come together (both or neither)");
-  const int nchunks = (T_ + DW_TT - 1) / DW_TT;
-  dim3 grid((unsigned)((C / 4 + 31) / 32), (unsigned)(B * nchunks)); const ColPlan plan = ColPlan::grid<KMAX + 1>(grid, C, st);
-  size_t l2 = (size_t)2 * (DW_TT - 1 + K) * 128 * sizeof(float);
-  if (l2 < (size_t)4 * (KMAX + 1) * 128 * sizeof(float)) l2 = (size_t)4 * (KMAX + 1) * 128 * sizeof(float);
-  AVEC_CHECK_ARG(l2 <= 64 * 1024, "dwconv_glu_bwd_bn: kernel size %d too large", K);
-  DwBnb bnb{c, ss, gamma, dstats, 1.f / count, dgamma, dbeta};
-  DISPATCH_T(dtype, hipLaunchKernelGGL(dwconv_glu_bwd_fused_kernel<T>, grid, dim3(256), l2, st, (const T*)da, (const T*)u, w, (T*)du, dw, dbias, B, T_, C, K, pad_left, nchunks, plan.ws, bnb));
-  AVEC_LAUNCH_CHECK();
-  return dw_finish(plan, dw, dbias, C, K, st);
-}
-extern "C" int avec_dwconv_glu_bwd(int dtype, const void* dc, const void* u, const float* w, void* du, float* dw, float* dbias,
-                                   int B, int T_, int C, int K, int stride, int pad_left, hipStream_t st) {
-  AVEC_CHECK_ARG(dc && u && w && du && dw && B > 0 && T_ > 0 && C > 0 && C % 4 == 0 && K > 0 && K <= KMAX && stride > 0 && pad_left >= 0 && pad_left < K, "dwconv_glu_bwd: bad arguments");
+  return dwconv_glu_bwd_bn_impl(dtype, da, c, ss, gamma, dstats, count, u, w, du, dw, dbias, nullptr, dgamma, dbeta, B, T_, C, K, pad_left, st);
+}
+extern "C" int avec_dwconv_glu_bwd_bn_partials(int dtype, const void* da, const void* c, const float* ss, const float* gamma, const float* dstats, float count, const void* u, const float* w,
+                                               void* du, float* partial, long long partial_floats, float* dgamma, float* dbeta, int B, int T_, int C, int K, int pad_left, hipStream_t st) {
+  AVEC_CHECK_ARG(da && c && ss && gamma && dstats && count > 0.f && u && w && du && B > 0 && T_ > 0 && C > 0 && C % 4 == 0 && K > 0 && K <= KMAX && pad_left >= 0 && pad_left < K,
+                 "dwconv_glu_bwd_bn_partials: bad arguments");
+  AVEC_CHECK_ARG((dgamma == nullptr) == (dbeta == nullptr), "dwconv_glu_bwd_bn_partials: dgamma and dbeta come together (both or neither)");
+  AVEC_CHECK_ARG(partial && (((uintptr_t)partial) & 3) == 0 && partial_floats >= avec_dwconv_bwd_partial_floats(B, T_, C, 1),
+                 "dwconv_glu_bwd_bn_partials: partial rows of %lld floats, %lld needed (avec_dwconv_bwd_partial_floats)", partial_floats, avec_dwconv_bwd_partial_floats(B, T_, C, 1));
+  return dwconv_glu_bwd_bn_impl(dtype, da, c, ss, gamma, dstats, count, u, w, du, nullptr, nullptr, partial, dgamma, dbeta, B, T_, C, K, pad_left, st);
+}
+static int dwconv_glu_bwd_impl(int dtype, const void* dc, const void* u, const float* w, void* du, float* dw, float* dbias, float* partial,
+                               int B, int T_, int C, int K, int stride, int pad_left, hipStream_t st) {
   const int To = (T_ - 1) / stride + 1;
   long long n4 = (long long)B * T_ * (C / 4); long long nb = (n4 + 255) / 256; if (nb > 4096) nb = 4096;
   const int nchunks = (To + DW_TT - 1) / DW_TT;
-  dim3 grid((unsigned)((C / 4 + 31) / 32), (unsigned)(B * nchunks)); const ColPlan plan = ColPlan::grid<KMAX + 1>(grid, C, st);
+  const dim3 grid = dw_bwd_grid(B, To, C); const ColPlan plan = dw_plan(grid, C, partial, st);
   size_t lds = (size_t)((DW_TT - 1) * stride + K) * 128 * sizeof(float);
   if (lds < (size_t)4 * (KMAX + 1) * 128 * sizeof(float)) lds = (size_t)4 * (KMAX + 1) * 128 * sizeof(float);
   AVEC_CHECK_ARG(lds <= 64 * 1024, "dwconv_glu_bwd: stride %d too large", stride);
@@ -352,7 +381,19 @@
   DISPATCH_T(dtype, hipLaunchKernelGGL(dwconv_glu_bwd_input_kernel<T>, dim3((unsigned)nb), dim3(256), 0, st, (const T*)dc, (const T*)u, w, (T*)du, B, T_, C, K, stride, To, pad_left);
              hipLaunchKernelGGL(dwconv_bwd_weight_kernel<T>, grid, dim3(256), lds, st, (const T*)dc, (const T*)u, dw, dbias, B, T_, C, K, stride, To, pad_left, nchunks, plan.ws));
   AVEC_LAUNCH_CHECK();
-  return dw_finish(plan, dw, dbias, C, K, st);
+  return partial ? 0 : dw_finish(plan, dw, dbias, C, K, st);
+}
+extern "C" int avec_dwconv_glu_bwd(int dtype, const void* dc, const void* u, const float* w, void* du, float* dw, float* dbias,
+                                   int B, int T_, int C, int K, int stride, int pad_left, hipStream_t st) {
+  AVEC_CHECK_ARG(dc && u && w && du && dw && B > 0 && T_ > 0 && C > 0 && C % 4 == 0 && K > 0 && K <= KMAX && stride > 0 && pad_left >= 0 && pad_left < K, "dwconv_glu_bwd: bad arguments");
+  return dwconv_glu_bwd_impl(dtype, dc, u, w, du, dw, dbias, nullptr, B, T_, C, K, stride, pad_left, st);
+}
+extern "C" int avec_dwconv_glu_bwd_partials(int dtype, const void* dc, const void* u, const float* w, void* du, float* partial, long long partial_floats,
+                                            int B, int T_, int C, int K, int stride, int pad_left, hipStream_t st) {
+  AVEC_CHECK_ARG(dc && u && w && du && B > 0 && T_ > 0 && C > 0 && C % 4 == 0 && K > 0 && K <= KMAX && stride > 0 && pad_left >= 0 && pad_left < K, "dwconv_glu_bwd_partials: bad arguments");
+  AVEC_CHECK_ARG(partial && (((uintptr_t)partial) & 3) == 0 && partial_floats >= avec_dwconv_bwd_partial_floats(B, T_, C, stride),
+                 "dwconv_glu_bwd_partials: partial rows of %lld floats, %lld needed (avec_dwconv_bwd_partial_floats)", partial_floats, avec_dwconv_bwd_partial_floats(B, T_, C, stride));
+  return dwconv_glu_bwd_impl(dtype, dc, u, w, du, nullptr, nullptr, partial, B, T_, C, K, stride, pad_left, st);
 }
 
 template <typename T>
diff --git a/avec_amd/csrc/norm.hip b/avec_amd/csrc/norm.hip
--- a/avec_amd/csrc/norm.hip
+++ b/avec_amd/csrc/norm.hip
@@ -41,6 +41,73 @@
   dim3 grid((unsigned)((NV * W + 15) / 16), colblocks, (nslots + 127) / 128);
   hipLaunchKernelGGL(col_finalize_kernel, grid, dim3(256), 0, st, f);
   AVEC_LAUNCH_CHECK(); return 0;
+}
+
+static constexpr int FIN_POOL = 256;
+struct FinItem { const float* partial; int NV, W, C, nslots, dstride, colblocks, dst0, first; };
+struct FinGroup { FinItem it[AVEC_FIN_GROUP_MAX]; float* dst[FIN_POOL]; int n; };
+static_assert(sizeof(FinGroup) <= 4096, "the grouped finalize's work-list travels in the kernel argument block");
+__global__ __launch_bounds__(256) void col_finalize_grouped_kernel(FinGroup grp) {
+  __shared__ float red[16][17];
+  const int wg = blockIdx.x;
+  int lo = 0, hi = grp.n - 1;
+  while (lo < hi) { const int mid = (lo + hi + 1) >> 1; if (grp.it[mid].first <= wg) lo = mid; else hi = mid - 1; }
+  const FinItem& t = grp.it[lo];
+  const int tiles = (t.W + 15) >> 4, gx = t.NV * tiles;
+  int l = wg - t.first;
+  const int bx = l % gx; l /= gx;
+  const int cb = l % t.colblocks, s0 = (l / t.colblocks) * 128;
+  const int n = bx / tiles, w = (bx - n * tiles) * 16 + (threadIdx.x & 15);
+  const int cw = threadIdx.x & 15, sl = threadIdx.x >> 4;
+  const int ncols = t.NV * t.W, nslots = t.nslots;
+  float* const d = grp.dst[t.dst0 + n];
+  const bool live = w < t.W && d != nullptr;
+  float s = 0.f;
+  if (live) {
+    const float* p = t.partial + ((size_t)cb * nslots) * ncols + n * t.W + w;
+#pragma unroll
+    for (int k = 0; k < 8; ++k) {
+      const int si = s0 + sl + 16 * k; const int sc = si < nslots ? si : nslots - 1;
+      const float v = p[(size_t)sc * ncols];
+      s += si < nslots ? v : 0.f;
+    }
+  }
+  red[sl][cw] = s;
+  __syncthreads();
+  if (sl == 0 && live) {
+    float r = 0.f;
+#pragma unroll
+    for (int k = 0; k < 16; ++k) r += red[k][cw];
+    const int col = cb * t.W + w;
+    if (col < t.C) atomicAdd(d + (long long)col * t.dstride, r);
+  }
+}
+static int fin_grouped_launch(const FinGroup& grp, int total, hipStream_t st) {
+  hipLaunchKernelGGL(col_finalize_grouped_kernel, dim3((unsigned)total), dim3(256), 0, st, grp);
+  AVEC_LAUNCH_CHECK(); return 0;
+}
+extern "C" int avec_col_finalize_grouped(const avec_fin_item_t* items, int n, hipStream_t st) {
+  AVEC_CHECK_ARG(items && n > 0 && n <= AVEC_FIN_GROUP_MAX, "col_finalize_grouped: need 1..%d items (got %d)", AVEC_FIN_GROUP_MAX, n);
+  for (int k = 0; k < n; ++k) {
+    const avec_fin_item_t& s = items[k];
+    AVEC_CHECK_ARG(s.partial && s.NV >= 1 && s.NV <= AVEC_FIN_MAXNV && s.W > 0 && s.C > 0 && s.colblocks > 0 && s.nslots > 0 && s.dstride > 0,
+                   "col_finalize_grouped: item %d: null partial rows or bad geometry (NV=%d W=%d C=%d colblocks=%d nslots=%d dstride=%d)", k, s.NV, s.W, s.C, s.colblocks, s.nslots, s.dstride);
+    AVEC_CHECK_ARG((long long)s.colblocks * s.W >= s.C && (long long)(s.colblocks - 1) * s.W < s.C, "col_finalize_grouped: item %d: %d column blocks of %d do not tile C=%d", k, s.colblocks, s.W, s.C);
+    const long long wgs = (long long)s.NV * ((s.W + 15) / 16) * s.colblocks * ((s.nslots + 127) / 128);
+    AVEC_CHECK_ARG(wgs < (1ll << 24) && (long long)s.nslots * s.NV * s.W < (1ll << 31), "col_finalize_grouped: item %d too large", k);
+  }
+  FinGroup grp; grp.n = 0; int used = 0, total = 0;
+  for (int k = 0; k < n; ++k) {
+    const avec_fin_item_t& s = items[k];
+    if (used + s.NV > FIN_POOL) { if (int r = fin_grouped_launch(grp, total, st)) return r; grp.n = 0; used = 0; total = 0; }
+    FinItem& t = grp.it[grp.n++];
+    t.partial = s.partial; t.NV = s.NV; t.W = s.W; t.C = s.C; t.nslots = s.nslots; t.dstride = s.dstride; t.colblocks = s.colblocks; t.dst0 = used; t.first = total;
+    for (int i = 0; i < s.NV; ++i) grp.dst[used + i] = s.dst[i];
+    used += s.NV;
+    total += s.NV * ((s.W + 15) / 16) * s.colblocks * ((s.nslots + 127) / 128);
+  }
+  for (int i = used; i < FIN_POOL; ++i) grp.dst[i] = nullptr;
+  return fin_grouped_launch(grp, total, st);
 }
 
 template <typename TO>
@@ -140,12 +207,46 @@
 }
 
 struct LnPrep { void* out; float alpha, p; const unsigned long long* rng; unsigned stream; int f32; };
+__device__ __forceinline__ float ln_xhat(float x, float mu, float rs) {
+#pragma clang fp contract(off)
+  return (x - mu) * rs;
+}
+__device__ __forceinline__ float ln_mul(float a, float b) {
+#pragma clang fp contract(off)
+  return a * b;
+}
+__device__ __forceinline__ float ln_add(float a, float b) {
+#pragma clang fp contract(off)
+  return a + b;
+}
+__device__ __forceinline__ float ln_dx(float o, float rs, float t, float s1, float xh, float s2) {
+#pragma clang fp contract(off)
+  return __builtin_fmaf(rs, __builtin_fmaf(-xh, s2, t - s1), o);
+}
+template <int NG>
+__device__ __forceinline__ void ln_rows_exchange(float* lds, const float (&a)[NG][4], const float (&b)[NG][4], bool ok, int D, float* out) {
+  const int lane = threadIdx.x & 63; float* mine = lds + (threadIdx.x >> 6) * 2 * D;
+#pragma unroll
+  for (int i = 0; i < NG; ++i) {
+    const int c = lane * 4 + i * 256; if (c >= D) break;
+    *(float4*)(mine + c) = ok ? make_float4(a[i][0] * b[i][0], a[i][1] * b[i][1], a[i][2] * b[i][2], a[i][3] * b[i][3]) : make_float4(0.f, 0.f, 0.f, 0.f);
+    *(float4*)(mine + D + c) = ok ? make_float4(a[i][0], a[i][1], a[i][2], a[i][3]) : make_float4(0.f, 0.f, 0.f, 0.f);
+  }
+  __syncthreads();
+  for (int o = threadIdx.x * 4; o < 2 * D; o += 1024) {
+    const float4 p0 = *(const float4*)(lds + o), p1 = *(const float4*)(lds + 2 * D + o), p2 = *(const float4*)(lds + 4 * D + o), p3 = *(const float4*)(lds + 6 * D + o);
+    *(float4*)(out + o) = make_float4(((p0.x + p1.x) + p2.x) + p3.x, ((p0.y + p1.y) + p2.y) + p3.y, ((p0.z + p1.z) + p2.z) + p3.z, ((p0.w + p1.w) + p2.w) + p3.w);
+  }
+}
 template <typename TG, int NG>
 __global__ __launch_bounds__(256) void ln_bwd_rows_kernel(const TG* __restrict__ dy, const float* __restrict__ x, const float* __restrict__ mean,
                                                           const float* __restrict__ rstd, const float* __restrict__ g, float* __restrict__ dx,
-                                                          const float* __restrict__ dres, long long M, int D, LnPrep pr) {
-  const int lane = threadIdx.x & 63; const long long row = (long long)blockIdx.x * 4 + (threadIdx.x >> 6);
-  if (row >= M) return;
+                                                          const float* __restrict__ dres, long long M, int D, LnPrep pr, float* __restrict__ partial = nullptr) {
+  extern __shared__ __attribute__((aligned(16))) float lnx[];
+  const int lane = threadIdx.x & 63; const long long row0 = (long long)blockIdx.x * 4 + (threadIdx.x >> 6);
+  const bool ok = row0 < M, PART = partial != nullptr;
+  if (!PART && !ok) return;
+  const long long row = ok ? row0 : M - 1;
   const float mu = mean[row], rs = rstd[row];
   DropKey dk; dk.k0 = 0u; dk.thr = 0u; dk.scale = 1.f;
   if (pr.out) dk = drop_key(pr.rng, pr.stream, pr.p);
@@ -165,13 +266,14 @@
 #pragma unroll
   for (int i = 0; i < NG; ++i)
 #pragma unroll
-    for (int e = 0; e < 4; ++e) { const float xh = (v[i][e] - mu) * rs, t = d[i][e] * gg[i][e]; v[i][e] = xh; s1 += t; s2 += t * xh; }
+    for (int e = 0; e < 4; ++e) { const float xh = ln_xhat(v[i][e], mu, rs), t = ln_mul(d[i][e], gg[i][e]); v[i][e] = xh; s1 = ln_add(s1, t); s2 = __builtin_fmaf(t, xh, s2); }
   s1 = wave_sum(s1) / D; s2 = wave_sum(s2) / D;
 #pragma unroll
   for (int i = 0; i < NG; ++i) {
     const int c = lane * 4 + i * 256; if (c >= D) break;
 #pragma unroll
-    for (int e = 0; e < 4; ++e) o[i][e] += rs * (d[i][e] * gg[i][e] - s1 - v[i][e] * s2);
+    for (int e = 0; e < 4; ++e) o[i][e] = ln_dx(o[i][e], rs, ln_mul(d[i][e], gg[i][e]), s1, v[i][e], s2);
+    if (PART && !ok) continue;
     st4<float>(dx + row * D + c, o[i]);
     if (pr.out) {
       float q[4];
@@ -181,6 +283,7 @@
       if (pr.f32) st4<float>((float*)pr.out + row * D + c, q); else st4<bf16>((bf16*)pr.out + row * D + c, q);
     }
   }
+  if (PART) ln_rows_exchange<NG>(lnx, d, v, ok, D, partial + (size_t)blockIdx.x * 2 * D);
 }
 
 template <typename TO>
@@ -230,9 +333,13 @@
 __global__ __launch_bounds__(256) void ln_bwd_rows2_kernel(const TG* __restrict__ dy2, const float* __restrict__ x2, const float* __restrict__ mean2, const float* __restrict__ rstd2,
                                                            const float* __restrict__ g2, const float* __restrict__ dres2, float* __restrict__ dx2,
                                                            const float* __restrict__ x1, const float* __restrict__ mean1, const float* __restrict__ rstd1,
-                                                           const float* __restrict__ g1, float* __restrict__ dx1, long long M, int D, LnPrep pr) {
-  const int lane = threadIdx.x & 63; const long long row = (long long)blockIdx.x * 4 + (threadIdx.x >> 6);
-  if (row >= M) return;
+                                                           const float* __restrict__ g1, float* __restrict__ dx1, long long M, int D, LnPrep pr,
+                                                           float* __restrict__ partial2 = nullptr, float* __restrict__ partial1 = nullptr) {
+  extern __shared__ __attribute__((aligned(16))) float lnx[];
+  const int lane = threadIdx.x & 63; const long long row0 = (long long)blockIdx.x * 4 + (threadIdx.x >> 6);
+  const bool ok = row0 < M, PART = partial2 != nullptr;
+  if (!PART && !ok) return;
+  const long long row = ok ? row0 : M - 1;
   float d[2][4], v[2][4], o[2][4], gg[2][4], w1[2][4], gg1[2][4];
   const float mu2 = mean2[row], rs2 = rstd2[row], mu1 = mean1[row], rs1 = rstd1[row];
   DropKey dk; dk.k0 = 0u; dk.thr = 0u; dk.scale = 1.f;
@@ -252,27 +359,28 @@
 #pragma unroll
   for (int i = 0; i < 2; ++i)
 #pragma unroll
-    for (int e = 0; e < 4; ++e) { const float xh = (v[i][e] - mu2) * rs2, t = d[i][e] * gg[i][e]; v[i][e] = xh; s1 += t; s2 += t * xh; }
+    for (int e = 0; e < 4; ++e) { const float xh = ln_xhat(v[i][e], mu2, rs2), t = ln_mul(d[i][e], gg[i][e]); v[i][e] = xh; s1 = ln_add(s1, t); s2 = __builtin_fmaf(t, xh, s2); }
   s1 = wave_sum(s1) / D; s2 = wave_sum(s2) / D;
 #pragma unroll
   for (int i = 0; i < 2; ++i) {
     const int c = lane * 4 + i * 256;
 #pragma unroll
-    for (int e = 0; e < 4; ++e) o[i][e] += rs2 * (d[i][e] * gg[i][e] - s1 - v[i][e] * s2);
-    if (c < D) st4<float>(dx2 + row * D + c, o[i]); else { o[i][0] = o[i][1] = o[i][2] = o[i][3] = 0.f; }
+    for (int e = 0; e < 4; ++e) o[i][e] = ln_dx(o[i][e], rs2, ln_mul(d[i][e], gg[i][e]), s1, v[i][e], s2);
+    if (c < D) { if (!PART || ok) st4<float>(dx2 + row * D + c, o[i]); } else { o[i][0] = o[i][1] = o[i][2] = o[i][3] = 0.f; }
   }
   float t1 = 0.f, t2 = 0.f;
 #pragma unroll
   for (int i = 0; i < 2; ++i)
 #pragma unroll
-    for (int e = 0; e < 4; ++e) { const float xh = (w1[i][e] - mu1) * rs1, t = o[i][e] * gg1[i][e]; w1[i][e] = xh; t1 += t; t2 += t * xh; }
+    for (int e = 0; e < 4; ++e) { const float xh = ln_xhat(w1[i][e], mu1, rs1), t = ln_mul(o[i][e], gg1[i][e]); w1[i][e] = xh; t1 = ln_add(t1, t); t2 = __builtin_fmaf(t, xh, t2); }
   t1 = wave_sum(t1) / D; t2 = wave_sum(t2) / D;
 #pragma unroll
   for (int i = 0; i < 2; ++i) {
     const int c = lane * 4 + i * 256; if (c >= D) break;
     float r[4];
 #pragma unroll
-    for (int e = 0; e < 4; ++e) r[e] = rs1 * (o[i][e] * gg1[i][e] - t1 - w1[i][e] * t2);
+    for (int e = 0; e < 4; ++e) r[e] = ln_dx(0.f, rs1, ln_mul(o[i][e], gg1[i][e]), t1, w1[i][e], t2);
+    if (PART && !ok) continue;
     st4<float>(dx1 + row * D + c, r);
     if (pr.out) {
       float q[4], ds[4]; drop4(dk, (unsigned long long)row * D + c, ds);
@@ -280,6 +388,10 @@
       for (int e = 0; e < 4; ++e) q[e] = r[e] * (pr.alpha * ds[e]);
       if (pr.f32) st4<float>((float*)pr.out + row * D + c, q); else st4<bf16>((bf16*)pr.out + row * D + c, q);
     }
+  }
+  if (PART) {
+    ln_rows_exchange<2>(lnx, d, v, ok, D, partial2 + (size_t)blockIdx.x * 2 * D);
+    ln_rows_exchange<2>(lnx + 8 * D, o, w1, ok, D, partial1 + (size_t)blockIdx.x * 2 * D);
   }
 }
 extern "C" int avec_layernorm_bwd2(int dtype, const void* dy2, const float* x2, const float* mean2, const float* rstd2, const float* gamma2, const float* dres2, float* dx2,
@@ -291,6 +403,22 @@
   dim3 grid((unsigned)((M + 3) / 4));
   if (dtype == AVEC_F32) hipLaunchKernelGGL(ln_bwd_rows2_kernel<float>, grid, dim3(256), 0, st, (const float*)dy2, x2, mean2, rstd2, gamma2, dres2, dx2, x1, mean1, rstd1, gamma1, dx1, M, D, pr);
   else hipLaunchKernelGGL(ln_bwd_rows2_kernel<bf16>, grid, dim3(256), 0, st, (const bf16*)dy2, x2, mean2, rstd2, gamma2, dres2, dx2, x1, mean1, rstd1, gamma1, dx1, M, D, pr);
+  AVEC_LAUNCH_CHECK(); return 0;
+}
+
+extern "C" int avec_layernorm_bwd2_partials(int dtype, const void* dy2, const float* x2, const float* mean2, const float* rstd2, const float* gamma2, const float* dres2, float* dx2,
+                                            const float* x1, const float* mean1, const float* rstd1, const float* gamma1, float* dx1,
+                                            void* prep, float prep_alpha, float prep_drop_p, const unsigned long long* rng, unsigned rng_stream,
+                                            float* partial2, float* partial1, long long partial_floats, long long M, int D, hipStream_t st) {
+  AVEC_CHECK_ARG(dy2 && x2 && mean2 && rstd2 && gamma2 && dx2 && x1 && mean1 && rstd1 && gamma1 && dx1, "layernorm_bwd2_partials: null pointer");
+  AVEC_CHECK_ARG(M > 0 && M < (1ll << 31) && D > 0 && D % 4 == 0 && D <= 512 && (!prep || prep_drop_p <= 0.f || rng), "layernorm_bwd2_partials: D=%d must be a multiple of 4 in [4, 512]; dropout needs rng", D);
+  const long long need = ((M + 3) / 4) * 2 * D;
+  AVEC_CHECK_ARG(partial2 && partial1 && partial2 != partial1 && avec_aligned16(partial2) && avec_aligned16(partial1) && partial_floats >= need,
+                 "layernorm_bwd2_partials: two tensors of partial rows, %lld floats each (16-byte aligned), %lld needed", partial_floats, need);
+  LnPrep pr; pr.out = prep; pr.alpha = prep_alpha; pr.p = prep ? prep_drop_p : 0.f; pr.rng = rng; pr.stream = rng_stream; pr.f32 = dtype == AVEC_F32;
+  dim3 grid((unsigned)((M + 3) / 4)); const size_t lds = (size_t)16 * D * sizeof(float);
+  if (dtype == AVEC_F32) hipLaunchKernelGGL((ln_bwd_rows2_kernel<float>), grid, dim3(256), lds, st, (const float*)dy2, x2, mean2, rstd2, gamma2, dres2, dx2, x1, mean1, rstd1, gamma1, dx1, M, D, pr, partial2, partial1);
+  else hipLaunchKernelGGL((ln_bwd_rows2_kernel<bf16>), grid, dim3(256), lds, st, (const bf16*)dy2, x2, mean2, rstd2, gamma2, dres2, dx2, x1, mean1, rstd1, gamma1, dx1, M, D, pr, partial2, partial1);
   AVEC_LAUNCH_CHECK(); return 0;
 }
 
@@ -385,6 +513,24 @@
   LnPrep pr; pr.out = prep; pr.alpha = prep_alpha; pr.p = prep_drop_p; pr.rng = rng; pr.stream = rng_stream; pr.f32 = dtype == AVEC_F32;
   return layernorm_bwd_impl(dtype, dy, dy_f32, x, mean, rstd, gamma, dx, dres, nullptr, nullptr, M, D, pr, st);
 }
+extern "C" long long avec_layernorm_partial_floats(long long M, int D) { return (M > 0 && D > 0) ? ((M + 3) / 4) * 2 * D : 0; }
+extern "C" int avec_layernorm_bwd_partials(int dtype, const void* dy, int dy_f32, const float* x, const float* mean, const float* rstd, const float* gamma,
+                                           float* dx, const float* dres, void* prep, float prep_alpha, float prep_drop_p, const unsigned long long* rng, unsigned rng_stream,
+                                           float* partial, long long partial_floats, long long M, int D, hipStream_t st) {
+  AVEC_CHECK_ARG(dy && x && mean && rstd && gamma && dx, "layernorm_bwd_partials: null pointer");
+  AVEC_CHECK_ARG(M > 0 && M < (1ll << 31) && D > 0 && D % 4 == 0 && D <= 1536, "layernorm_bwd_partials: D=%d must be a multiple of 4 and <= 1536", D);
+  AVEC_CHECK_ARG(!prep || prep_drop_p <= 0.f || rng, "layernorm_bwd_partials: dropout needs rng");
+  AVEC_CHECK_ARG(partial && avec_aligned16(partial) && partial_floats >= avec_layernorm_partial_floats(M, D),
+                 "layernorm_bwd_partials: partial rows of %lld floats (16-byte aligned), %lld needed (avec_layernorm_partial_floats)", partial_floats, avec_layernorm_partial_floats(M, D));
+  LnPrep pr; pr.out = prep; pr.alpha = prep_alpha; pr.p = prep ? prep_drop_p : 0.f; pr.rng = rng; pr.stream = rng_stream; pr.f32 = dtype == AVEC_F32;
+  const dim3 grid((unsigned)((M + 3) / 4)); const bool f32in = dy_f32 || dtype == AVEC_F32;
+  const size_t lds = (size_t)8 * D * sizeof(float);
+#define AVEC_LN_ROWS(TG, NG) hipLaunchKernelGGL((ln_bwd_rows_kernel<TG, NG>), grid, dim3(256), lds, st, (const TG*)dy, x, mean, rstd, gamma, dx, dres, M, D, pr, partial)
+  if (D <= 512) { if (f32in) AVEC_LN_ROWS(float, 2); else AVEC_LN_ROWS(bf16, 2); }
+  else { if (f32in) AVEC_LN_ROWS(float, 6); else AVEC_LN_ROWS(bf16, 6); }
+#undef AVEC_LN_ROWS
+  AVEC_LAUNCH_CHECK(); return 0;
+}
 
 template <typename T>
 __global__ __launch_bounds__(256) void grad_prep_kernel(const float* __restrict__ dout, long long ldd, T* __restrict__ dacc, float alpha, float p,
diff --git a/avec_amd/lib.py b/avec_amd/lib.py
--- a/avec_amd/lib.py
+++ b/avec_amd/lib.py
@@ -75,8 +75,16 @@
                 ("ctx_bo", ctypes.c_void_p), ("ctx_off", ctypes.c_void_p), ("ctx_cnt", ctypes.c_void_p), ("cont_tok", ctypes.c_void_p), ("cont_lp", ctypes.c_void_p)]
 
 
-TN_GROUP_MAX, LN_GROUP_MAX, WGRAD_GROUP_MAX = 32, 40, 16
-ABI_STRUCTS = (Rows, Epilogue, Attn, TnItem, TnBatched, LnItem, Fp8Item, WgradItem, NGram)
+FIN_MAXNV = 20
+
+
+class FinItem(ctypes.Structure):
+    _fields_ = [("partial", ctypes.c_void_p), ("dst", ctypes.c_void_p * FIN_MAXNV), ("colblocks", ctypes.c_int), ("nslots", ctypes.c_int), ("NV", ctypes.c_int),
+                ("W", ctypes.c_int), ("C", ctypes.c_int), ("dstride", ctypes.c_int)]
+
+
+TN_GROUP_MAX, LN_GROUP_MAX, WGRAD_GROUP_MAX, FIN_GROUP_MAX = 32, 40, 16, 40
+ABI_STRUCTS = (Rows, Epilogue, Attn, TnItem, TnBatched, LnItem, Fp8Item, WgradItem, NGram, FinItem)
 
 
 def _ctype(decl):
diff --git a/avec_amd/ops.py b/avec_amd/ops.py
--- a/avec_amd/ops.py
+++ b/avec_amd/ops.py
@@ -6,7 +6,7 @@
 
 from . import fp8
 from . import runtime as rt
-from .lib import (ACT_GELU, ACT_NONE, ACT_RELU, ACT_SWISH, BF16, LN_GROUP_MAX, ROWS_CONV_BWD, ROWS_CONV_FWD, ROWS_PLAIN, ROWS_STEM3D, TN_GROUP_MAX, WGRAD_GROUP_MAX, Attn, Epilogue, LnItem, Rows, TnBatched, TnItem,
+from .lib import (ACT_GELU, ACT_NONE, ACT_RELU, ACT_SWISH, BF16, FIN_GROUP_MAX, LN_GROUP_MAX, ROWS_CONV_BWD, ROWS_CONV_FWD, ROWS_PLAIN, ROWS_STEM3D, TN_GROUP_MAX, WGRAD_GROUP_MAX, Attn, Epilogue, FinItem, LnItem, Rows, TnBatched, TnItem,
                   WgradItem, lib)
 
 _byref = ctypes.byref
@@ -225,6 +225,7 @@
 _QUEUE_KINDS = {
     "tn": _QueueKind(TnItem, TN_GROUP_MAX, "gemm_tn_grouped", lambda: BF16, (1, ROWS_PLAIN), lambda it: 2.0 * it.M * (it.I + it.J) + 4.0 * it.I * it.J, True),
     "ln": _QueueKind(LnItem, LN_GROUP_MAX, "layernorm_param_grads_grouped", rt.dt, None, None, True),
+    "fin": _QueueKind(FinItem, FIN_GROUP_MAX, "col_finalize_grouped", None, None, None, True),
     "cw": _QueueKind(WgradItem, WGRAD_GROUP_MAX, "wgrad3x3_c128_grouped", None, (2, 2), _wgrad3x3_bytes, False),
     "cw64": _QueueKind(WgradItem, WGRAD_GROUP_MAX, "wgrad3x3_c64_grouped", None, (2, 2), _wgrad3x3_bytes, False),
 }
@@ -378,10 +379,33 @@
     return None
 
 
+LN_ROW_PARTIALS = True
+
+
+def _ln_partials(M, D, ref):
+    return empty((lib.raw("avec_layernorm_partial_floats")(M, D),), torch.float32, ref)
+
+
+def _queue_ln_fin(part, w, b, M, D):
+    it = FinItem()
+    it.partial, it.colblocks, it.nslots, it.NV, it.W, it.C, it.dstride = part.data_ptr(), 1, (M + 3) // 4, 2, D, D, 1
+    it.dst[0], it.dst[1] = grad_of(w).data_ptr(), grad_of(b).data_ptr()
+    _pass().pending().push("fin", it, [part])
+
+
 def layernorm_bwd(dy, dy_f32, x, mean, rstd, w, b, M, D, dres=None, prep=None):
     dx = empty((M, D), torch.float32, x)
     gw, gb = grad_of(w), grad_of(b)
     if D <= 1024 and D % 4 == 0 and _in_backward():
+        if LN_ROW_PARTIALS:
+            pt, (alpha, drop_p, sid) = (None, (1.0, 0.0, 0)) if prep is None else (empty((M, D), rt.act_dtype(), x), prep)
+            part = _ln_partials(M, D, x)
+            lib.layernorm_bwd_partials(rt.dt(), dy.data_ptr(), int(dy_f32), x.data_ptr(), mean.data_ptr(), rstd.data_ptr(), w.data_ptr(), dx.data_ptr(), _p(dres),
+                                       _p(pt), alpha, drop_p, _rng(x.device, drop_p), sid, part.data_ptr(), part.numel(), M, D, rt.stream())
+            if pt is not None:
+                _pass().prep[dx.data_ptr()] = (pt, M, D, alpha, drop_p, sid)
+            _queue_ln_fin(part, w, b, M, D)
+            return dx
         if prep is not None:
             pt = empty((M, D), rt.act_dtype(), x)
             alpha, drop_p, sid = prep
@@ -405,10 +429,18 @@
         pt = empty((M, D), rt.act_dtype(), x2)
         alpha, drop_p, sid = req1
         _pass().prep[dx1.data_ptr()] = (pt, M, D, alpha, drop_p, sid)
+    if LN_ROW_PARTIALS:
+        part2, part1 = _ln_partials(M, D, x2), _ln_partials(M, D, x2)
+        lib.layernorm_bwd2_partials(rt.dt(), dy2.data_ptr(), x2.data_ptr(), mean2.data_ptr(), rstd2.data_ptr(), w2.data_ptr(), dres2.data_ptr(), dx2.data_ptr(),
+                                    x1.data_ptr(), mean1.data_ptr(), rstd1.data_ptr(), w1.data_ptr(), dx1.data_ptr(), _p(pt), alpha, drop_p, _rng(x2.device, drop_p), sid,
+                                    part2.data_ptr(), part1.data_ptr(), part2.numel(), M, D, rt.stream())
+        _pass().ln2[dx2.data_ptr()] = (dx1, ctx1, dx2, dx2._version, part1)
+        _queue_ln_fin(part2, w2, b2, M, D)
+        return dx2
     lib.layernorm_bwd2(rt.dt(), dy2.data_ptr(), x2.data_ptr(), mean2.data_ptr(), rstd2.data_ptr(), w2.data_ptr(), dres2.data_ptr(), dx2.data_ptr(),
                        x1.data_ptr(), mean1.data_ptr(), rstd1.data_ptr(), w1.data_ptr(), dx1.data_ptr(), _p(pt), alpha, drop_p, _rng(x2.device, drop_p), sid, M, D,
                        rt.stream())
-    _pass().ln2[dx2.data_ptr()] = (dx1, ctx1, dx2, dx2._version)
+    _pass().ln2[dx2.data_ptr()] = (dx1, ctx1, dx2, dx2._version, None)
     defer_ln_param_grads(dy2, False, x2, mean2, rstd2, w2, b2, M, D)
     return dx2
 
@@ -526,7 +558,10 @@
         if p is not None:
             r = p.ln2.pop(dy.data_ptr(), None)
             if r is not None and r[1] is ctx and dy.dtype == torch.float32 and dy.is_contiguous() and (dy is r[2] or dy._base is r[2]) and r[2]._version == r[3]:
-                defer_ln_param_grads(dy.reshape(M, D), True, x2, mean, rstd, w, b, M, D)
+                if r[4] is not None:
+                    _queue_ln_fin(r[4], w, b, M, D)
+                else:
+                    defer_ln_param_grads(dy.reshape(M, D), True, x2, mean, rstd, w, b, M, D)
                 return r[0].view(shp), None, None, None, None
         dx = layernorm_bwd(_f32c(dy.reshape(M, D)), True, x2, mean, rstd, w, b, M, D, prep=req)
         return dx.view(shp), None, None, None, None
@@ -1018,6 +1053,17 @@
     return K // 2
 
 CONVMOD_BN_FUSE = True
+DW_FIN_DEFER = True
+
+
+def _dw_partials(B, T, C, K, stride, dw, ref):
+    if not (DW_FIN_DEFER and _in_backward()):
+        return None, None
+    n = lib.raw("avec_dwconv_bwd_partial_floats")(B, T, C, stride)
+    part = empty((n,), torch.float32, ref)
+    it = FinItem()
+    lib.dwconv_bwd_fin_item(part.data_ptr(), grad_of(dw.weight).data_ptr(), None if dw.bias is None else grad_of(dw.bias).data_ptr(), B, T, C, K, stride, _byref(it))
+    return part, it
 
 
 class ConvModuleFn(torch.autograd.Function):
@@ -1071,16 +1117,29 @@
         if use_batch and CONVMOD_BN_FUSE and stride == 1 and not rt.sync_batchnorm():
             dstats = rt.zeros_scratch(2 * Dp, da.device)
             lib.bn_bwd_reduce(rt.dt(), da.data_ptr(), c.data_ptr(), None, st.ss.data_ptr(), ACT_SWISH, dstats.data_ptr(), Mo, Dp, rt.stream())
-            lib.dwconv_glu_bwd_bn(rt.dt(), da.data_ptr(), c.data_ptr(), st.ss.data_ptr(), bn.weight.data_ptr(), dstats.data_ptr(), float(Mo), u.data_ptr(), dw.weight.data_ptr(),
-                                  du.data_ptr(), grad_of(dw.weight).data_ptr(), None if dw.bias is None else grad_of(dw.bias).data_ptr(),
-                                  grad_of(bn.weight).data_ptr(), grad_of(bn.bias).data_ptr(), B, T, Dp, K, dw_pad_left(dw), rt.stream())
+            part, fin = _dw_partials(B, T, Dp, K, 1, dw, da)
+            if part is not None:
+                lib.dwconv_glu_bwd_bn_partials(rt.dt(), da.data_ptr(), c.data_ptr(), st.ss.data_ptr(), bn.weight.data_ptr(), dstats.data_ptr(), float(Mo), u.data_ptr(),
+                                               dw.weight.data_ptr(), du.data_ptr(), part.data_ptr(), part.numel(), grad_of(bn.weight).data_ptr(), grad_of(bn.bias).data_ptr(),
+                                               B, T, Dp, K, dw_pad_left(dw), rt.stream())
+                _pass().pending().push("fin", fin, [part])
+            else:
+                lib.dwconv_glu_bwd_bn(rt.dt(), da.data_ptr(), c.data_ptr(), st.ss.data_ptr(), bn.weight.data_ptr(), dstats.data_ptr(), float(Mo), u.data_ptr(), dw.weight.data_ptr(),
+                                      du.data_ptr(), grad_of(dw.weight).data_ptr(), None if dw.bias is None else grad_of(dw.bias).data_ptr(),
+                                      grad_of(bn.weight).data_ptr(), grad_of(bn.bias).data_ptr(), B, T, Dp, K, dw_pad_left(dw), rt.stream())
         else:
             if use_batch:
                 dc, _ = bn_backward(bn, st, cptr, Mo, da, c, None, ACT_SWISH, Mo)
             else:
                 dc = _bn_eval_backward(bn, st, da, c, ACT_SWISH, Mo)
-            lib.dwconv_glu_bwd(rt.dt(), dc.data_ptr(), u.data_ptr(), dw.weight.data_ptr(), du.data_ptr(), grad_of(dw.weight).data_ptr(),
-                               None if dw.bias is None else grad_of(dw.bias).data_ptr(), B, T, Dp, K, stride, dw_pad_left(dw), rt.stream())
+            part, fin = _dw_partials(B, T, Dp, K, stride, dw, da)
+            if part is not None:
+                lib.dwconv_glu_bwd_partials(rt.dt(), dc.data_ptr(), u.data_ptr(), dw.weight.data_ptr(), du.data_ptr(), part.data_ptr(), part.numel(),
+                                            B, T, Dp, K, stride, dw_pad_left(dw), rt.stream())
+                _pass().pending().push("fin", fin, [part])
+            else:
+                lib.dwconv_glu_bwd(rt.dt(), dc.data_ptr(), u.data_ptr(), dw.weight.data_ptr(), du.data_ptr(), grad_of(dw.weight).data_ptr(),
+                                   None if dw.bias is None else grad_of(dw.bias).data_ptr(), B, T, Dp, K, stride, dw_pad_left(dw), rt.stream())
         linear_bwd_weight(du, h, pw1.weight, M, bias=pw1.bias)
         dh = linear_bwd_input(du, pw1.weight, M, out_f32=False)
         if res_conv is None:
diff --git a/include/avec_hip.h b/include/avec_hip.h
--- a/include/avec_hip.h
+++ b/include/avec_hip.h
@@ -113,6 +113,21 @@
   long long M; int D; int dy_f32;
 } avec_ln_item_t;
 int avec_layernorm_param_grads_grouped(int dtype, const avec_ln_item_t* items, int n, hipStream_t stream);
+#define AVEC_FIN_GROUP_MAX 40
+#define AVEC_FIN_MAXNV 20
+typedef struct avec_fin_item {
+  const float* partial; float* dst[AVEC_FIN_MAXNV];
+  int colblocks, nslots, NV, W, C, dstride;
+} avec_fin_item_t;
+int avec_col_finalize_grouped(const avec_fin_item_t* items, int n, hipStream_t stream);
+long long avec_layernorm_partial_floats(long long M, int D);
+int avec_layernorm_bwd_partials(int dtype, const void* dy, int dy_f32, const float* x, const float* mean, const float* rstd, const float* gamma,
+                                float* dx, const float* dres, void* prep, float prep_alpha, float prep_drop_p, const unsigned long long* rng, unsigned rng_stream,
+                                float* partial, long long partial_floats, long long M, int D, hipStream_t stream);
+int avec_layernorm_bwd2_partials(int dtype, const void* dy2, const float* x2, const float* mean2, const float* rstd2, const float* gamma2, const float* dres2, float* dx2,
+                                 const float* x1, const float* mean1, const float* rstd1, const float* gamma1, float* dx1,
+                                 void* prep, float prep_alpha, float prep_drop_p, const unsigned long long* rng, unsigned rng_stream,
+                                 float* partial2, float* partial1, long long partial_floats, long long M, int D, hipStream_t stream);
 int avec_grad_prep(int dtype, const float* dout, long long ld, void* dacc, float alpha, float drop_p, const unsigned long long* rng,
                    unsigned rng_stream, float* dbias, long long M, int N, hipStream_t stream);
 int avec_colsum(int dtype, const void* x, long long ld, float* out, long long M, int N, hipStream_t stream);
@@ -162,6 +177,12 @@
                         int B, int T, int C, int K, int stride, int pad_left, hipStream_t stream);
 int avec_dwconv_glu_bwd_bn(int dtype, const void* da, const void* c, const float* ss, const float* gamma, const float* dstats, float count, const void* u, const float* w,
                            void* du, float* dw, float* dbias, float* dgamma, float* dbeta, int B, int T, int C, int K, int pad_left, hipStream_t stream);
+long long avec_dwconv_bwd_partial_floats(int B, int T, int C, int stride);
+int avec_dwconv_bwd_fin_item(const float* partial, float* dw, float* dbias, int B, int T, int C, int K, int stride, avec_fin_item_t* item);
+int avec_dwconv_glu_bwd_partials(int dtype, const void* dc, const void* u, const float* w, void* du, float* partial, long long partial_floats,
+                                 int B, int T, int C, int K, int stride, int pad_left, hipStream_t stream);
+int avec_dwconv_glu_bwd_bn_partials(int dtype, const void* da, const void* c, const float* ss, const float* gamma, const float* dstats, float count, const void* u, const float* w,
+                                    void* du, float* partial, long long partial_floats, float* dgamma, float* dbeta, int B, int T, int C, int K, int pad_left, hipStream_t stream);
 
 typedef struct avec_attn {
   const void *q, *k, *v; long long ld;
```

Result: no change. 1879 (-0.1%).
